# HUSRCF/JaTSR-Just-audio-transformer-super-solution

Measured on AMD Instinct MI355X. Metric: DiT latent-frames/sec (B=28,C=1024,T=512, 50-step CFG), higher is better.
Workload: dtype bf16; 1 GPU; v3mod2 DiT 50-step CFG=3.0 flow-matching sampling, hipGraph, B=28/GPU C=1024 T=512; B_per_gpu=28, global_batch=28, T=512, C=1024, euler_steps=50, weights=recipe (random-init, non-zero adaLN/final), parallelism=replicas x1, no collective in the loop, rccl_ranks=1

## Files before the change

### include/jat_hip.h

```cpp
#ifndef JAT_HIP_H
#define JAT_HIP_H

#include <stddef.h>
#include <stdint.h>

#ifdef __cplusplus
extern "C" {
#endif

#define JAT_OK 0
#define JAT_E_INVALID (-1)
#define JAT_E_HIP (-2)
#define JAT_E_STATE (-3)
#define JAT_E_SEQLEN (-4)

#define JAT_NORM_RMS_W 0
#define JAT_NORM_LN_NOAFFINE 1

typedef struct jat_model jat_model;
typedef struct jat_sampler jat_sampler;

typedef struct jat_config {
  int32_t input_channels;
  int32_t cond_channels;
  int32_t patch_len;
  int32_t hidden_size;
  int32_t depth;
  int32_t num_q_heads;
  int32_t num_kv_heads;
  int32_t bottleneck_dim;
  int32_t mlp_hidden;
  int32_t norm_mode;
} jat_config;

typedef struct jat_tensor_ref {
  const char* name;
  const float* data;
  int64_t numel;
} jat_tensor_ref;

const char* jat_last_error(void);
int jat_version(void);
int jat_operand_dtype(void);

int jat_model_create(const jat_config* cfg, jat_model** out);
void jat_model_destroy(jat_model* m);
int jat_model_load_weights(jat_model* m, const jat_tensor_ref* named, int32_t n, void* stream);
int jat_model_workspace_bytes(const jat_model* m, int32_t B, int32_t T, size_t* out);
int jat_model_set_switch(jat_model* m, const char* name, int32_t value);

int jat_forward(jat_model* m, const float* x_t, const float* t, const float* x_cond, float* x_pred,
                int32_t B, int32_t T, void* workspace, size_t workspace_bytes, void* stream);

int jat_block_forward(jat_model* m, int32_t layer, const float* x, const float* t_emb, float* y,
                      int32_t B, int32_t N, void* workspace, size_t workspace_bytes, void* stream);
int jat_attn_forward(jat_model* m, int32_t layer, const float* x, float* y, int32_t B, int32_t N,
                     void* workspace, size_t workspace_bytes, void* stream);
int jat_time_embed(jat_model* m, const float* t, float* t_emb, int32_t B, void* workspace,
                   size_t workspace_bytes, void* stream);

int jat_sampler_create(jat_model* m, int32_t B, int32_t T, int32_t steps, float cfg_scale,
                       jat_sampler** out);
void jat_sampler_destroy(jat_sampler* s);
int jat_sampler_info(const jat_sampler* sampler, int32_t* folded, int32_t* fused_attn, int64_t* fold_bytes);
int jat_sampler_set_lengths(jat_sampler* sampler, const int32_t* frames, int32_t n, void* stream);

int jat_sampler_run(jat_sampler* s, const float* lr_latent, const float* z0_noise, float* z_out,
                    int32_t use_graph, void* stream);
int jat_cfg_euler_step(const float* x_pred_2B, float* z, float cfg_scale, float t, float dt, int32_t B,
                       int32_t C, int32_t T, void* stream);

int jat_channel_affine(const float* in, const float* mean, const float* std, float* out, int32_t B,
                       int32_t C, int32_t T, int32_t inverse, void* stream);
int jat_crossfade_pair(const float* prev, int32_t Tp, const float* cur, int32_t Tc, int32_t overlap,
                       float* out, int32_t rows, void* stream);

typedef struct jat_trainer jat_trainer;
int jat_trainer_create(jat_model* m, const jat_tensor_ref* params, int32_t n_params, float* params_flat,
                       float* grads_flat, float* exp_avg, float* exp_avg_sq, int64_t total, int32_t B, int32_t T,
                       void* stream, jat_trainer** out);
void jat_trainer_destroy(jat_trainer* tr);
int jat_trainer_set_grad_hook(jat_trainer* tr, void (*hook)(int64_t off, int64_t n, void* user), void* user);
int jat_trainer_set_regularisers(jat_trainer* tr, const float* dropout, const float* drop_path);
int jat_trainer_set_latent_loss(jat_trainer* tr, double latent_weight, double freq_weight, double ms_weight,
                                double consistency_weight, double low_freq_phase_ratio, double strict_cutoff,
                                double soft_cutoff);
int jat_trainer_set_charbonnier(jat_trainer* tr, double eps);
int jat_trainer_loss_terms(jat_trainer* tr, float* out6, void* stream);
int jat_trainer_workspace_bytes(const jat_trainer* tr, size_t* out);
int jat_trainer_repack(jat_trainer* tr, void* stream);
int jat_trainer_prepare(jat_trainer* tr, const float* hr_norm, float* cond, const float* noise,
                        const float* cond_noise, float cond_noise_ratio, int32_t adaptive, const float* keep,
                        const float* t, float* z_t, void* stream);
int jat_trainer_fwd_bwd(jat_trainer* tr, const float* z_t, const float* t, const float* x_cond, const float* target,
                        const float* cond_clean, float loss_scale, uint64_t rng_seed, float* loss_out, float* x_pred_out,
                        void* stream);
int jat_trainer_optim(jat_trainer* tr, float lr, float beta1, float beta2, float eps, float weight_decay,
                      float max_grad_norm, float loss_scale, int32_t step, float* grad_norm_out, void* stream);

int jat_k_norm_modulate(const float* x, const float* w, const float* shift, const float* scale,
                        int64_t mod_bstride, uint16_t* y_bf16, int32_t M, int32_t D, int32_t rows_per_batch,
                        int32_t norm_mode, void* stream);
int jat_k_gemm(const uint16_t* A, const uint16_t* W, const float* bias, void* C, int32_t M, int32_t N,
               int32_t K, int32_t epilogue, const float* gate, int64_t gate_bstride, int32_t rows_per_batch,
               int32_t variant, void* stream);
int jat_k_gemm_fold(const uint16_t* A, const uint16_t* W, const float* bias, void* C, int32_t M, int32_t N, int32_t K,
                    int32_t epilogue, const float* gate, int64_t gate_bstride, int32_t rows_per_batch, uint16_t* hi,
                    uint16_t* lo, float* part_out, const float* part_in, int32_t part_in_np, int32_t variant, void* stream);
int jat_k_gemm_splitk(const uint16_t* A, const uint16_t* W, float* parts, int32_t M, int32_t N, int32_t K, int32_t ksplit,
                      int32_t variant, void* stream);
int jat_k_qkv_attn(const uint16_t* A, const uint16_t* Wg, const float* bias, uint16_t* out, int32_t M, int32_t Hkv, int32_t K,
                   const float* rope_inv_freq, const float* part_in, int32_t part_in_np, void* stream);
int jat_k_gemm_wave_n(int32_t variant);
int jat_k_gemm_plan(const jat_model* m, int32_t site, int32_t M, int32_t N, int32_t K, int32_t folding, int32_t* variant,
                    int32_t* ksplit);
int jat_k_weight_grad(const uint16_t* dY, const uint16_t* X, float* dW, float* db, int32_t tokens, int32_t out, int32_t in,
                      int32_t ksplit, void* work, size_t work_bytes, void* stream);
int jat_k_attention(const uint16_t* q, const uint16_t* k, const uint16_t* vt, uint16_t* o, int32_t B,
                    int32_t N, int32_t Hq, int32_t Hkv, int32_t Npad, void* stream);
int jat_k_latent_loss(const float* pred, const float* target, const float* lr, float* dpred, float* out6,
                      int32_t rows, int32_t T, double latent_weight, double freq_weight, double ms_weight,
                      double consistency_weight, double low_freq_phase_ratio, double strict_cutoff, double soft_cutoff,
                      float loss_scale, void* work, size_t work_bytes, void* stream);
int jat_k_recon_loss(const float* pred, const float* target, float* dpred, float* loss_out, int64_t n, double eps,
                     float loss_scale, void* work, size_t work_bytes, void* stream);
int jat_k_cast_bf16(const float* in, uint16_t* out, int64_t n, void* stream);

int jat_k_attention_train(const uint16_t* q, const uint16_t* k, const uint16_t* vt, uint16_t* o, float* lse, int32_t B,
                          int32_t N, int32_t Hq, int32_t Hkv, int32_t Npad, uint64_t seed, int32_t site, float p, void* stream);
int jat_k_attention_bwd(const uint16_t* q, const uint16_t* k, const uint16_t* vt, const uint16_t* o, const uint16_t* dout,
                        const float* lse, uint16_t* dqkv, const float* rope_cos, const float* rope_sin, int32_t B, int32_t N,
                        int32_t Hq, int32_t Hkv, int32_t Npad, uint64_t seed, int32_t site, float p, int32_t split_heads,
                        void* work, size_t work_bytes, void* stream);
int jat_k_norm_bwd(const float* x, const uint16_t* dy, const float* w, const float* scale, int64_t mod_bstride, float* dx,
                   int32_t accumulate, float* dshift, float* dscale, int64_t dmod_bstride, float* dw, int32_t B, int32_t D,
                   int32_t ntok, int32_t mode, void* work, size_t work_bytes, void* stream);
int jat_k_gate_bwd(const float* dx, const uint16_t* y, const float* gate, int64_t gate_bstride, uint16_t* dy, float* dgate,
                   int64_t dgate_bstride, int32_t B, int32_t D, int32_t ntok, uint64_t seed, int32_t path_site, float path_p,
                   int32_t elem_site, float elem_p, void* work, size_t work_bytes, void* stream);
int jat_k_resid_gate(const float* x_in, const uint16_t* y, const float* gate, int64_t gate_bstride, float* x_out, int32_t M,
                     int32_t D, int32_t ntok, uint64_t seed, int32_t path_site, float path_p, int32_t elem_site, float elem_p,
                     void* stream);
int jat_k_gelu(const uint16_t* in, uint16_t* out, int64_t n, uint64_t seed, int32_t site, float p, void* stream);
int jat_k_gelu_bwd(const uint16_t* pre, uint16_t* d, int64_t n, uint64_t seed, int32_t site, float p, void* stream);
int jat_k_adamw(float* p, const float* g, float* m, float* v, int64_t n, float lr, float beta1, float beta2, float eps,
                float weight_decay, float max_grad_norm, float loss_scale, int32_t step, float* grad_norm_out, void* work,
                size_t work_bytes, void* stream);
int jat_k_small_dw(const float* dy, int64_t ldy, const float* x, int64_t ldx, float* dW, float* db, int32_t B, int32_t N,
                   int32_t K, int32_t silu_x, void* stream);
int jat_k_small_dx(const float* dy, int64_t ldy, const void* W, int32_t w_is_bf16, float* dx, int32_t B, int32_t N, int32_t K,
                   int32_t accumulate, const float* silu_pre, void* work, size_t work_bytes, void* stream);

int jat_prof_gemm_site(jat_model* m, int32_t site, int32_t max_launches);
int jat_prof_collect(jat_model* m, double* total_ms, int32_t* launches, double* flops, int32_t* variant);

typedef struct jat_dac_decoder jat_dac_decoder;
#define JAT_DAC_BF16X3 0
#define JAT_DAC_BF16 1
typedef struct jat_dac_config {
  int32_t latent_channels;
  int32_t channels;
  int32_t n_blocks;
  int32_t strides[4];
} jat_dac_config;
int jat_dac_decoder_create(const jat_dac_config* cfg, const jat_tensor_ref* named, int32_t n, int32_t max_B,
                           int32_t max_T, void* stream, jat_dac_decoder** out);
void jat_dac_decoder_destroy(jat_dac_decoder* d);
int jat_dac_workspace_bytes(const jat_dac_decoder* d, size_t* bytes);
int jat_dac_decode(jat_dac_decoder* d, const float* z, float* audio, int32_t B, int32_t T, int32_t precision, void* stream);
int jat_dac_pack_weight(int32_t kind, const float* w, int32_t cin, int32_t cout, int32_t k_or_stride, float* out);
int jat_k_dac_split(const float* x, uint16_t* hi, uint16_t* lo, int64_t n, void* stream);
int jat_k_dac_conv(const uint16_t* a_hi, const uint16_t* a_lo, const uint16_t* w_hi, const uint16_t* w_lo,
                   const float* bias, const float* res, float* out32, const float* alpha, uint16_t* o_hi, uint16_t* o_lo,
                   int32_t B, int32_t T, int32_t cin, int32_t N, int32_t cch, int32_t taps, int32_t dil,
                   int32_t precision, void* stream);
int jat_k_dac_tail(const float* x, const float* alpha, const float* w, const float* bias, float* out, int32_t B, int32_t T,
                   int32_t C, void* stream);

typedef struct jat_dac_encoder jat_dac_encoder;
#define JAT_DAC_MAX_CODEBOOKS 9
typedef struct jat_dac_encoder_config {
  int32_t channels;
  int32_t hidden_size;
  int32_t n_blocks;
  int32_t strides[4];
  int32_t n_codebooks;
  int32_t codebook_size;
  int32_t codebook_dim;
} jat_dac_encoder_config;
int jat_dac_encoder_create(const jat_dac_encoder_config* cfg, const jat_tensor_ref* named, int32_t n, int32_t max_B,
                           int32_t max_T, void* stream, jat_dac_encoder** out);
// ... 46 lines not shown
```

### jatsr-just-audio-transformer-super-solution_amd/_lib.py

```python
from __future__ import annotations

import ctypes as C
import os

_HERE = os.path.dirname(os.path.abspath(__file__))
OPERAND_DTYPE = os.environ.get("JAT_OPERAND_DTYPE", "bf16").lower()
if OPERAND_DTYPE not in ("bf16", "fp16", "float16", "bfloat16"):
    raise ValueError(f"JAT_OPERAND_DTYPE must be bf16 or fp16, got {OPERAND_DTYPE!r}")
OPERAND_DTYPE = "fp16" if OPERAND_DTYPE in ("fp16", "float16") else "bf16"
LIB_PATH = os.environ.get("JAT_LIB_PATH") or os.path.join(
    _HERE, "csrc", "libjat_hip_fp16.so" if OPERAND_DTYPE == "fp16" else "libjat_hip.so")

JAT_OK, JAT_E_INVALID, JAT_E_HIP, JAT_E_STATE, JAT_E_SEQLEN = 0, -1, -2, -3, -4
NORM_RMS_W, NORM_LN_NOAFFINE = 0, 1


class JatConfig(C.Structure):
    _fields_ = [(n, C.c_int32) for n in (
        "input_channels", "cond_channels", "patch_len", "hidden_size", "depth", "num_q_heads",
        "num_kv_heads", "bottleneck_dim", "mlp_hidden", "norm_mode")]


class JatDacConfig(C.Structure):
    _fields_ = [("latent_channels", C.c_int32), ("channels", C.c_int32), ("n_blocks", C.c_int32),
                ("strides", C.c_int32 * 4)]


class JatDacEncoderConfig(C.Structure):
    _fields_ = [("channels", C.c_int32), ("hidden_size", C.c_int32), ("n_blocks", C.c_int32), ("strides", C.c_int32 * 4),
                ("n_codebooks", C.c_int32), ("codebook_size", C.c_int32), ("codebook_dim", C.c_int32)]


class JatTensorRef(C.Structure):
    _fields_ = [("name", C.c_char_p), ("data", C.c_void_p), ("numel", C.c_int64)]


_VP, _I32, _I64, _F32, _SZ = C.c_void_p, C.c_int32, C.c_int64, C.c_float, C.c_size_t
SIGNATURES = {
    "jat_last_error": (C.c_char_p, []),
    "jat_version": (C.c_int, []),
    "jat_operand_dtype": (C.c_int, []),
    "jat_model_create": (C.c_int, [C.POINTER(JatConfig), C.POINTER(_VP)]),
    "jat_model_destroy": (None, [_VP]),
    "jat_model_load_weights": (C.c_int, [_VP, C.POINTER(JatTensorRef), _I32, _VP]),
    "jat_model_set_switch": (C.c_int, [_VP, C.c_char_p, _I32]),
    "jat_model_workspace_bytes": (C.c_int, [_VP, _I32, _I32, C.POINTER(_SZ)]),
    "jat_forward": (C.c_int, [_VP, _VP, _VP, _VP, _VP, _I32, _I32, _VP, _SZ, _VP]),
    "jat_block_forward": (C.c_int, [_VP, _I32, _VP, _VP, _VP, _I32, _I32, _VP, _SZ, _VP]),
    "jat_attn_forward": (C.c_int, [_VP, _I32, _VP, _VP, _I32, _I32, _VP, _SZ, _VP]),
    "jat_time_embed": (C.c_int, [_VP, _VP, _VP, _I32, _VP, _SZ, _VP]),
    "jat_sampler_create": (C.c_int, [_VP, _I32, _I32, _I32, _F32, C.POINTER(_VP)]),
    "jat_sampler_destroy": (None, [_VP]),
    "jat_sampler_run": (C.c_int, [_VP, _VP, _VP, _VP, _I32, _VP]),
    "jat_sampler_info": (C.c_int, [_VP, _VP, _VP, _VP]),
    "jat_sampler_set_lengths": (C.c_int, [_VP, C.POINTER(_I32), _I32, _VP]),
    "jat_cfg_euler_step": (C.c_int, [_VP, _VP, _F32, _F32, _F32, _I32, _I32, _I32, _VP]),
    "jat_channel_affine": (C.c_int, [_VP, _VP, _VP, _VP, _I32, _I32, _I32, _I32, _VP]),
    "jat_crossfade_pair": (C.c_int, [_VP, _I32, _VP, _I32, _I32, _VP, _I32, _VP]),
    "jat_k_norm_modulate": (C.c_int, [_VP, _VP, _VP, _VP, _I64, _VP, _I32, _I32, _I32, _I32, _VP]),
    "jat_k_gemm": (C.c_int, [_VP, _VP, _VP, _VP, _I32, _I32, _I32, _I32, _VP, _I64, _I32, _I32, _VP]),
    "jat_k_gemm_fold": (C.c_int, [_VP, _VP, _VP, _VP, _I32, _I32, _I32, _I32, _VP, _I64, _I32, _VP, _VP, _VP, _VP, _I32, _I32, _VP]),
    "jat_k_gemm_splitk": (C.c_int, [_VP, _VP, _VP, _I32, _I32, _I32, _I32, _I32, _VP]),
    "jat_k_gemm_wave_n": (C.c_int, [_I32]),
    "jat_k_gemm_plan": (C.c_int, [_VP, _I32, _I32, _I32, _I32, _I32, _VP, _VP]),
    "jat_k_qkv_attn": (C.c_int, [_VP, _VP, _VP, _VP, _I32, _I32, _I32, _VP, _VP, _I32, _VP]),
    "jat_k_weight_grad": (C.c_int, [_VP, _VP, _VP, _VP, _I32, _I32, _I32, _I32, _VP, _SZ, _VP]),
    "jat_k_attention": (C.c_int, [_VP, _VP, _VP, _VP, _I32, _I32, _I32, _I32, _I32, _VP]),
    "jat_k_recon_loss": (C.c_int, [_VP, _VP, _VP, _VP, _I64, C.c_double, _F32, _VP, _SZ, _VP]),
    "jat_k_cast_bf16": (C.c_int, [_VP, _VP, _I64, _VP]),
    "jat_k_attention_train": (C.c_int, [_VP] * 5 + [_I32] * 5 + [C.c_uint64, _I32, _F32, _VP]),
    "jat_k_attention_bwd": (C.c_int, [_VP] * 9 + [_I32] * 5 + [C.c_uint64, _I32, _F32, _I32, _VP, _SZ, _VP]),
    "jat_k_norm_bwd": (C.c_int, [_VP, _VP, _VP, _VP, _I64, _VP, _I32, _VP, _VP, _I64, _VP] + [_I32] * 4 + [_VP, _SZ, _VP]),
    "jat_k_gate_bwd": (C.c_int, [_VP, _VP, _VP, _I64, _VP, _VP, _I64] + [_I32] * 3 + [C.c_uint64, _I32, _F32, _I32, _F32] +
                       [_VP, _SZ, _VP]),
    "jat_k_resid_gate": (C.c_int, [_VP, _VP, _VP, _I64, _VP] + [_I32] * 3 + [C.c_uint64, _I32, _F32, _I32, _F32, _VP]),
    "jat_k_gelu": (C.c_int, [_VP, _VP, _I64, C.c_uint64, _I32, _F32, _VP]),
    "jat_k_gelu_bwd": (C.c_int, [_VP, _VP, _I64, C.c_uint64, _I32, _F32, _VP]),
    "jat_k_adamw": (C.c_int, [_VP, _VP, _VP, _VP, _I64] + [_F32] * 7 + [_I32, _VP, _VP, _SZ, _VP]),
    "jat_k_small_dw": (C.c_int, [_VP, _I64, _VP, _I64, _VP, _VP] + [_I32] * 4 + [_VP]),
    "jat_k_small_dx": (C.c_int, [_VP, _I64, _VP, _I32, _VP] + [_I32] * 4 + [_VP, _VP, _SZ, _VP]),
    "jat_k_latent_loss": (C.c_int, [_VP, _VP, _VP, _VP, _VP, _I32, _I32] + [C.c_double] * 7 + [_F32, _VP, _SZ, _VP]),
    "jat_trainer_create": (C.c_int, [_VP, C.POINTER(JatTensorRef), _I32, _VP, _VP, _VP, _VP, _I64, _I32, _I32, _VP,
                                     C.POINTER(_VP)]),
    "jat_trainer_destroy": (None, [_VP]),
    "jat_trainer_workspace_bytes": (C.c_int, [_VP, C.POINTER(_SZ)]),
    "jat_trainer_repack": (C.c_int, [_VP, _VP]),
    "jat_trainer_prepare": (C.c_int, [_VP, _VP, _VP, _VP, _VP, _F32, _I32, _VP, _VP, _VP, _VP]),
    "jat_trainer_set_grad_hook": (C.c_int, [_VP, _VP, _VP]),
    "jat_trainer_set_regularisers": (C.c_int, [_VP, C.POINTER(_F32), C.POINTER(_F32)]),
    "jat_trainer_set_latent_loss": (C.c_int, [_VP] + [C.c_double] * 7),
    "jat_trainer_set_charbonnier": (C.c_int, [_VP, C.c_double]),
    "jat_trainer_loss_terms": (C.c_int, [_VP, _VP, _VP]),
    "jat_trainer_fwd_bwd": (C.c_int, [_VP, _VP, _VP, _VP, _VP, _VP, _F32, C.c_uint64, _VP, _VP, _VP]),
    "jat_trainer_optim": (C.c_int, [_VP, _F32, _F32, _F32, _F32, _F32, _F32, _F32, _I32, _VP, _VP]),
    "jat_prof_gemm_site": (C.c_int, [_VP, _I32, _I32]),
    "jat_prof_collect": (C.c_int, [_VP, C.POINTER(C.c_double), C.POINTER(_I32), C.POINTER(C.c_double), C.POINTER(_I32)]),
    "jat_dac_decoder_create": (C.c_int, [C.c_void_p, C.POINTER(JatTensorRef), _I32, _I32, _I32, _VP, C.POINTER(_VP)]),
    "jat_dac_decoder_destroy": (None, [_VP]),
    "jat_dac_workspace_bytes": (C.c_int, [_VP, C.POINTER(_SZ)]),
    "jat_dac_decode": (C.c_int, [_VP, _VP, _VP, _I32, _I32, _I32, _VP]),
    "jat_dac_pack_weight": (C.c_int, [_I32, _VP, _I32, _I32, _I32, _VP]),
    "jat_k_dac_split": (C.c_int, [_VP, _VP, _VP, _I64, _VP]),
    "jat_k_dac_conv": (C.c_int, [_VP] * 10 + [_I32] * 8 + [_VP]),
    "jat_k_dac_tail": (C.c_int, [_VP] * 5 + [_I32] * 3 + [_VP]),
    "jat_dac_encoder_create": (C.c_int, [C.c_void_p, C.POINTER(JatTensorRef), _I32, _I32, _I32, _VP, C.POINTER(_VP)]),
    "jat_dac_encoder_destroy": (None, [_VP]),
    "jat_dac_encoder_workspace_bytes": (C.c_int, [_VP, C.POINTER(_SZ)]),
    "jat_dac_encode": (C.c_int, [_VP] * 6 + [_I32] * 4 + [_VP]),
    "jat_k_dac_head": (C.c_int, [_VP] * 7 + [_I32] * 3 + [_VP]),
    "jat_k_dac_rvq": (C.c_int, [_VP] * 10 + [_I32] * 4 + [_VP]),
    "jat_resample_table": (C.c_int, [_I32, _I32, _I32, C.c_double, _VP] + [C.POINTER(_I32)] * 4),
    "jat_resampler_create": (C.c_int, [_I32, _I32, _I32, C.c_double, _VP, C.POINTER(_VP)]),
    "jat_resampler_destroy": (None, [_VP]),
    "jat_resample_out_length": (C.c_int, [_VP, _I64, C.POINTER(_I64)]),
    "jat_resample": (C.c_int, [_VP, _VP, _VP, _I32, _I64, _VP]),
    "jat_channel_stats": (C.c_int, [_VP, _I32, _I32, _I32, _VP, _VP, _VP, _SZ, _VP]),
    "jat_mel_filterbank": (C.c_int, [_I32, _I32, _I32, _VP]),
    "jat_stft_frames": (C.c_int, [_I64, _I32, C.POINTER(_I64)]),
    "jat_audio_metrics_create": (C.c_int, [_I32, _I32, _I32, _I32, _VP, C.POINTER(_VP)]),
    "jat_audio_metrics_destroy": (None, [_VP]),
    "jat_audio_metrics_workspace_bytes": (C.c_int, [_VP, _I32, _I64, C.POINTER(_SZ)]),
    "jat_audio_metrics_run": (C.c_int, [_VP, _VP, _VP, _I32, _I64, _I32, _VP, _VP, _VP, _VP, _VP, _SZ, _VP]),
    "jat_stft": (C.c_int, [_VP, _VP, _VP, _I32, _I64, _VP, _VP, _VP]),
    "jat_latent_gather": (C.c_int, [_VP] * 10 + [_I32] * 3 + [_VP]),
    "jat_train_monitor": (C.c_int, [_VP, _VP, _VP, _I64, _VP, _VP, _SZ, _VP]),
}
MONITOR_WORK_BYTES = 49152

GRAD_HOOK = C.CFUNCTYPE(None, C.c_int64, C.c_int64, C.c_void_p)

_lib = None


class JatError(RuntimeError):
    pass


def lib():
    global _lib
    if _lib is None:
        if not os.path.exists(LIB_PATH):
            raise JatError(f"{LIB_PATH} not found: build it first (`python -c 'import __graft_entry__ as g; "
                           f"g.build()'` or `make -C {os.path.dirname(LIB_PATH)}`); there is no CPU fallback")
        h = C.CDLL(LIB_PATH)
# ... 40 lines not shown
```

### jatsr-just-audio-transformer-super-solution_amd/csrc/elementwise.hip

```cpp
#include "jat_kernels.h"
#include "jat_gelu.h"
#include "jat_dtype.h"
#include <cstdlib>

__device__ __forceinline__ unsigned short f2bf_e(float f) { return jat_f2op(f); }
__device__ __forceinline__ uint2 pack4_e(float a, float b, float c, float d) {
  uint2 r;
  r.x = jat_pack2(a, b);
  r.y = jat_pack2(c, d);
  return r;
}
__device__ __forceinline__ float wave_sum(float v) {
#pragma unroll
  for (int o = 32; o > 0; o >>= 1) v += __shfl_xor(v, o);
  return v;
}
__device__ __forceinline__ float silu_f(float x) { return x / (1.0f + __expf(-x)); }

__global__ void __launch_bounds__(256) norm_modulate_kernel(const float* __restrict__ x, const float* __restrict__ w,
                                                            const float* __restrict__ shift,
                                                            const float* __restrict__ scale, int64_t mod_bstride,
                                                            bf16_t* __restrict__ y, int M, int D, int ntok, int mode) {
  const int lane = threadIdx.x & 63;
  const int row = blockIdx.x * 4 + (threadIdx.x >> 6);
  if (row >= M) return;
  const int nch = D >> 8;
  const float* xr = x + (int64_t)row * D + lane * 4;
  float4 v[8];
  float s1 = 0.f, s2 = 0.f;
#pragma unroll
  for (int c = 0; c < 8; ++c) {
    if (c < nch) {
      v[c] = *(const float4*)(xr + c * 256);
      s1 += v[c].x + v[c].y + v[c].z + v[c].w;
      s2 += v[c].x * v[c].x + v[c].y * v[c].y + v[c].z * v[c].z + v[c].w * v[c].w;
    }
  }
  float mu = 0.f, rstd = 1.f;
  if (mode == 0) {
    s2 = wave_sum(s2);
    rstd = rsqrtf(s2 / (float)D + 1e-6f);
  } else if (mode == 1) {
    s1 = wave_sum(s1);
    mu = s1 / (float)D;
    float var = 0.f;
#pragma unroll
    for (int c = 0; c < 8; ++c)
      if (c < nch) {
        const float a = v[c].x - mu, b2 = v[c].y - mu, c2 = v[c].z - mu, d2 = v[c].w - mu;
        var += a * a + b2 * b2 + c2 * c2 + d2 * d2;
      }
    var = wave_sum(var);
    rstd = rsqrtf(var / (float)D + 1e-6f);
  }
  const int b = row / ntok;
  const float* sh = shift ? shift + (int64_t)b * mod_bstride + lane * 4 : nullptr;
  const float* sc = scale ? scale + (int64_t)b * mod_bstride + lane * 4 : nullptr;
  bf16_t* yr = y + (int64_t)row * D + lane * 4;
#pragma unroll
  for (int c = 0; c < 8; ++c) {
    if (c < nch) {
      float4 t = v[c];
      t.x = (t.x - mu) * rstd; t.y = (t.y - mu) * rstd; t.z = (t.z - mu) * rstd; t.w = (t.w - mu) * rstd;
      if (mode == 0 && w) {
        const float4 ww = *(const float4*)(w + c * 256 + lane * 4);
        t.x *= ww.x; t.y *= ww.y; t.z *= ww.z; t.w *= ww.w;
      }
      if (sc) {
        const float4 a = *(const float4*)(sc + c * 256);
        const float4 s = *(const float4*)(sh + c * 256);
        t.x = t.x * (1.f + a.x) + s.x; t.y = t.y * (1.f + a.y) + s.y;
        t.z = t.z * (1.f + a.z) + s.z; t.w = t.w * (1.f + a.w) + s.w;
      }
      *(uint2*)(yr + c * 256) = pack4_e(t.x, t.y, t.z, t.w);
    }
  }
}

typedef __attribute__((ext_vector_type(4))) float f32x4_e;
template <int NCH>
__global__ void __launch_bounds__(256) norm_modulate_rows_kernel(const float* __restrict__ x, const float* __restrict__ w,
                                                                 const float* __restrict__ shift,
                                                                 const float* __restrict__ scale, int64_t mod_bstride,
                                                                 bf16_t* __restrict__ y, int M, int ntok, int mode) {
  constexpr int D = NCH * 256;
// ... 223 lines not shown
  if (n <= 0) return hipSuccess;
  hipLaunchKernelGGL(cast_bf16_kernel, dim3((unsigned)((n + 1023) / 1024)), dim3(256), 0, s, in, out, n, 1);
  return hipGetLastError();
}

__global__ void cast_bf16_rope_rows_kernel(const float* __restrict__ in, bf16_t* __restrict__ out, int rows, int cols) {
  const int64_t i = ((int64_t)blockIdx.x * blockDim.x + threadIdx.x) * 4;
  if (i >= (int64_t)rows * cols) return;
  const int r = (int)(i / cols), c = (int)(i - (int64_t)r * cols);
  const int h = r >> 6, q = r & 63;
  const int src = (h << 6) + (q >> 1) + ((q & 1) << 5);
  const float4 v = *(const float4*)(in + (int64_t)src * cols + c);
  *(uint2*)(out + i) = pack4_e(v.x, v.y, v.z, v.w);
}
hipError_t launch_cast_bf16_rope_rows(const float* in, bf16_t* out, int rows, int cols, hipStream_t s) {
  if (rows % 64 != 0 || cols % 4 != 0) return hipErrorInvalidValue;
  const int64_t n = (int64_t)rows * cols;
  hipLaunchKernelGGL(cast_bf16_rope_rows_kernel, dim3((unsigned)((n / 4 + 255) / 256)), dim3(256), 0, s, in, out, rows,
                     cols);
  return hipGetLastError();
}

__global__ void fold_weight_kernel(const float* __restrict__ in, const float* __restrict__ w, const float* __restrict__ scale,
                                   bf16_t* __restrict__ out, int rows, int cols, int rope) {
  const int64_t i = ((int64_t)blockIdx.x * blockDim.x + threadIdx.x) * 4;
  if (i >= (int64_t)rows * cols) return;
  const int r = (int)(i / cols), c = (int)(i - (int64_t)r * cols);
  int src = r;
  if (rope) {
    const int h = r >> 6, q = r & 63;
    src = (h << 6) + (q >> 1) + ((q & 1) << 5);
  }
  const float4 v = *(const float4*)(in + (int64_t)src * cols + c);
  float4 g = *(const float4*)(w + c);
  if (scale) {
    const float4 sc = *(const float4*)(scale + c);
    g.x *= 1.0f + sc.x; g.y *= 1.0f + sc.y; g.z *= 1.0f + sc.z; g.w *= 1.0f + sc.w;
  }
  *(uint2*)(out + i) = pack4_e(v.x * g.x, v.y * g.y, v.z * g.z, v.w * g.w);
}
hipError_t launch_fold_weight(const float* in, const float* w, const float* scale, bf16_t* out, int rows, int cols, int rope,
                              hipStream_t s) {
  if ((rope && rows % 64 != 0) || cols % 4 != 0) return hipErrorInvalidValue;
  const int64_t n = (int64_t)rows * cols;
  hipLaunchKernelGGL(fold_weight_kernel, dim3((unsigned)((n / 4 + 255) / 256)), dim3(256), 0, s, in, w, scale, out, rows, cols, rope);
  return hipGetLastError();
}

__global__ void fold_scale_kernel(const float* __restrict__ w, const float* __restrict__ scale, int64_t in_stride,
                                  float* __restrict__ out, int64_t out_stride, int rows, int cols) {
  const int i = blockIdx.x * blockDim.x + threadIdx.x;
  if (i >= rows * cols) return;
  const int r = i / cols, k = i - r * cols;
  out[(int64_t)r * out_stride + k] = w[k] * (1.0f + scale[(int64_t)r * in_stride + k]);
}
hipError_t launch_fold_scale(const float* w, const float* scale, int64_t in_stride, float* out, int64_t out_stride,
                             int rows, int cols, hipStream_t s) {
  const int n = rows * cols;
  hipLaunchKernelGGL(fold_scale_kernel, dim3((n + 255) / 256), dim3(256), 0, s, w, scale, in_stride, out, out_stride, rows, cols);
  return hipGetLastError();
}
__global__ void gather_cast_rows_kernel(const float* __restrict__ in, int64_t in_stride, bf16_t* __restrict__ out, int rows,
                                        int cols) {
  const int i = blockIdx.x * blockDim.x + threadIdx.x;
  if (i >= rows * cols) return;
  const int r = i / cols, k = i - r * cols;
  out[(int64_t)r * cols + k] = f2bf_e(in[(int64_t)r * in_stride + k]);
}
hipError_t launch_gather_cast_rows(const float* in, int64_t in_stride, bf16_t* out, int rows, int cols, hipStream_t s) {
  const int n = rows * cols;
  hipLaunchKernelGGL(gather_cast_rows_kernel, dim3((n + 255) / 256), dim3(256), 0, s, in, in_stride, out, rows, cols);
  return hipGetLastError();
}

__global__ void __launch_bounds__(256) cfg_euler_kernel(const float* __restrict__ xp, float* __restrict__ z,
                                                        float cfg_scale, float denom, float dt, int use_cfg,
                                                        int direct, int64_t n) {
  const int64_t stride = (int64_t)gridDim.x * blockDim.x * 4;
  for (int64_t i = ((int64_t)blockIdx.x * blockDim.x + threadIdx.x) * 4; i < n; i += stride) {
    if (i + 3 < n) {
      float4 c = *(const float4*)(xp + i);
      if (use_cfg) {
        const float4 u = *(const float4*)(xp + n + i);
        c.x = u.x + cfg_scale * (c.x - u.x); c.y = u.y + cfg_scale * (c.y - u.y);
        c.z = u.z + cfg_scale * (c.z - u.z); c.w = u.w + cfg_scale * (c.w - u.w);
      }
      if (!direct) {
        const float4 zz = *(const float4*)(z + i);
        c.x = zz.x + __fdiv_rn(c.x - zz.x, denom) * dt; c.y = zz.y + __fdiv_rn(c.y - zz.y, denom) * dt;
        c.z = zz.z + __fdiv_rn(c.z - zz.z, denom) * dt; c.w = zz.w + __fdiv_rn(c.w - zz.w, denom) * dt;
      }
      *(float4*)(z + i) = c;
    } else {
      for (int64_t j = i; j < n; ++j) {
        float c = xp[j];
        if (use_cfg) { const float u = xp[n + j]; c = u + cfg_scale * (c - u); }
        if (!direct) c = z[j] + __fdiv_rn(c - z[j], denom) * dt;
        z[j] = c;
      }
    }
  }
}
hipError_t launch_cfg_euler(const float* xp, float* z, float cfg_scale, float t, float dt, int use_cfg,
                            int64_t n_per_half, hipStream_t s) {
  const int direct = !(t < 0.999f);
  const float denom = 1.0f - t + 1e-5f;
  int64_t blocks = (n_per_half / 4 + 255) / 256;
  if (blocks > 2048) blocks = 2048;
  if (blocks < 1) blocks = 1;
  hipLaunchKernelGGL(cfg_euler_kernel, dim3((unsigned)blocks), dim3(256), 0, s, xp, z, cfg_scale, denom, dt, use_cfg,
                     direct, n_per_half);
  return hipGetLastError();
}

__global__ void channel_affine_kernel(const float* __restrict__ in, const float* __restrict__ mean,
                                      const float* __restrict__ sd, float* __restrict__ out, int C, int T,
                                      int inverse, int64_t n) {
  const int64_t i = (int64_t)blockIdx.x * blockDim.x + threadIdx.x;
  if (i >= n) return;
  const int c = (int)((i / T) % C);
  out[i] = inverse ? in[i] * sd[c] + mean[c] : (in[i] - mean[c]) / sd[c];
}
hipError_t launch_channel_affine(const float* in, const float* mean, const float* std, float* out, int B, int C, int T,
                                 int inverse, hipStream_t s) {
  const int64_t n = (int64_t)B * C * T;
  if (n <= 0) return hipSuccess;
  hipLaunchKernelGGL(channel_affine_kernel, dim3((unsigned)((n + 255) / 256)), dim3(256), 0, s, in, mean, std, out, C,
                     T, inverse, n);
  return hipGetLastError();
}

__device__ __forceinline__ float linspace_at(float a, float b, int n, int i) {
  if (n == 1) return a;
  const float step = (b - a) / (float)(n - 1);
  return i < n / 2 ? fmaf(step, (float)i, a) : fmaf(-step, (float)(n - 1 - i), b);
}
__global__ void crossfade_pair_kernel(const float* __restrict__ prev, int Tp, const float* __restrict__ cur, int Tc,
                                      int ov, float* __restrict__ out, int rows) {
  const int To = Tp + Tc - ov;
  const int64_t i = (int64_t)blockIdx.x * blockDim.x + threadIdx.x;
  if (i >= (int64_t)rows * To) return;
  const int r = (int)(i / To), t = (int)(i - (int64_t)r * To);
  float v;
  if (t < Tp - ov) {
    v = prev[(int64_t)r * Tp + t];
  } else if (t < Tp) {
    const int k = t - (Tp - ov);
    v = prev[(int64_t)r * Tp + t] * linspace_at(1.f, 0.f, ov, k) + cur[(int64_t)r * Tc + k] * linspace_at(0.f, 1.f, ov, k);
  } else {
    v = cur[(int64_t)r * Tc + (t - Tp + ov)];
  }
  out[i] = v;
}
hipError_t launch_crossfade_pair(const float* prev, int Tp, const float* cur, int Tc, int overlap, float* out, int rows,
                                 hipStream_t s) {
  if (overlap < 0 || overlap > Tp || overlap > Tc) return hipErrorInvalidValue;
  const int64_t n = (int64_t)rows * (Tp + Tc - overlap);
  if (n <= 0) return hipSuccess;
  hipLaunchKernelGGL(crossfade_pair_kernel, dim3((unsigned)((n + 255) / 256)), dim3(256), 0, s, prev, Tp, cur, Tc,
                     overlap, out, rows);
  return hipGetLastError();
}

__global__ void __launch_bounds__(256) splitk_resid_finish_kernel(const float* __restrict__ part, int nsplit, int64_t stride,
                                                                  const float* __restrict__ bias, const float* __restrict__ gate,
                                                                  int64_t gate_bstride, int ntok, float* __restrict__ x, int M,
                                                                  int N) {
  const int64_t i = (int64_t)blockIdx.x * 256 + threadIdx.x;
  const int per_row = N / 4;
  if (i >= (int64_t)M * per_row) return;
  const int row = (int)(i / per_row), c = (int)(i % per_row) * 4;
  f32x4_e acc = *(const f32x4_e*)(part + (int64_t)row * N + c);
  for (int z = 1; z < nsplit; ++z) {
    const f32x4_e v = *(const f32x4_e*)(part + (int64_t)z * stride + (int64_t)row * N + c);
    acc[0] += v[0]; acc[1] += v[1]; acc[2] += v[2]; acc[3] += v[3];
  }
  const f32x4_e b = bias ? *(const f32x4_e*)(bias + c) : f32x4_e{0.f, 0.f, 0.f, 0.f};
  const f32x4_e g = *(const f32x4_e*)(gate + (int64_t)(row / ntok) * gate_bstride + c);
  f32x4_e xv = *(const f32x4_e*)(x + (int64_t)row * N + c);
#pragma unroll
  for (int j = 0; j < 4; ++j) xv[j] += g[j] * (acc[j] + b[j]);
  *(f32x4_e*)(x + (int64_t)row * N + c) = xv;
}
__global__ void __launch_bounds__(256) splitk_gelu_finish_kernel(const float* __restrict__ part, int nsplit, int64_t stride,
                                                                 const float* __restrict__ bias, const float* __restrict__ dual_add,
                                                                 int dual_rows, bf16_t* __restrict__ out, int64_t ldo, int M, int N) {
  const int64_t i = (int64_t)blockIdx.x * 256 + threadIdx.x;
  const int per_row = N / 4;
  if (i >= (int64_t)M * per_row) return;
  const int row = (int)(i / per_row), c = (int)(i % per_row) * 4;
  f32x4_e acc = *(const f32x4_e*)(part + (int64_t)row * N + c);
  for (int z = 1; z < nsplit; ++z) {
    const f32x4_e v = *(const f32x4_e*)(part + (int64_t)z * stride + (int64_t)row * N + c);
    acc[0] += v[0]; acc[1] += v[1]; acc[2] += v[2]; acc[3] += v[3];
  }
// ... 127 lines not shown
```

### jatsr-just-audio-transformer-super-solution_amd/csrc/gemm.hip

```cpp
#include "jat_kernels.h"
#include "jat_dtype.h"
#include "gemm_variants.h"

#include <type_traits>
#include <utility>

typedef jat_opx8 bf16x8;
typedef __attribute__((ext_vector_type(4))) float f32x4;
typedef __attribute__((ext_vector_type(4))) unsigned u32x4;
typedef __attribute__((address_space(3))) void* lds_ptr_t;

template <int I, int N, class F>
__device__ __forceinline__ void static_for(F&& f) {
  if constexpr (I < N) {
    f(std::integral_constant<int, I>{});
    static_for<I + 1, N>(f);
  }
}

__device__ __forceinline__ unsigned short f2bf(float f) { return jat_f2op(f); }
__device__ __forceinline__ uint2 pack4(float a, float b, float c, float d) {
  uint2 r;
  r.x = jat_pack2(a, b);
  r.y = jat_pack2(c, d);
  return r;
}
#include "jat_gelu.h"
__device__ __forceinline__ uint2 gelu_pack4(float a, float b, float c, float d) {
  f32x2 g[2] = {f32x2{a, b}, f32x2{c, d}};
  gelu_erf_n<2>(g);
  return pack4(g[0][0], g[0][1], g[1][0], g[1][1]);
}

__device__ __forceinline__ float2 rope_rot(float a, float b, float c, float s) {
  return float2{__builtin_fmaf(a, c, -(b * s)), __builtin_fmaf(b, c, a * s)};
}

template <int TM>
__device__ __forceinline__ void rows_rstd_issue(const GemmArgs& p, int row0, int lane, f32x4 (&rsv)[TM]) {
  const int lg = p.rs_np >> 3;
  const int rpi = 64 >> lg;
#pragma unroll
  for (int t = 0; t < TM; ++t) {
    const int row = min(row0 + t * rpi + (lane >> lg), p.M - 1);
    const float* ptr = p.rs_part + (int64_t)row * p.rs_np + (lane & ((1 << lg) - 1)) * 4;
    asm volatile("global_load_dwordx4 %0, %1, off" : "=v"(rsv[t]) : "v"(ptr) : "memory");
  }
}
template <int TM, int YOUNGER>
__device__ __forceinline__ void rows_rstd_reduce(const GemmArgs& p, f32x4 (&rsv)[TM], float (&sums)[TM]) {
  asm volatile("s_waitcnt vmcnt(%0)" ::"n"(YOUNGER) : "memory");
#pragma unroll
  for (int t = 0; t < TM; ++t) asm volatile("" : "+v"(rsv[t]));
  const int lpr = p.rs_np >> 2;
#pragma unroll
  for (int t = 0; t < TM; ++t) {
    float sq = (rsv[t][0] + rsv[t][1]) + (rsv[t][2] + rsv[t][3]);
    if (lpr >= 2) sq += __shfl_xor(sq, 1);
    if (lpr >= 4) sq += __shfl_xor(sq, 2);
    sums[t] = sq;
  }
}
template <int TM>
__device__ __forceinline__ void rows_rstd_finish(const GemmArgs& p, int lane, const float (&sums)[TM], float (&rstd)[TM]) {
  const int lg = p.rs_np >> 3, rlog = 6 - lg, frow = lane & 15;
  const float invk = 1.0f / (float)p.K;
  float sq[TM];
#pragma unroll
  for (int i = 0; i < TM; ++i) {
    const int ti = (i * 16) >> rlog;
    float sel = sums[0];
#pragma unroll
    for (int t = 1; t < TM; ++t) sel = (t == ti) ? sums[t] : sel;
    sq[i] = __shfl(sel, ((i * 16 + frow) & ((1 << rlog) - 1)) << lg);
  }
#pragma unroll
  for (int i = 0; i < TM; ++i) rstd[i] = rsqrtf(sq[i] * invk + 1e-6f);
}
template <int WM, int WN, int TM, int TN, int PIPE, int CE, int EPI>
__global__ void __launch_bounds__((WM * WN + (PIPE == 6 ? 4 : 0)) * 64, (WM * WN == 4 && TM * TN <= 20) ? 2 : 1)
    gemm_bf16_kernel(const GemmArgs p_in) {
  GemmArgs p = p_in;
#ifdef JAT_TIMELINE
  unsigned long long tl_[7] = {0, 0, 0, 0, 0, 0, 0}, tlx_[8] = {0, 0, 0, 0, 0, 0, 0, 0};
#define JAT_TL(i)                                                                          \
  if (p.dbg_out) {                                                                         \
    __builtin_amdgcn_sched_barrier(0);                                                     \
    asm volatile("s_memtime %0\n\ts_waitcnt lgkmcnt(0)" : "=s"(tl_[i])::"memory");       \
    __builtin_amdgcn_sched_barrier(0);                                                     \
  }
#define JAT_TLX(i)                                                                         \
  if (p.dbg_out) {                                                                         \
    __builtin_amdgcn_sched_barrier(0);                                                     \
    asm volatile("s_memtime %0\n\ts_waitcnt lgkmcnt(0)" : "=s"(tlx_[i])::"memory");      \
    __builtin_amdgcn_sched_barrier(0);                                                     \
  }
#define JAT_TLR(i)                                                                         \
  if (p.dbg_out) {                                                                         \
    __builtin_amdgcn_sched_barrier(0);                                                     \
    asm volatile("s_memrealtime %0\n\ts_waitcnt lgkmcnt(0)" : "=s"(tl_[i])::"memory");   \
    __builtin_amdgcn_sched_barrier(0);                                                     \
  }
#define JAT_TL_FLUSH()                                                                     \
  {                                                                                        \
    JAT_TL(4) JAT_TLR(6)                                                                   \
    if (p.dbg_out && (threadIdx.x & 63) == 0) {                                            \
      unsigned long long* o_ = p.dbg_out + ((size_t)blockIdx.x * (blockDim.x >> 6) + (threadIdx.x >> 6)) * 16; \
      for (int i_ = 0; i_ < 7; ++i_) o_[i_] = tl_[i_];                                     \
      o_[7] = blockIdx.x;                                                                  \
      for (int i_ = 0; i_ < 8; ++i_) o_[8 + i_] = tlx_[i_];                                \
    }                                                                                      \
  }
  JAT_TL(0) JAT_TLR(5)
#else
#define JAT_TL(i)
#define JAT_TLX(i)
#define JAT_TLR(i)
#define JAT_TL_FLUSH()
#endif
  if (p.ksplit > 1) {
    const int z = blockIdx.y;
    p.A += (int64_t)z * p.K;
    p.W += (int64_t)z * p.K;
    p.out = (float*)p.out + (int64_t)z * p.split_stride;
  }
  constexpr int BM = WM * TM * 16, BN = WN * TN * 16, BK = 64;
  constexpr int NW = WM * WN;
  constexpr int A_BYTES = BM * 128, B_BYTES = BN * 128, STAGE = A_BYTES + B_BYTES;
  constexpr int PA = BM / 8, PB = BN / 8;
  constexpr int AI = (PA + NW - 1) / NW, BI = (PB + NW - 1) / NW;
  static_assert(BM % 8 == 0 && BN % 8 == 0, "tile rows must be a multiple of 8");
  extern __shared__ __attribute__((aligned(16))) char smem[];

  const int tid = threadIdx.x, lane = tid & 63;
  const int wave = __builtin_amdgcn_readfirstlane(tid >> 6);
  const int wm = wave / WN, wn = wave % WN;

  const int tiles_m = (p.M + BM - 1) / BM, tiles_n = p.N / BN;
  int id;
  {
    const int nwg = gridDim.x, bid = blockIdx.x;
    const int q = nwg >> 3, r = nwg & 7, xcd = bid & 7;
    id = (xcd < r ? xcd * (q + 1) : r * (q + 1) + (xcd - r) * q) + (bid >> 3);
  }
  constexpr int GROUP = 8;
  const int per_group = GROUP * tiles_n;
  const int first_m = (id / per_group) * GROUP;
  const int gsz = min(tiles_m - first_m, GROUP);
  const int in_g = id % per_group;
  const int m0 = (first_m + in_g % gsz) * BM;
  const int n0 = (in_g / gsz) * BN;

  const int srow = lane >> 3;
  const int schunk = (lane & 7) ^ srow;
  const bf16_t* a_src[AI];
  const bf16_t* b_src[BI];
#pragma unroll
  for (int j = 0; j < AI; ++j) {
    const int r = min(wave + j * NW, PA - 1) * 8 + srow;
    const int gm = min(m0 + r, p.M - 1);
    a_src[j] = p.A + (int64_t)gm * p.lda + schunk * 8;
  }
#pragma unroll
  for (int j = 0; j < BI; ++j) {
    const int r = min(wave + j * NW, PB - 1) * 8 + srow;
    b_src[j] = p.W + (int64_t)(n0 + r) * p.ldw + schunk * 8;
  }
  auto stage = [&](int st, int kt) {
    char* sA = smem + st * STAGE;
    char* sB = sA + A_BYTES;
    const int koff = kt * BK;
#pragma unroll
    for (int j = 0; j < AI; ++j)
      if (PA % NW == 0 || wave + j * NW < PA)
        __builtin_amdgcn_global_load_lds((const void*)(a_src[j] + koff),
                                         (lds_ptr_t)(sA + min(wave + j * NW, PA - 1) * 1024), 16, 0, 0);
#pragma unroll
    for (int j = 0; j < BI; ++j)
      if (PB % NW == 0 || wave + j * NW < PB)
        __builtin_amdgcn_global_load_lds((const void*)(b_src[j] + koff),
                                         (lds_ptr_t)(sB + min(wave + j * NW, PB - 1) * 1024), 16, 0, 0);
  };

  f32x4 acc[TM][TN];
#pragma unroll
  for (int i = 0; i < TM; ++i)
#pragma unroll
    for (int j = 0; j < TN; ++j) acc[i][j] = f32x4{0.f, 0.f, 0.f, 0.f};

  const int frow = lane & 15, fg = lane >> 4;
  const int a_row_off = (wm * TM * 16 + frow) * 128;
  const int b_row_off = (wn * TN * 16 + frow) * 128;
  const int coff0 = ((0 + fg) ^ (frow & 7)) * 16, coff1 = ((4 + fg) ^ (frow & 7)) * 16;
  constexpr bool QA = EPI == EPI_QKV_ATTN;
  static_assert(!QA || (TN == 7 && WN == 4), "fused QKV + attention: 5 q + k + v tiles per wave column");
  auto ctile = [](int w, int j) { return QA ? (j < 5 ? w * 5 + j : j == 5 ? 20 + w : 24 + w) : w * TN + j; };
  auto b_frag_off = [&](int j) {
    return QA ? ctile(wn, j) * 2048 + frow * 128 : b_row_off + j * 2048;
  };

  auto read_frags = [&](bf16x8(&af)[TM], bf16x8(&wf)[TN], int st, int coff) {
    const char* sA = smem + st * STAGE;
    const char* sB = sA + A_BYTES;
#pragma unroll
    for (int i = 0; i < TM; ++i) af[i] = *(const bf16x8*)(sA + a_row_off + i * 2048 + coff);
#pragma unroll
    for (int j = 0; j < TN; ++j) wf[j] = *(const bf16x8*)(sB + b_row_off + j * 2048 + coff);
  };
  auto mma = [&](const bf16x8(&af)[TM], const bf16x8(&wf)[TN]) {
#pragma unroll
    for (int i = 0; i < TM; ++i)
#pragma unroll
      for (int j = 0; j < TN; ++j)
        acc[i][j] = JAT_MFMA_16x16x32(wf[j], af[i], acc[i][j], 0, 0, 0);
  };

  float rstd_rows[TM], rstd_sums[TM];
  [[maybe_unused]] f32x4 rstd_raw[TM];
#pragma unroll
  for (int i = 0; i < TM; ++i) rstd_rows[i] = 1.0f;
  if (p.rs_part) {
    rows_rstd_issue<TM>(p, m0 + wm * TM * 16, lane, rstd_raw);
    if constexpr (PIPE != 8) rows_rstd_reduce<TM, 0>(p, rstd_raw, rstd_sums);
  }

  const int nk = p.K / BK;
  if constexpr (PIPE == 6) {
    static_assert(NW == 8 && PA % 4 == 0 && PB % 4 == 0, "PIPE 6: 8 MFMA waves + 4 DMA waves");
    constexpr int NDW = 4, AI6 = PA / NDW, BI6 = PB / NDW;
    if (wave >= NW) {
      const int dw = wave - NW;
      const bf16_t* asrc[AI6];
      const bf16_t* bsrc[BI6];
#pragma unroll
      for (int j = 0; j < AI6; ++j)
        asrc[j] = p.A + (int64_t)min(m0 + (dw + j * NDW) * 8 + srow, p.M - 1) * p.lda + schunk * 8;
#pragma unroll
      for (int j = 0; j < BI6; ++j) bsrc[j] = p.W + (int64_t)(n0 + (dw + j * NDW) * 8 + srow) * p.ldw + schunk * 8;
      auto issue_a = [&](int st, int kt) {
#pragma unroll
        for (int j = 0; j < AI6; ++j)
          __builtin_amdgcn_global_load_lds((const void*)(asrc[j] + kt * BK),
                                           (lds_ptr_t)(smem + st * STAGE + (dw + j * NDW) * 1024), 16, 0, 0);
      };
      auto issue_b = [&](int st, int kt) {
#pragma unroll
        for (int j = 0; j < BI6; ++j)
          __builtin_amdgcn_global_load_lds((const void*)(bsrc[j] + kt * BK),
                                           (lds_ptr_t)(smem + st * STAGE + A_BYTES + (dw + j * NDW) * 1024), 16, 0, 0);
      };
      issue_a(0, 0);
      issue_b(0, 0);
      if (nk > 1) {
        issue_a(1, 1);
        issue_b(1, 1);
        asm volatile("s_waitcnt vmcnt(%0)" ::"n"(AI6 + BI6) : "memory");
      } else {
        asm volatile("s_waitcnt vmcnt(0)" ::: "memory");
      }
      __builtin_amdgcn_s_barrier();
      int st = 2;
      for (int sl = 0; sl <= 2 * nk; ++sl) {
        const int t = (sl >> 1) + 2;
        if (t < nk) {
          if (sl & 1) issue_b(st, t); else issue_a(st, t);
          asm volatile("s_waitcnt vmcnt(%0)" ::"n"(AI6 + BI6) : "memory");
        } else {
          asm volatile("s_waitcnt vmcnt(0)" ::: "memory");
        }
        __builtin_amdgcn_s_barrier();
        if (sl & 1) st = st == 2 ? 0 : st + 1;
      }
      if constexpr (CE && EPI <= EPI_QKV_ROPE) __builtin_amdgcn_s_barrier();
      return;
    }
    const int grp = wave >> 2;
    bf16x8 a0[TM], w0[TN], a1[TM], w1[TN];
    __builtin_amdgcn_s_barrier();
    if (grp == 1) __builtin_amdgcn_s_barrier();
    int cur = 0;
    for (int kt = 0; kt < nk; ++kt) {
      read_frags(a0, w0, cur, coff0);
      read_frags(a1, w1, cur, coff1);
      asm volatile("s_waitcnt lgkmcnt(0)" ::: "memory");
      __builtin_amdgcn_sched_barrier(0);
      __builtin_amdgcn_s_barrier();
      __builtin_amdgcn_s_setprio(1);
      mma(a0, w0);
      mma(a1, w1);
      __builtin_amdgcn_s_setprio(0);
      __builtin_amdgcn_sched_barrier(0);
      __builtin_amdgcn_s_barrier();
      cur = cur == 2 ? 0 : cur + 1;
    }
    if (grp == 0) __builtin_amdgcn_s_barrier();
  } else if constexpr (PIPE == 8) {
    static_assert(NW == 8, "quadrant ping-pong needs two waves per SIMD in one block");
    constexpr bool SPLIT_M = TM * TN > 20;
    constexpr int TMa = SPLIT_M ? (TM + 1) / 2 : TM, TMb = TM - TMa, TNa = (TN + 1) / 2, TNb = TN - TNa;
    constexpr int PA0 = WM * TMa * 2, PA1 = WM * TMb * 2, PB0 = WN * TNa * 2, PB1 = WN * TNb * 2;
    constexpr int CA0 = (PA0 + 7) / 8, CA1 = (PA1 + 7) / 8, CB0 = (PB0 + 7) / 8, CB1 = (PB1 + 7) / 8;
    constexpr int CTILE = CA0 + CA1 + CB0 + CB1;
    const int grp = wave >> 2;
    const char* a_base = (const char*)(p.A + (int64_t)m0 * p.lda);
    const char* b_base = (const char*)(p.W + (int64_t)n0 * p.ldw);
    unsigned oa0[CA0], oa1[CA1 > 0 ? CA1 : 1], ob0[CB0], ob1[CB1];
    int la0[CA0], la1[CA1 > 0 ? CA1 : 1], lb0[CB0], lb1[CB1];
    auto piece_row = [&](int q, int per, int tiles, int first) {
      const int w = q / per, in = q - w * per;
      return w * tiles * 16 + first * 16 + in * 8;
    };
#pragma unroll
    for (int j = 0; j < CA0; ++j) {
      const int r = piece_row(min(wave + 8 * j, PA0 - 1), TMa * 2, TM, 0);
      oa0[j] = (unsigned)((min(m0 + r + srow, p.M - 1) - m0) * (int)p.lda * 2 + schunk * 16);
      la0[j] = r * 128;
    }
#pragma unroll
    for (int j = 0; j < CA1; ++j) {
      const int r = piece_row(min(wave + 8 * j, PA1 - 1), TMb * 2, TM, TMa);
      oa1[j] = (unsigned)((min(m0 + r + srow, p.M - 1) - m0) * (int)p.lda * 2 + schunk * 16);
      la1[j] = r * 128;
    }
    auto piece_row_b = [&](int q, int per, int first) {
      const int w = q / per, in = q - w * per;
      return ctile(w, first + (in >> 1)) * 16 + (in & 1) * 8;
    };
#pragma unroll
    for (int j = 0; j < CB0; ++j) {
      const int r = piece_row_b(min(wave + 8 * j, PB0 - 1), TNa * 2, 0);
      ob0[j] = (unsigned)((r + srow) * (int)p.ldw * 2 + schunk * 16);
      lb0[j] = A_BYTES + r * 128;
    }
#pragma unroll
    for (int j = 0; j < CB1; ++j) {
      const int r = piece_row_b(min(wave + 8 * j, PB1 - 1), TNb * 2, TNa);
      ob1[j] = (unsigned)((r + srow) * (int)p.ldw * 2 + schunk * 16);
      lb1[j] = A_BYTES + r * 128;
    }
    auto dma_a0 = [&](int st, int kt) {
#pragma unroll
      for (int j = 0; j < CA0; ++j)
        __builtin_amdgcn_global_load_lds((const void*)(a_base + kt * 128 + oa0[j]), (lds_ptr_t)(smem + st * STAGE + la0[j]), 16, 0, 0);
    };
    auto dma_a1 = [&](int st, int kt) {
#pragma unroll
      for (int j = 0; j < CA1; ++j)
        __builtin_amdgcn_global_load_lds((const void*)(a_base + kt * 128 + oa1[j]), (lds_ptr_t)(smem + st * STAGE + la1[j]), 16, 0, 0);
    };
    auto dma_b0 = [&](int st, int kt) {
#pragma unroll
      for (int j = 0; j < CB0; ++j)
        __builtin_amdgcn_global_load_lds((const void*)(b_base + kt * 128 + ob0[j]), (lds_ptr_t)(smem + st * STAGE + lb0[j]), 16, 0, 0);
    };
    auto dma_b1 = [&](int st, int kt) {
#pragma unroll
      for (int j = 0; j < CB1; ++j)
        __builtin_amdgcn_global_load_lds((const void*)(b_base + kt * 128 + ob1[j]), (lds_ptr_t)(smem + st * STAGE + lb1[j]), 16, 0, 0);
    };
    bf16x8 fa[2][TMa], fb[2][TNa];
    auto rd_a = [&](int st, int i0, int cnt) {
      const char* sA = smem + st * STAGE + a_row_off + i0 * 2048;
#pragma unroll
      for (int i = 0; i < TMa; ++i)
        if (i < cnt) {
          fa[0][i] = *(const bf16x8*)(sA + i * 2048 + coff0);
          fa[1][i] = *(const bf16x8*)(sA + i * 2048 + coff1);
        }
    };
    auto rd_b = [&](int st, int j0, int cnt) {
      if constexpr (QA) {
        const char* sB = smem + st * STAGE + A_BYTES;
#pragma unroll
        for (int j = 0; j < TNa; ++j)
          if (j < cnt) {
            fb[0][j] = *(const bf16x8*)(sB + b_frag_off(j0 + j) + coff0);
            fb[1][j] = *(const bf16x8*)(sB + b_frag_off(j0 + j) + coff1);
          }
      } else {
        const char* sB = smem + st * STAGE + A_BYTES + b_row_off + j0 * 2048;
#pragma unroll
        for (int j = 0; j < TNa; ++j)
          if (j < cnt) {
            fb[0][j] = *(const bf16x8*)(sB + j * 2048 + coff0);
            fb[1][j] = *(const bf16x8*)(sB + j * 2048 + coff1);
          }
      }
    };
#define JAT_Q(I0, IC, J0, JC)                                                                                   \
  _Pragma("unroll") for (int ks = 0; ks < 2; ++ks)                                                              \
  _Pragma("unroll") for (int i = 0; i < (IC); ++i)                                                              \
  _Pragma("unroll") for (int j = 0; j < (JC); ++j)                                                              \
    acc[(I0) + i][(J0) + j] = (QA && (J0) + j == TN - 1)                                                        \
        ? JAT_MFMA_16x16x32(fa[ks][i], fb[ks][j], acc[(I0) + i][(J0) + j], 0, 0, 0)                             \
        : JAT_MFMA_16x16x32(fb[ks][j], fa[ks][i], acc[(I0) + i][(J0) + j], 0, 0, 0);
#define JAT_LOAD_END()                              \
  asm volatile("s_waitcnt lgkmcnt(0)" ::: "memory"); \
  __builtin_amdgcn_sched_barrier(0);                \
  __builtin_amdgcn_s_barrier();                     \
  __builtin_amdgcn_s_setprio(1);
#define JAT_MMA_END()                 \
  __builtin_amdgcn_s_setprio(0);      \
  __builtin_amdgcn_sched_barrier(0);  \
  __builtin_amdgcn_s_barrier();
// ... 493 lines not shown
    const int q = wave * 16 + frow;
    constexpr int G = 5;
    const int hbase = (n0 / 448) * G;
    bf16x8 qf[G][2];
#pragma unroll
    for (int h = 0; h < G; ++h) {
      qf[h][0] = *(const bf16x8*)(smem + SQ + h * 16384 + q * 128 + (((0 + fg) ^ (q & 7)) << 4));
      qf[h][1] = *(const bf16x8*)(smem + SQ + h * 16384 + q * 128 + (((4 + fg) ^ (q & 7)) << 4));
    }
    f32x4 st[G][8];
#pragma unroll
    for (int h = 0; h < G; ++h)
#pragma unroll
      for (int kt = 0; kt < 8; ++kt) st[h][kt] = f32x4{0.f, 0.f, 0.f, 0.f};
#pragma unroll
    for (int kt = 0; kt < 8; ++kt) {
      const int r = 32 * (kt >> 1) + 8 * (frow >> 2) + (frow & 3) + 4 * (kt & 1);
      const int ks = (r & 3) | (((r >> 3) & 1) << 2);
      const bf16x8 kf0 = *(const bf16x8*)(smem + SK + r * 128 + (((0 + fg) ^ ks) << 4));
      const bf16x8 kf1 = *(const bf16x8*)(smem + SK + r * 128 + (((4 + fg) ^ ks) << 4));
#pragma unroll
      for (int h = 0; h < G; ++h) {
        st[h][kt] = JAT_MFMA_16x16x32(kf0, qf[h][0], st[h][kt], 0, 0, 0);
        st[h][kt] = JAT_MFMA_16x16x32(kf1, qf[h][1], st[h][kt], 0, 0, 0);
      }
    }
    JAT_TLX(2)
    float inv[G];
    bf16x8 pf[G][4];
#pragma unroll
    for (int h = 0; h < G; ++h) {
      float mx = -1e30f;
#pragma unroll
      for (int kt = 0; kt < 8; ++kt) mx = fmaxf(mx, fmaxf(fmaxf(st[h][kt][0], st[h][kt][1]), fmaxf(st[h][kt][2], st[h][kt][3])));
      mx = fmaxf(mx, __shfl_xor(mx, 16));
      mx = fmaxf(mx, __shfl_xor(mx, 32));
      const float nb = -mx * p.attn_scale_log2e;
      float sum = 0.f;
#pragma unroll
      for (int kt = 0; kt < 8; ++kt)
#pragma unroll
        for (int e = 0; e < 4; ++e) {
          const float pv = __builtin_amdgcn_exp2f(fmaf(st[h][kt][e], p.attn_scale_log2e, nb));
          st[h][kt][e] = pv;
          sum += pv;
        }
      sum += __shfl_xor(sum, 16);
      sum += __shfl_xor(sum, 32);
      inv[h] = 1.0f / sum;
#pragma unroll
      for (int kk = 0; kk < 4; ++kk) {
        pf[h][kk] = jat_pack8(st[h][2 * kk], st[h][2 * kk + 1]);
      }
    }
    JAT_TLX(3)
    f32x4 o[G][4];
#pragma unroll
    for (int h = 0; h < G; ++h)
#pragma unroll
      for (int dt = 0; dt < 4; ++dt) o[h][dt] = f32x4{0.f, 0.f, 0.f, 0.f};
#pragma unroll
    for (int kk = 0; kk < 4; ++kk)
#pragma unroll
      for (int dt = 0; dt < 4; ++dt) {
        const int d = dt * 16 + frow, ch = kk * 4 + fg;
        const bf16x8 vf = *(const bf16x8*)(smem + SV + d * 256 + (ch >> 3) * 128 + (((ch & 7) ^ (d & 7)) << 4));
#pragma unroll
        for (int h = 0; h < G; ++h) o[h][dt] = JAT_MFMA_16x16x32(vf, pf[h][kk], o[h][dt], 0, 0, 0);
      }
    JAT_TLX(4)
    if (m0 + q < p.M) {
#pragma unroll
      for (int h = 0; h < G; ++h) {
        bf16_t* op = (bf16_t*)p.out + (int64_t)(m0 + q) * p.ldo + (hbase + h) * 64 + fg * 4;
#pragma unroll
        for (int dt = 0; dt < 4; ++dt)
          *(uint2*)(op + dt * 16) = pack4(o[h][dt][0] * inv[h], o[h][dt][1] * inv[h], o[h][dt][2] * inv[h], o[h][dt][3] * inv[h]);
      }
    }
    JAT_TL_FLUSH()
    return;
  }

#pragma unroll
  for (int i = 0; i < TM; ++i) {
    const int m = m0 + wm * TM * 16 + i * 16 + frow;
    if (m >= p.M) continue;
    int b = 0, pos = m;
    if constexpr (EPI == EPI_RESID || EPI == EPI_QKV_ROPE || EPI == EPI_UNPATCH) {
      b = m / p.ntok;
      pos = m - b * p.ntok;
    }
    const float rstd_d = rstd_rows[i];
#pragma unroll
    for (int j = 0; j < TN; ++j) {
      const int nt = nw0 + j * 16;
      const int n = nt + fg * 4;
      f32x4 v = acc[i][j] * rstd_d;
      if constexpr (EPI == EPI_QKV_ROPE) {
        if (nt < p.D + p.kvD) {
          const int d0 = ((nt & 63) >> 1) + fg * 2;
          const float2 c = *(const float2*)(p.rope_cos + (int64_t)pos * 32 + d0);
          const float2 s = *(const float2*)(p.rope_sin + (int64_t)pos * 32 + d0);
          const float o0 = v[0] * c.x - v[1] * s.x, o1 = v[1] * c.x + v[0] * s.x;
          const float o2 = v[2] * c.y - v[3] * s.y, o3 = v[3] * c.y + v[2] * s.y;
          bf16_t* dst = (nt < p.D) ? ((bf16_t*)p.out + (int64_t)m * p.D + n)
                                   : (p.k_out + (int64_t)m * p.kvD + (n - p.D));
          *(uint2*)dst = pack4(o0, o1, o2, o3);
        } else {
          const int nv = n - p.D - p.kvD;
          bf16_t* dst = p.vt_out + ((int64_t)(b * (p.kvD >> 6) + (nv >> 6)) * 64 + (nv & 63)) * p.npad + pos;
#pragma unroll
          for (int r = 0; r < 4; ++r) dst[(int64_t)r * p.npad] = f2bf(v[r]);
        }
      } else {
        if (p.bias) {
          const float4 bb = *(const float4*)(p.bias + n);
          v[0] += bb.x; v[1] += bb.y; v[2] += bb.z; v[3] += bb.w;
        }
        if constexpr (EPI == EPI_F32) {
          *(float4*)((float*)p.out + (int64_t)m * p.ldo + n) = float4{v[0], v[1], v[2], v[3]};
        } else if constexpr (EPI == EPI_BF16) {
          *(uint2*)((bf16_t*)p.out + (int64_t)m * p.ldo + n) = pack4(v[0], v[1], v[2], v[3]);
        } else if constexpr (EPI == EPI_BF16_GELU) {
          *(uint2*)((bf16_t*)p.out + (int64_t)m * p.ldo + n) = gelu_pack4(v[0], v[1], v[2], v[3]);
        } else if constexpr (EPI == EPI_RESID) {
          const float4 g = *(const float4*)(p.gate + (int64_t)b * p.gate_bstride + n);
          float4* xp = (float4*)((float*)p.out + (int64_t)m * p.ldo + n);
          float4 x = *xp;
          x.x += g.x * v[0]; x.y += g.y * v[1]; x.z += g.z * v[2]; x.w += g.w * v[3];
          *xp = x;
        } else if constexpr (EPI == EPI_UNPATCH) {
          const int c = n >> 2, t0 = pos * 4;
          float* dst = (float*)p.out + ((int64_t)b * p.C_out + c) * p.T_orig + t0;
          if ((p.T_orig & 3) == 0) {
            *(float4*)dst = float4{v[0], v[1], v[2], v[3]};
          } else {
#pragma unroll
            for (int r = 0; r < 4; ++r)
              if (t0 + r < p.T_orig) dst[r] = v[r];
          }
        }
      }
    }
  }
}

template <int WM, int WN, int TM, int TN, int EPI>
__global__ void __launch_bounds__(WM * WN * 64, 1) gemm_persist_kernel(const GemmArgs p) {
  constexpr int BM = WM * TM * 16, BN = WN * TN * 16;
  constexpr int NW = WM * WN;
  constexpr int A_BYTES = BM * 128, B_BYTES = BN * 128, STAGE = A_BYTES + B_BYTES;
  static_assert(NW == 8 && TM * TN > 20, "the row-split quadrant ping-pong of the large wave tiles");
  static_assert(EPI == EPI_BF16 || EPI == EPI_BF16_GELU, "consumer epilogues only");
  constexpr int TMa = (TM + 1) / 2, TMb = TM - TMa, TNa = (TN + 1) / 2, TNb = TN - TNa;
  constexpr int PA0 = WM * TMa * 2, PA1 = WM * TMb * 2, PB0 = WN * TNa * 2, PB1 = WN * TNb * 2;
  constexpr int CA0 = (PA0 + 7) / 8, CA1 = (PA1 + 7) / 8, CB0 = (PB0 + 7) / 8, CB1 = (PB1 + 7) / 8;
  constexpr int CTILE = CA0 + CA1 + CB0 + CB1;
  constexpr int XB_PIECES = (BN * 4 + 1023) / 1024, XP_PIECES = BM * 64 / 1024;
  constexpr int XB_OFF = 2 * STAGE, XP_OFF = XB_OFF + XB_PIECES * 1024;
  constexpr int CXP = (XP_PIECES + 7) / 8, CX = 1 + CXP;
  static_assert(BM * 64 % 1024 == 0, "whole pieces of row partials");
  constexpr int RS = TN * 32 + 16, SLAB = 16 * RS, CPR = TN * 2, NCH = (16 * CPR + 63) / 64;
  constexpr int NST = TM * NCH;
  static_assert(NW * 2 * SLAB <= STAGE, "slabs live in stage 1");
  static_assert(NST + CTILE <= 63 && 2 * CTILE + CX <= 63, "vmcnt immediates");
  extern __shared__ __attribute__((aligned(16))) char smem[];

  const int tid = threadIdx.x, lane = tid & 63;
  const int wave = __builtin_amdgcn_readfirstlane(tid >> 6);
  const int wm = wave / WN, wn = wave % WN, grp = wave >> 2;
  const int tiles_m = p.M / BM, tiles_n = p.N / BN, ntiles = tiles_m * tiles_n;
  const int nk = p.K / 64;
  auto coords = [&](int v, int& m0, int& n0) {
    const int q = ntiles >> 3, r = ntiles & 7, xcd = v & 7;
    const int id = (xcd < r ? xcd * (q + 1) : r * (q + 1) + (xcd - r) * q) + (v >> 3);
    constexpr int GROUP = 8;
    const int per_group = GROUP * tiles_n;
    const int first_m = (id / per_group) * GROUP;
    const int gsz = min(tiles_m - first_m, GROUP);
    const int in_g = id % per_group;
    m0 = (first_m + in_g % gsz) * BM;
    n0 = (in_g / gsz) * BN;
  };
  const int srow = lane >> 3, schunk = (lane & 7) ^ srow;
  const int frow = lane & 15, fg = lane >> 4;
  const int a_row_off = (wm * TM * 16 + frow) * 128;
  const int b_row_off = (wn * TN * 16 + frow) * 128;
  const int coff0 = ((0 + fg) ^ (frow & 7)) * 16, coff1 = ((4 + fg) ^ (frow & 7)) * 16;
  unsigned oa0[CA0], oa1[CA1], ob0[CB0], ob1[CB1];
  int la0[CA0], la1[CA1], lb0[CB0], lb1[CB1];
  auto piece_row = [&](int q, int per, int tiles, int first) {
    const int w = q / per, in = q - w * per;
    return w * tiles * 16 + first * 16 + in * 8;
  };
#pragma unroll
  for (int j = 0; j < CA0; ++j) {
    const int r = piece_row(min(wave + 8 * j, PA0 - 1), TMa * 2, TM, 0);
    oa0[j] = (unsigned)((r + srow) * (int)p.lda * 2 + schunk * 16);
// ... 487 lines not shown
        if (row < 32) *(float*)slot = live ? sq : 0.f;
      }
      asm volatile("s_waitcnt lgkmcnt(0)" ::: "memory");
      if constexpr (!PART) {
        constexpr int HALF = CPR8 / 2;
        const int r = lane >> 1, h = lane & 1;
        float sq = 0.f;
#pragma unroll
        for (int cc = 0; cc < HALF; ++cc) sq += *(const float*)(wbuf + r * RS + (h * HALF + cc) * 32);
        sq += __shfl_xor(sq, 1);
        const int m = mw0 + ig * 32 + r;
        if (h == 0 && r < grows) p.fold_part[(int64_t)m * p.fold_np + nw0 / (TN * 16)] = sq;
      }
      asm volatile("s_waitcnt lgkmcnt(0)" ::: "memory");
    }
  };
  if (grp == 0) half_epilogue(std::integral_constant<int, 0>{}, std::integral_constant<int, 4>{});
  else half_epilogue(std::integral_constant<int, 4>{}, std::integral_constant<int, 3>{});
  JAT_TL_FLUSH()
}

static bool gemm_kpair_eligible(const GemmArgs& a, int epi) {
  return (epi == EPI_RESID || epi == EPI_F32) && a.fold_out && a.fold_lo && a.fold_part && a.M > 0 && a.M % 224 == 0 &&
         a.N % 160 == 0 && a.K % 64 == 0 && a.ksplit <= 1 && !a.rs_part &&
         (int64_t)a.M * a.ldo * 2 < (1ll << 32);
}
static bool gemm_kpair_part_eligible(const GemmArgs& a, int epi) {
  return epi == EPI_F32 && a.ksplit > 1 && !a.fold_out && !a.rs_part && !a.dual_rows && a.out && a.M > 0 && a.M % 224 == 0 &&
         a.N % 160 == 0 && a.K % 64 == 0 && a.K >= 192;
}
template <int EPI, int LONGK, bool PART = false>
static hipError_t launch_kpair(const GemmArgs& a, hipStream_t s) {
  constexpr int LDS = 3 * (224 + 160) * 128;
  static_assert(LDS <= 160 * 1024, "three stages must fit the 160 KiB LDS");
  static bool attr_set = false;
  auto kern = gemm_kpair_kernel<EPI, LONGK, PART>;
  if (!attr_set) {
    hipError_t e = hipFuncSetAttribute((const void*)kern, hipFuncAttributeMaxDynamicSharedMemorySize, LDS);
    if (e != hipSuccess) return e;
    attr_set = true;
  }
  hipLaunchKernelGGL(kern, dim3((a.M / 224) * (a.N / 160), PART ? a.ksplit : 1), dim3(512), LDS, s, a);
  return hipGetLastError();
}

static bool gemm_persist_eligible(const GemmArgs& a, int epi) {
  return (epi == EPI_BF16 || epi == EPI_BF16_GELU) && a.M > 0 && a.M % 224 == 0 && a.N % 320 == 0 && a.K % 64 == 0 && a.ksplit <= 1 &&
         a.dual_rows == 0 && !a.fold_out && (!a.rs_part || a.rs_np == 16) && a.ldo * 2 * 16 < (1ll << 31);
}
template <int EPI>
static hipError_t launch_persist(const GemmArgs& a, hipStream_t s) {
  constexpr int BM = 224, BN = 320, STAGE = (BM + BN) * 128;
  constexpr int LDS = 2 * STAGE + 2048 + BM * 64;
  static_assert(LDS <= 160 * 1024, "stages + bias slice + row partials must fit the 160 KiB LDS");
  static bool attr_set = false;
  auto kern = gemm_persist_kernel<2, 4, 7, 5, EPI>;
  if (!attr_set) {
    hipError_t e = hipFuncSetAttribute((const void*)kern, hipFuncAttributeMaxDynamicSharedMemorySize, LDS);
    if (e != hipSuccess) return e;
    attr_set = true;
  }
  const int tiles = (a.M / BM) * (a.N / BN);
  int grid = tiles <= 256 ? tiles : (tiles + 1) / 2;
  if (grid < 256 && tiles > 256) grid = 256;
  static const int half_env = getenv("JAT_PERSIST_HALF") ? atoi(getenv("JAT_PERSIST_HALF")) : 0;
  if (half_env > 0 && tiles > half_env && tiles <= 2 * half_env) grid = (tiles + 1) / 2;
  hipLaunchKernelGGL(kern, dim3(grid), dim3(512), LDS, s, a);
  return hipGetLastError();
}

template <int WM, int WN, int TM, int TN, int PIPE, int CE, int EPI>
static hipError_t launch_one(const GemmArgs& a, hipStream_t s) {
  constexpr int BM = WM * TM * 16, BN = WN * TN * 16;
  constexpr int LDS = (PIPE == 6 ? 3 : 2) * (BM + BN) * 128;
  static_assert(LDS <= 160 * 1024, "tile does not fit the 160 KiB LDS");
  static bool attr_set = false;
  auto kern = gemm_bf16_kernel<WM, WN, TM, TN, PIPE, CE, EPI>;
  if (!attr_set) {
    hipError_t e = hipFuncSetAttribute((const void*)kern, hipFuncAttributeMaxDynamicSharedMemorySize, LDS);
    if (e != hipSuccess) return e;
    attr_set = true;
  }
  if (a.N % BN != 0 || a.K % 64 != 0 || a.M <= 0) return hipErrorInvalidValue;
  const int tiles = ((a.M + BM - 1) / BM) * (a.N / BN);
  if (a.ksplit > 1 && EPI != EPI_F32) return hipErrorInvalidValue;
  hipLaunchKernelGGL(kern, dim3(tiles, a.ksplit > 1 ? a.ksplit : 1), dim3((WM * WN + (PIPE == 6 ? 4 : 0)) * 64), LDS, s, a);
  return hipGetLastError();
}

template <int WM, int WN, int TM, int TN, int PIPE, int CE = 0>
static hipError_t launch_epi(const GemmArgs& a, int epi, hipStream_t s) {
  switch (epi) {
    case EPI_F32: return launch_one<WM, WN, TM, TN, PIPE, CE, EPI_F32>(a, s);
    case EPI_BF16: return launch_one<WM, WN, TM, TN, PIPE, CE, EPI_BF16>(a, s);
    case EPI_BF16_GELU: return launch_one<WM, WN, TM, TN, PIPE, CE, EPI_BF16_GELU>(a, s);
    case EPI_RESID: return launch_one<WM, WN, TM, TN, PIPE, CE, EPI_RESID>(a, s);
    case EPI_QKV_ROPE: return launch_one<WM, WN, TM, TN, PIPE, CE, EPI_QKV_ROPE>(a, s);
    case EPI_UNPATCH: return launch_one<WM, WN, TM, TN, PIPE, CE, EPI_UNPATCH>(a, s);
  }
  return hipErrorInvalidValue;
}

hipError_t launch_qkv_attn(const GemmArgs& a, hipStream_t s) {
  if (a.ntok != 128 || a.N % 448 != 0 || a.M % 128 != 0) return hipErrorInvalidValue;
  return launch_one<2, 4, 4, 7, 8, 0, EPI_QKV_ATTN>(a, s);
}

template <int I>
static hipError_t launch_row(const GemmArgs& a, int epi, hipStream_t s) {
  constexpr GemmVariant v = kGemmVariants[I];
  static_assert(v.fallback >= 0 || v.blocks_per_cu == ((v.WM * v.WN == 4 && v.TM * v.TN <= 20) ? 2 : 1),
                "blocks_per_cu must be what the launch bounds of gemm_bf16_kernel allow");
  if constexpr (v.fallback >= 0) {
    constexpr const GemmVariant* f = gemm_variant(v.fallback);
    static_assert(f && f->fallback < 0 && f->WM == v.WM && f->WN == v.WN && f->TM == v.TM && f->TN == v.TN && f->PIPE == v.PIPE && f->CE == v.CE,
                  "a variant with a kernel of its own carries the row of its (live, final) fallback");
  }
  return launch_epi<v.WM, v.WN, v.TM, v.TN, v.PIPE, v.CE>(a, epi, s);
}
template <int... I>
static hipError_t launch_rows(int id, const GemmArgs& a, int epi, hipStream_t s, std::integer_sequence<int, I...>) {
  hipError_t e = hipErrorInvalidValue;
  (void)((kGemmVariants[I].id == id && ((e = launch_row<I>(a, epi, s)), true)) || ...);
  return e;
}

hipError_t launch_gemm(const GemmArgs& a, int epi, int variant, hipStream_t s) {
  const GemmVariant* v = gemm_variant(variant);
  if (!v) return hipErrorInvalidValue;
  if (a.N % v->bn() != 0) v = gemm_variant(a.N % 128 == 0 ? V_128x128 : V_LAST_RESORT);
  if (v->id == V_KPAIR) {
    if (gemm_kpair_part_eligible(a, epi)) return launch_kpair<EPI_F32, 0, true>(a, s);
    if (gemm_kpair_eligible(a, epi))
      return epi != EPI_RESID ? launch_kpair<EPI_F32, 0>(a, s) : a.K >= 4096 ? launch_kpair<EPI_RESID, 1>(a, s) : launch_kpair<EPI_RESID, 0>(a, s);
  }
  if (v->id == V_PERSIST && gemm_persist_eligible(a, epi))
    return epi == EPI_BF16 ? launch_persist<EPI_BF16>(a, s) : launch_persist<EPI_BF16_GELU>(a, s);
  return launch_rows(v->fallback >= 0 ? v->fallback : v->id, a, epi, s, std::make_integer_sequence<int, kNumGemmVariants>{});
}
```

### jatsr-just-audio-transformer-super-solution_amd/csrc/jat_api.cpp

```cpp
#include "../../include/jat_hip.h"

#include <hip/hip_runtime.h>

#include <cmath>
#include <cstdarg>
#include <cstdio>
#include <cstdlib>
#include <cstring>
#include <string>
#include <unordered_map>
#include <vector>

#include "jat_internal.h"
#include "jat_dtype.h"
#include "gemm_plan.h"
#include "gemm_variants.h"

static thread_local char g_err[512] = "";
int jat_fail(int code, const char* fmt, ...) {
  va_list ap;
  va_start(ap, fmt);
  vsnprintf(g_err, sizeof(g_err), fmt, ap);
  va_end(ap);
  return code;
}

struct Workspace {
  bf16_t *a_patch, *h_patch, *xn, *xlo, *q, *k, *vt, *ao, *hm, *t_silu;
  float *x, *mod, *e_sin, *t_h, *t_emb, *part;
  float* kpart;
  const int* lens = nullptr;
  const int* tvalid = nullptr;
  int npad;
  size_t vt_bytes, total;
};

static Workspace carve(const jat_model* m, int B, int ntok, char* base) {
  Workspace w;
  size_t off = 0;
  const size_t M = (size_t)B * ntok;
  auto take = [&](size_t bytes) {
    char* p = base ? base + off : nullptr;
    off += align_up(bytes, 256);
    return p;
  };
  w.npad = (int)align_up((size_t)ntok, 64);
  w.a_patch = (bf16_t*)take(M * m->Kp * 2);
  w.h_patch = (bf16_t*)take(M * m->bott * 2);
  w.x = (float*)take(M * m->D * 4);
  w.xn = (bf16_t*)take(M * m->D * 2);
  w.xlo = (bf16_t*)take(M * m->D * 2);
  w.q = (bf16_t*)take(M * m->D * 2);
  w.k = (bf16_t*)take(M * m->kvD * 2);
  w.vt_bytes = (size_t)B * m->Hkv * HEAD_DIM * w.npad * 2;
  w.vt = (bf16_t*)take(w.vt_bytes);
  w.ao = (bf16_t*)take(M * m->D * 2);
  w.hm = (bf16_t*)take(M * m->mlp * 2);
  w.mod = (float*)take((size_t)B * m->depth * 6 * m->D * 4);
  w.e_sin = (float*)take((size_t)B * m->D * 4);
  w.t_h = (float*)take((size_t)B * m->D * 4);
  w.t_emb = (float*)take((size_t)B * m->D * 4);
  w.t_silu = (bf16_t*)take((size_t)B * m->D * 2);
  w.part = (float*)take(M * 32 * 4);
  w.kpart = split_ws_slices(M) ? (float*)take((size_t)split_ws_slices(M) * M * (m->D + 2 * m->kvD) * 4) : nullptr;
  w.total = off;
  return w;
}

extern "C" const char* jat_last_error(void) { return g_err; }
extern "C" int jat_version(void) { return 2; }
extern "C" int jat_operand_dtype(void) { return JAT_OPERAND_DTYPE; }

extern "C" int jat_model_create(const jat_config* c, jat_model** out) {
  if (!c || !out) return fail(JAT_E_INVALID, "null argument");
  if (c->num_q_heads <= 0 || c->hidden_size % c->num_q_heads != 0)
    return fail(JAT_E_INVALID, "hidden_size must be divisible by num_q_heads");
  if (c->num_kv_heads <= 0 || c->num_q_heads % c->num_kv_heads != 0)
    return fail(JAT_E_INVALID, "num_q_heads must be divisible by num_kv_heads");
  if (c->hidden_size / c->num_q_heads != HEAD_DIM) return fail(JAT_E_INVALID, "head_dim must be 64");
  if (c->patch_len != 4) return fail(JAT_E_INVALID, "patch_len must be 4");
  if (c->hidden_size % 256 != 0 || c->hidden_size > 2048)
    return fail(JAT_E_INVALID, "hidden_size must be a multiple of 256, <= 2048");
  if (c->bottleneck_dim % 128 != 0 || c->mlp_hidden % 128 != 0)
    return fail(JAT_E_INVALID, "bottleneck_dim and mlp_hidden must be multiples of 128");
  if (c->input_channels % 32 != 0 || c->cond_channels % 32 != 0 || c->input_channels <= 0 || c->cond_channels <= 0)
    return fail(JAT_E_INVALID, "channel counts must be positive multiples of 32");
  if (c->depth <= 0) return fail(JAT_E_INVALID, "depth must be positive");
  if (c->norm_mode != JAT_NORM_RMS_W && c->norm_mode != JAT_NORM_LN_NOAFFINE)
    return fail(JAT_E_INVALID, "unknown norm_mode");
  jat_model* m = new jat_model();
  m->cfg = *c;
  m->D = c->hidden_size; m->depth = c->depth; m->Hq = c->num_q_heads; m->Hkv = c->num_kv_heads;
  m->kvD = m->Hkv * HEAD_DIM; m->mlp = c->mlp_hidden; m->bott = c->bottleneck_dim;
  m->Cin = c->input_channels; m->Cc = c->cond_channels; m->P = 4;
  m->Kp = m->P * (m->Cin + m->Cc); m->Fout = m->P * m->Cin;
  auto env_int = [](const char* name, int dflt) { const char* v = getenv(name); return v ? atoi(v) : dflt; };
  m->sw.fuse_qkv_attn = env_int("JAT_FUSE_QKV_ATTN", 1); m->sw.qkv_split = env_int("JAT_QKV_SPLIT", 1);
  m->sw.fuse_finish = env_int("JAT_FUSE_FINISH", 1); m->sw.fold_norm = env_int("JAT_FOLD_NORM", 1);
  m->sw.split_patch = env_int("JAT_SPLIT_PATCH", 1);
  m->sw.fold_cap_mb = env_int("JAT_FOLD_CAP_MB", 0); m->sw.patch_split = env_int("JAT_PATCH_SPLIT", 1);
  if (const char* v = getenv("JAT_GEMM_VARIANT"))
    for (int i = 0; i < 5; ++i) m->variants[i] = atoi(v);
  if (const char* v = getenv("JAT_GEMM_VARIANTS")) {
    int x[5];
    if (sscanf(v, "%d,%d,%d,%d,%d", &x[0], &x[1], &x[2], &x[3], &x[4]) == 5)
      for (int i = 0; i < 5; ++i) m->variants[i] = x[i];
  }
  *out = m;
  return JAT_OK;
}

extern "C" int jat_model_set_switch(jat_model* m, const char* name, int32_t value) {
  if (!m || !name) return fail(JAT_E_INVALID, "null argument");
  const std::string n(name);
  int* slot = n == "fuse_qkv_attn" ? &m->sw.fuse_qkv_attn : n == "qkv_split" ? &m->sw.qkv_split : n == "fuse_finish" ? &m->sw.fuse_finish
            : n == "fold_norm" ? &m->sw.fold_norm : n == "split_patch" ? &m->sw.split_patch
            : n == "fold_cap_mb" ? &m->sw.fold_cap_mb : n == "patch_split" ? &m->sw.patch_split : nullptr;
  if (!slot) return fail(JAT_E_INVALID, "unknown switch '%s'", name);
  *slot = value;
  return JAT_OK;
}

extern "C" void jat_model_destroy(jat_model* m) {
  if (!m) return;
  for (hipEvent_t e : m->prof.ev) (void)hipEventDestroy(e);
  if (m->blob) (void)hipFree(m->blob);
  delete m;
}

extern "C" int jat_model_load_weights(jat_model* m, const jat_tensor_ref* named, int32_t n, void* stream_) {
  if (!m || !named) return fail(JAT_E_INVALID, "null argument");
  return jat_pack_weights(m, named, n, (hipStream_t)stream_, true);
}

int jat_pack_weights(jat_model* m, const jat_tensor_ref* named, int32_t n, hipStream_t s, bool build_tables) {
  std::unordered_map<std::string, const jat_tensor_ref*> by_name;
  for (int i = 0; i < n; ++i) by_name[named[i].name] = &named[i];
  const int D = m->D, kvD = m->kvD, mlp = m->mlp, bott = m->bott, depth = m->depth;
  const bool rms = m->cfg.norm_mode == JAT_NORM_RMS_W;

  size_t off = 0;
  auto take = [&](size_t bytes) { size_t o = off; off += align_up(bytes, 256); return o; };
  const size_t o_pe_w1 = take((size_t)bott * m->Kp * 2), o_pe_w2 = take((size_t)D * bott * 2);
  const size_t o_wada = take((size_t)depth * 6 * D * D * 2), o_wfinal = take((size_t)m->Fout * D * 2);
  std::vector<size_t> o_qkv(depth), o_wo(depth), o_w1(depth), o_w2(depth), o_n1(depth), o_n2(depth), o_b1(depth),
      o_b2(depth), o_qkvg(depth), o_q32(depth), o_k32(depth), o_v32(depth), o_w132(depth);
  const bool keep32 = rms;
  const bool group5 = m->Hq / m->Hkv == 5;
  for (int l = 0; l < depth; ++l) {
    o_qkv[l] = take((size_t)(D + 2 * kvD) * D * 2); o_wo[l] = take((size_t)D * D * 2);
    o_qkvg[l] = group5 ? take((size_t)(D + 2 * kvD) * D * 2) : 0;
    o_w1[l] = take((size_t)mlp * D * 2); o_w2[l] = take((size_t)D * mlp * 2);
    o_n1[l] = take((size_t)D * 4); o_n2[l] = take((size_t)D * 4);
    o_b1[l] = take((size_t)mlp * 4); o_b2[l] = take((size_t)D * 4);
    if (keep32) {
      o_q32[l] = take((size_t)D * D * 4); o_k32[l] = take((size_t)kvD * D * 4); o_v32[l] = take((size_t)kvD * D * 4);
      o_w132[l] = take((size_t)mlp * D * 4);
    }
  }
  const size_t o_wfinal32 = keep32 ? take((size_t)m->Fout * D * 4) : 0;
  const size_t o_pe_b1 = take((size_t)bott * 4), o_pe_b2 = take((size_t)D * 4);
  const size_t o_te_w1 = take((size_t)D * D * 4), o_te_b1 = take((size_t)D * 4);
  const size_t o_te_w2 = take((size_t)D * D * 4), o_te_b2 = take((size_t)D * 4);
  const size_t o_bada = take((size_t)depth * 6 * D * 4), o_fn = take((size_t)D * 4), o_bfinal = take((size_t)m->Fout * 4);
  const size_t o_cos = take((size_t)MAX_LEN * 32 * 4), o_sin = take((size_t)MAX_LEN * 32 * 4), o_invf = take(32 * 4);
  if (!m->blob) {
    HIPCHK(hipMalloc((void**)&m->blob, off));
    m->blob_bytes = off;
  }
  char* base = m->blob;
  m->pe_w1 = (bf16_t*)(base + o_pe_w1); m->pe_w2 = (bf16_t*)(base + o_pe_w2);
  m->wada = (bf16_t*)(base + o_wada); m->wfinal = (bf16_t*)(base + o_wfinal);
  m->pe_b1 = (float*)(base + o_pe_b1); m->pe_b2 = (float*)(base + o_pe_b2);
  m->te_w1 = (float*)(base + o_te_w1); m->te_b1 = (float*)(base + o_te_b1);
  m->te_w2 = (float*)(base + o_te_w2); m->te_b2 = (float*)(base + o_te_b2);
  m->bada = (float*)(base + o_bada); m->final_norm = (float*)(base + o_fn); m->bfinal = (float*)(base + o_bfinal);
  m->rope_cos = (float*)(base + o_cos); m->rope_sin = (float*)(base + o_sin); m->rope_invf = (float*)(base + o_invf);
  m->layers.resize(depth);
  for (int l = 0; l < depth; ++l) {
    LayerW& L = m->layers[l];
    L.wqkv = (bf16_t*)(base + o_qkv[l]); L.wo = (bf16_t*)(base + o_wo[l]);
    L.wqkv_g = group5 ? (bf16_t*)(base + o_qkvg[l]) : nullptr;
    L.w1 = (bf16_t*)(base + o_w1[l]); L.w2 = (bf16_t*)(base + o_w2[l]);
    L.norm1 = (float*)(base + o_n1[l]); L.norm2 = (float*)(base + o_n2[l]);
    L.b1 = (float*)(base + o_b1[l]); L.b2 = (float*)(base + o_b2[l]);
    if (keep32) {
      L.q32 = (float*)(base + o_q32[l]); L.k32 = (float*)(base + o_k32[l]); L.v32 = (float*)(base + o_v32[l]);
      L.w132 = (float*)(base + o_w132[l]);
    }
  }
  m->wfinal32 = keep32 ? (float*)(base + o_wfinal32) : nullptr;
  m->fold_cache.clear();
  m->fold_src_ok = false;

  int rc = JAT_OK;
  auto find = [&](const std::string& name, int64_t numel) -> const float* {
    auto it = by_name.find(name);
    if (it == by_name.end()) { rc = fail(JAT_E_STATE, "missing parameter '%s'", name.c_str()); return nullptr; }
    if (it->second->numel != numel) {
      rc = fail(JAT_E_INVALID, "parameter '%s' has %lld elements, expected %lld", name.c_str(),
// ... 166 lines not shown
  *norm_done = false;
  const GemmPlan plan = plan_resid(m, site, M, K, folding, w.kpart != nullptr);
  if (plan.ksplit == 1) {
    GemmArgs e{};
    e.out = w.x; e.ldo = D; e.bias = bias; e.gate = gate; e.gate_bstride = bstride; e.ntok = ntok;
    if (folding) { e.fold_out = w.xn; e.fold_lo = w.xlo; e.fold_part = w.part; }
    return jat_gemm(m, site, A, K, W, K, M, D, K, EPI_RESID, e, s, &plan);
  }
  GemmArgs p{};
  p.out = w.kpart; p.ldo = D; p.ntok = ntok; p.split_stride = (int64_t)M * D;
  JCHK(jat_gemm(m, site, A, K, W, K, M, D, K, EPI_F32, p, s, &plan));
  if (next && !folding && m->sw.fuse_finish && splitk_resid_norm_supported(D)) {
    KCHK(launch_splitk_resid_norm(w.kpart, plan.ksplit, (int64_t)M * D, bias, gate, bstride, w.x, next->w, next->shift, next->scale,
                                  bstride, w.xn, M, D, ntok, m->cfg.norm_mode, s));
    *norm_done = true;
  } else {
    KCHK(launch_splitk_resid_finish(w.kpart, plan.ksplit, (int64_t)M * D, bias, gate, bstride, ntok, w.x, M, D, s));
  }
  return JAT_OK;
}

static int run_block(const jat_model* m, const Workspace& w, int l, int B, int ntok, const float* mod_l,
                     int64_t bstride, hipStream_t s, const Fold* f = nullptr, bool xn_ready = false,
                     const NextNorm* next = nullptr, bool* next_done = nullptr) {
  const int D = m->D, M = B * ntok, Nqkv = D + 2 * m->kvD;
  const LayerW& L = m->layers[l];
  if (!f && !xn_ready) KCHK(launch_norm_modulate(w.x, L.norm1, mod_l + 0 * D, mod_l + 1 * D, bstride, w.xn, M, D, ntok, m->cfg.norm_mode, s));
  const int fuse_env = m->sw.fuse_qkv_attn;
  const bool fused_attn = f ? f->wqkv_g != nullptr
                            : (fuse_env && L.wqkv_g && !m->group_copy_stale && ntok == 128 && (B * m->Hkv >= 192 || fuse_env == 2));
  if (fused_attn) {
    GemmArgs a{};
    a.A = w.xn; a.lda = D; a.W = f ? f->wqkv_g + (int64_t)l * Nqkv * D : L.wqkv_g; a.ldw = D; a.M = M; a.N = m->Hkv * 448; a.K = D;
    a.out = w.ao; a.ldo = D; a.ntok = ntok; a.rope_inv_freq = m->rope_invf;
    a.attn_scale_log2e = kAttnScaleLog2e;
    if (f) { a.rs_part = w.part; a.rs_np = m->last_fold_np; a.bias = f->bq_g + (int64_t)l * Nqkv; }
    KCHK(launch_qkv_attn(a, s));
  } else {
    const GemmPlan plan = plan_qkv(m, M, D, f != nullptr, w.kpart != nullptr);
    if (plan.ksplit > 1) {
      GemmArgs p{};
      p.out = w.kpart; p.ldo = Nqkv; p.ntok = ntok; p.split_stride = (int64_t)M * Nqkv;
      JCHK(jat_gemm(m, G_QKV, w.xn, D, L.wqkv, D, M, Nqkv, D, EPI_F32, p, s, &plan));
      KCHK(launch_splitk_qkv_finish(w.kpart, plan.ksplit, (int64_t)M * Nqkv, m->rope_cos, m->rope_sin, w.q, w.k, w.vt, M, D, m->kvD,
                                    ntok, w.npad, s));
    } else {
      GemmArgs e = qkv_rope_args(m, w, ntok);
      if (f) { e.rs_part = w.part; e.bias = f->bq_i + (int64_t)l * Nqkv; }
      JCHK(jat_gemm(m, G_QKV, w.xn, D, f ? f->wqkv_i + (int64_t)l * Nqkv * D : L.wqkv, D, M, Nqkv, D, EPI_QKV_ROPE, e, s, &plan));
    }
    KCHK(launch_attention(attn_args(m, w, B, ntok), s));
  }
  const NextNorm norm2{L.norm2, mod_l + 3 * D, mod_l + 4 * D};
  bool norm2_done = false, done = false;
  JCHK(resid_gemm(m, w, G_OUT, w.ao, L.wo, D, nullptr, mod_l + 2 * D, bstride, M, ntok, f != nullptr, &norm2, &norm2_done, s));
  if (!f && !norm2_done) KCHK(launch_norm_modulate(w.x, L.norm2, mod_l + 3 * D, mod_l + 4 * D, bstride, w.xn, M, D, ntok, m->cfg.norm_mode, s));
  {
    GemmArgs e{};
    e.out = w.hm; e.ldo = m->mlp; e.bias = L.b1; e.ntok = ntok;
    if (f) { e.rs_part = w.part; e.bias = f->bf + (int64_t)l * m->mlp; }
    JCHK(jat_gemm(m, G_FC1, w.xn, D, f ? f->w1 + (int64_t)l * m->mlp * D : L.w1, D, M, m->mlp, D, EPI_BF16_GELU, e, s));
  }
  JCHK(resid_gemm(m, w, G_FC2, w.hm, L.w2, m->mlp, L.b2, mod_l + 5 * D, bstride, M, ntok, f != nullptr, next, &done, s));
  if (next_done) *next_done = done;
  return JAT_OK;
}

static int patch_linear1(const jat_model* m, const Workspace& w, int rows, int K, const float* pc, int ntok, hipStream_t s) {
  const GemmPlan plan = plan_patch(m, rows, K);
  GemmArgs e{};
  e.ldo = m->bott; e.ntok = ntok;
  if (plan.ksplit > 1) {
    e.out = w.hm; e.split_stride = (int64_t)rows * m->bott;
    JCHK(jat_gemm(m, G_OTHER, w.a_patch, K, m->pe_w1, m->Kp, rows, m->bott, K, EPI_F32, e, s, &plan));
    KCHK(launch_splitk_gelu_finish((const float*)w.hm, plan.ksplit, (int64_t)rows * m->bott, m->pe_b1, pc, pc ? rows : 0, w.h_patch,
                                   m->bott, rows, m->bott, s));
    return JAT_OK;
  }
  e.out = w.h_patch; e.bias = m->pe_b1;
  if (pc) { e.dual_add = pc; e.dual_rows = rows; }
  return jat_gemm(m, G_OTHER, w.a_patch, K, m->pe_w1, m->Kp, rows, m->bott, K, EPI_BF16_GELU, e, s, &plan);
}

static int forward_impl(const jat_model* m, const Workspace& w, const float* x_t, int B_src, const float* x_cond,
                        int cond_zero_from, const float* t, const float* mod, int64_t mod_bstride, float* x_pred,
                        int B, int T, hipStream_t s, const Fold* f = nullptr, const float* pc = nullptr) {
  const int ntok = (T + 3) / 4, M = B * ntok, D = m->D;
  if (!mod) {
    JCHK(time_path(m, w, t, B, s));
    JCHK(adaln_path(m, w.t_silu, w.mod, B, 0, m->depth, s));
    mod = w.mod;
    mod_bstride = (int64_t)m->depth * 6 * D;
  }
  if (t) HIPCHK(hipMemsetAsync(w.vt, 0, w.vt_bytes, s));
  if (pc) {
    KCHK(launch_patchify(x_t, nullptr, w.a_patch, B_src, B_src, B_src, m->Cin, 0, T, ntok, s, w.tvalid));
    JCHK(patch_linear1(m, w, M / 2, m->P * m->Cin, pc, ntok, s));
  } else {
    KCHK(launch_patchify(x_t, x_cond, w.a_patch, B, B_src, cond_zero_from, m->Cin, m->Cc, T, ntok, s, w.tvalid));
    JCHK(patch_linear1(m, w, M, m->Kp, nullptr, ntok, s));
  }
  {
    GemmArgs e{};
    e.out = w.x; e.ldo = D; e.bias = m->pe_b2; e.ntok = ntok;
    if (f) { e.fold_out = w.xn; e.fold_lo = w.xlo; e.fold_part = w.part; }
    JCHK(jat_gemm(m, G_OTHER, w.h_patch, m->bott, m->pe_w2, m->bott, M, D, m->bott, EPI_F32, e, s));
  }
  bool xn_ready = false;
  for (int l = 0; l < m->depth; ++l) {
    const float* mod_n = mod + (int64_t)(l + 1) * 6 * D;
    const NextNorm nn = l + 1 < m->depth ? NextNorm{m->layers[l + 1].norm1, mod_n + 0 * D, mod_n + 1 * D}
                                         : NextNorm{m->final_norm, nullptr, nullptr};
    bool done = false;
    JCHK(run_block(m, w, l, B, ntok, mod + (int64_t)l * 6 * D, mod_bstride, s, f, xn_ready, &nn, &done));
    xn_ready = done;
  }
  if (!f && !xn_ready) KCHK(launch_norm_modulate(w.x, m->final_norm, nullptr, nullptr, 0, w.xn, M, D, ntok, m->cfg.norm_mode, s));
  {
    GemmArgs e{};
    e.out = x_pred; e.bias = m->bfinal; e.ntok = ntok; e.C_out = m->Cin; e.T_orig = T;
    if (f) e.rs_part = w.part;
    JCHK(jat_gemm(m, G_OTHER, w.xn, D, f ? f->wfinal : m->wfinal, D, M, m->Fout, D, EPI_UNPATCH, e, s));
  }
  return JAT_OK;
}

static int check_ready(const jat_model* m, int B, int ntok, void* ws, size_t ws_bytes, Workspace* w) {
  if (!m) return fail(JAT_E_INVALID, "null model");
  if (!m->loaded) return fail(JAT_E_STATE, "weights not loaded");
  if (B <= 0 || ntok <= 0) return fail(JAT_E_INVALID, "B and T must be positive");
  if (ntok > MAX_LEN) return fail(JAT_E_SEQLEN, "Sequence length %d exceeds max_len %d", ntok, MAX_LEN);
  *w = carve(m, B, ntok, (char*)ws);
  if (!ws || ws_bytes < w->total)
    return fail(JAT_E_STATE, "workspace too small: %zu < %zu bytes", ws_bytes, w->total);
  return JAT_OK;
}

extern "C" int jat_forward(jat_model* m, const float* x_t, const float* t, const float* x_cond, float* x_pred,
                           int32_t B, int32_t T, void* ws, size_t ws_bytes, void* stream) {
  if (T <= 0) return fail(JAT_E_INVALID, "T must be positive");
  Workspace w;
  JCHK(check_ready(m, B, (T + 3) / 4, ws, ws_bytes, &w));
  return forward_impl(m, w, x_t, B, x_cond, B, t, nullptr, 0, x_pred, B, T, (hipStream_t)stream);
}

extern "C" int jat_time_embed(jat_model* m, const float* t, float* t_emb, int32_t B, void* ws, size_t ws_bytes,
                              void* stream) {
  Workspace w;
  JCHK(check_ready(m, B, 1, ws, ws_bytes, &w));
  hipStream_t s = (hipStream_t)stream;
  JCHK(time_path(m, w, t, B, s));
  HIPCHK(hipMemcpyAsync(t_emb, w.t_emb, (size_t)B * m->D * 4, hipMemcpyDeviceToDevice, s));
  return JAT_OK;
}

extern "C" int jat_block_forward(jat_model* m, int32_t layer, const float* x, const float* t_emb, float* y, int32_t B,
                                 int32_t N, void* ws, size_t ws_bytes, void* stream) {
  Workspace w;
  JCHK(check_ready(m, B, N, ws, ws_bytes, &w));
  if (layer < 0 || layer >= m->depth) return fail(JAT_E_INVALID, "layer out of range");
  hipStream_t s = (hipStream_t)stream;
  const size_t xb = (size_t)B * N * m->D * 4;
  KCHK(launch_silu_bf16(t_emb, w.t_silu, (int64_t)B * m->D, s));
  JCHK(adaln_path(m, w.t_silu, w.mod, B, layer, 1, s));
  HIPCHK(hipMemsetAsync(w.vt, 0, w.vt_bytes, s));
  HIPCHK(hipMemcpyAsync(w.x, x, xb, hipMemcpyDeviceToDevice, s));
  JCHK(run_block(m, w, layer, B, N, w.mod, (int64_t)6 * m->D, s));
  HIPCHK(hipMemcpyAsync(y, w.x, xb, hipMemcpyDeviceToDevice, s));
  return JAT_OK;
}

extern "C" int jat_attn_forward(jat_model* m, int32_t layer, const float* x, float* y, int32_t B, int32_t N, void* ws,
                                size_t ws_bytes, void* stream) {
  Workspace w;
  JCHK(check_ready(m, B, N, ws, ws_bytes, &w));
  if (layer < 0 || layer >= m->depth) return fail(JAT_E_INVALID, "layer out of range");
  hipStream_t s = (hipStream_t)stream;
  const int D = m->D, M = B * N;
  const LayerW& L = m->layers[layer];
  HIPCHK(hipMemsetAsync(w.vt, 0, w.vt_bytes, s));
  KCHK(launch_norm_modulate(x, nullptr, nullptr, nullptr, 0, w.xn, M, D, N, 2, s));
  JCHK(jat_gemm(m, G_QKV, w.xn, D, L.wqkv, D, M, D + 2 * m->kvD, D, EPI_QKV_ROPE, qkv_rope_args(m, w, N), s));
  KCHK(launch_attention(attn_args(m, w, B, N), s));
  {
    GemmArgs e{};
    e.out = y; e.ldo = D; e.ntok = N;
    JCHK(jat_gemm(m, G_OUT, w.ao, D, L.wo, D, M, D, D, EPI_F32, e, s));
  }
  return JAT_OK;
}

struct jat_sampler {
  jat_model* m;
  int B, T, steps, Bf;
  float cfg_scale;
  bool use_cfg;
  std::vector<float> ts;
  char* blob = nullptr;
  float *z, *lr, *xpred, *mod_table, *ts_dev;
  std::shared_ptr<FoldTable> fold;
  bool fused_attn = false;
  float* pc = nullptr;
  int* lens_dev = nullptr;
  int* frames_dev = nullptr;
  bool folded = false;
  void* ws;
  size_t ws_bytes;
  Workspace w;
  hipStream_t cap_stream = nullptr;
  hipGraph_t graph = nullptr;
  hipGraphExec_t exec = nullptr;
};

static void linspace01(int n, std::vector<float>& out) {
  out.resize(n);
  const float step = 1.0f / (float)(n - 1);
  for (int i = 0; i < n; ++i)
    out[i] = i < n / 2 ? (float)((double)step * i) : (float)(1.0 - (double)step * (n - 1 - i));
}

static int sampler_cond_part(jat_sampler* sp, hipStream_t s) {
  if (!sp->pc) return JAT_OK;
  jat_model* m = sp->m;
  const int ntok = (sp->T + 3) / 4, Kc = m->P * m->Cc;
  KCHK(launch_patchify(sp->lr, nullptr, sp->w.a_patch, sp->B, sp->B, sp->B, m->Cc, 0, sp->T, ntok, s, sp->w.tvalid));
  GemmArgs e{};
  e.out = sp->pc; e.ldo = m->bott; e.ntok = ntok;
  return jat_gemm(m, G_OTHER, sp->w.a_patch, Kc, m->pe_w1 + (int64_t)m->P * m->Cin, m->Kp, sp->B * ntok, m->bott, Kc, EPI_F32, e, s);
}

static int sampler_steps(jat_sampler* sp, hipStream_t s) {
  jat_model* m = sp->m;
  const int64_t n_half = (int64_t)sp->B * m->Cin * sp->T;
  const int64_t row = (int64_t)m->depth * 6 * m->D;
  for (int i = 0; i < sp->steps; ++i) {
    const float t_curr = sp->ts[i], dt = sp->ts[i + 1] - sp->ts[i];
    Fold f{};
    if (sp->folded) {
      const FoldTable& ft = *sp->fold;
      const int64_t Nqkv = m->D + 2 * m->kvD, dl = m->depth;
      if (sp->fused_attn) { f.wqkv_g = ft.qkv_g + (int64_t)i * dl * Nqkv * m->D; f.bq_g = ft.bq_g + (int64_t)i * dl * Nqkv; }
      else { f.wqkv_i = ft.qkv_i + (int64_t)i * dl * Nqkv * m->D; f.bq_i = ft.bq_i + (int64_t)i * dl * Nqkv; }
      f.w1 = ft.w1 + (int64_t)i * dl * m->mlp * m->D;
      f.bf = ft.bf + (int64_t)i * dl * m->mlp;
      f.wfinal = ft.wfinal;
    }
    JCHK(forward_impl(m, sp->w, sp->z, sp->B, sp->lr, sp->B, nullptr, sp->mod_table + i * row, 0, sp->xpred, sp->Bf,
                      sp->T, s, sp->folded ? &f : nullptr, sp->pc));
    KCHK(launch_cfg_euler(sp->xpred, sp->z, sp->cfg_scale, t_curr, dt, sp->use_cfg ? 1 : 0, n_half, s));
  }
  return JAT_OK;
}

static int fold_alloc(FoldTable& ft, void** p, size_t bytes) {
  if (hipMalloc(p, bytes) != hipSuccess) { (void)hipGetLastError(); return fail(JAT_E_HIP, "hipMalloc(%zu) for the folded weights", bytes); }
  ft.allocs.push_back(*p);
  return JAT_OK;
}
static int build_fold_table_impl(jat_model* m, FoldTable& ft, int steps, const float* mod, bool group_major, bf16_t* sh_bf16,
                                 hipStream_t s, bool need_w1, bool need_qkv);
static int build_fold_table(jat_model* m, FoldTable& ft, int steps, const float* mod, bool group_major, bf16_t* sh_bf16,
                            hipStream_t s) {
  const bool need_w1 = ft.w1 == nullptr;
  const bool need_qkv = group_major ? ft.qkv_g == nullptr : ft.qkv_i == nullptr;
  const size_t keep = ft.allocs.size();
  const int rc = build_fold_table_impl(m, ft, steps, mod, group_major, sh_bf16, s, need_w1, need_qkv);
  if (rc != JAT_OK) {
    (void)hipStreamSynchronize(s);
    while (ft.allocs.size() > keep) { (void)hipFree(ft.allocs.back()); ft.allocs.pop_back(); }
    if (need_w1) { ft.w1 = nullptr; ft.bf = nullptr; ft.wfinal = nullptr; }
    if (need_qkv) { if (group_major) { ft.qkv_g = nullptr; ft.bq_g = nullptr; } else { ft.qkv_i = nullptr; ft.bq_i = nullptr; } }
  }
  return rc;
}
static int build_fold_table_impl(jat_model* m, FoldTable& ft, int steps, const float* mod, bool group_major, bf16_t* sh_bf16,
                                 hipStream_t s, bool need_w1, bool need_qkv) {
  const int D = m->D, kvD = m->kvD, mlp = m->mlp, depth = m->depth, Nqkv = D + 2 * kvD;
  const int64_t mrow = (int64_t)depth * 6 * D;
  if (need_w1) {
    JCHK(fold_alloc(ft, (void**)&ft.w1, (size_t)steps * depth * mlp * D * 2));
    JCHK(fold_alloc(ft, (void**)&ft.bf, (size_t)steps * depth * mlp * 4));
    JCHK(fold_alloc(ft, (void**)&ft.wfinal, (size_t)m->Fout * D * 2));
    KCHK(launch_fold_weight(m->wfinal32, m->final_norm, nullptr, ft.wfinal, m->Fout, D, 0, s));
  }
  bf16_t* qkv = nullptr;
  float* bq = nullptr;
  if (need_qkv) {
    JCHK(fold_alloc(ft, (void**)&qkv, (size_t)steps * depth * Nqkv * D * 2));
    JCHK(fold_alloc(ft, (void**)&bq, (size_t)steps * depth * Nqkv * 4));
    if (group_major) { ft.qkv_g = qkv; ft.bq_g = bq; } else { ft.qkv_i = qkv; ft.bq_i = bq; }
  }
  ft.steps = steps;
  for (int l = 0; l < depth; ++l) {
    const LayerW& L = m->layers[l];
    for (int i = 0; i < steps; ++i) {
      const float* mod_il = mod + i * mrow + (int64_t)l * 6 * D;
      if (need_qkv) {
        bf16_t* dst = qkv + ((int64_t)i * depth + l) * Nqkv * D;
        if (group_major) {
          for (int g = 0; g < m->Hkv; ++g) {
            bf16_t* dg = dst + (int64_t)g * 448 * D;
            KCHK(launch_fold_weight(L.q32 + (int64_t)g * 320 * D, L.norm1, mod_il + D, dg, 320, D, 1, s));
            KCHK(launch_fold_weight(L.k32 + (int64_t)g * 64 * D, L.norm1, mod_il + D, dg + (int64_t)320 * D, 64, D, 1, s));
            KCHK(launch_fold_weight(L.v32 + (int64_t)g * 64 * D, L.norm1, mod_il + D, dg + (int64_t)384 * D, 64, D, 0, s));
          }
        } else {
          KCHK(launch_fold_weight(L.q32, L.norm1, mod_il + D, dst, D, D, 1, s));
          KCHK(launch_fold_weight(L.k32, L.norm1, mod_il + D, dst + (int64_t)D * D, kvD, D, 1, s));
          KCHK(launch_fold_weight(L.v32, L.norm1, mod_il + D, dst + (int64_t)(D + kvD) * D, kvD, D, 0, s));
        }
      }
      if (need_w1) KCHK(launch_fold_weight(L.w132, L.norm2, mod_il + 4 * D, ft.w1 + ((int64_t)i * depth + l) * mlp * D, mlp, D, 0, s));
    }
    if (need_qkv) {
      KCHK(launch_gather_cast_rows(mod + (int64_t)l * 6 * D, mrow, sh_bf16, steps, D, s));
      GemmArgs e{};
      e.out = bq + (int64_t)l * Nqkv; e.ldo = (int64_t)depth * Nqkv; e.ntok = 1;
      JCHK(jat_gemm(m, G_OTHER, sh_bf16, D, group_major ? L.wqkv_g : L.wqkv, D, steps, Nqkv, D, EPI_F32, e, s));
    }
    if (need_w1) {
      KCHK(launch_gather_cast_rows(mod + (int64_t)l * 6 * D + 3 * D, mrow, sh_bf16, steps, D, s));
      GemmArgs e{};
      e.out = ft.bf + (int64_t)l * mlp; e.ldo = (int64_t)depth * mlp; e.bias = L.b1; e.ntok = 1;
      JCHK(jat_gemm(m, G_OTHER, sh_bf16, D, L.w1, D, steps, mlp, D, EPI_F32, e, s));
    }
  }
  return JAT_OK;
}

extern "C" void jat_sampler_destroy(jat_sampler* sp) {
  if (!sp) return;
  if (sp->exec) (void)hipGraphExecDestroy(sp->exec);
  if (sp->graph) (void)hipGraphDestroy(sp->graph);
  if (sp->cap_stream) (void)hipStreamDestroy(sp->cap_stream);
  if (sp->blob) (void)hipFree(sp->blob);
  delete sp;
}

extern "C" int jat_sampler_create(jat_model* m, int32_t B, int32_t T, int32_t steps, float cfg_scale,
                                  jat_sampler** out) {
  if (!m || !out) return fail(JAT_E_INVALID, "null argument");
  if (!m->loaded) return fail(JAT_E_STATE, "weights not loaded");
  if (B <= 0 || T <= 0 || steps <= 0) return fail(JAT_E_INVALID, "B, T, steps must be positive");
  const int ntok = (T + 3) / 4;
  if (ntok > MAX_LEN) return fail(JAT_E_SEQLEN, "Sequence length %d exceeds max_len %d", ntok, MAX_LEN);
  HIPCHK(hipDeviceSynchronize());
  jat_sampler* sp = new jat_sampler();
  sp->m = m; sp->B = B; sp->T = T; sp->steps = steps; sp->cfg_scale = cfg_scale;
  sp->use_cfg = cfg_scale != 1.0f;
  sp->Bf = sp->use_cfg ? 2 * B : B;
  linspace01(steps + 1, sp->ts);

  const size_t lat = (size_t)B * m->Cin * T * 4;
  const size_t row = (size_t)m->depth * 6 * m->D;
  const int Bws = sp->Bf > steps ? sp->Bf : steps;
  const size_t ws_bytes = carve(m, Bws, ntok, nullptr).total;
  size_t off = 0;
  auto take = [&](size_t bytes) { size_t o = off; off += align_up(bytes, 256); return o; };
  const size_t o_z = take(lat), o_lr = take(lat), o_xp = take((size_t)sp->Bf * m->Cin * T * 4);
  const size_t o_tab = take((size_t)steps * row * 4), o_ts = take((size_t)steps * 4), o_ws = take(ws_bytes);
  sp->folded = plan_fold_norms(m, sp->Bf * ntok);
  const int fuse_env = m->sw.fuse_qkv_attn;
  sp->fused_attn = fuse_env && m->Hq / m->Hkv == 5 && !m->group_copy_stale && ntok == 128 && (sp->Bf * m->Hkv >= 192 || fuse_env == 2);
  const size_t o_sh = take((size_t)steps * m->D * 2);
  const size_t o_lens = take((size_t)sp->Bf * 4), o_frames = take((size_t)B * 4);
  const size_t o_pc = take((size_t)B * ntok * m->bott * 4);
  hipError_t e = hipMalloc((void**)&sp->blob, off);
  if (e != hipSuccess) { delete sp; return fail(JAT_E_HIP, "hipMalloc(%zu): %s", off, hipGetErrorString(e)); }
  sp->z = (float*)(sp->blob + o_z); sp->lr = (float*)(sp->blob + o_lr); sp->xpred = (float*)(sp->blob + o_xp);
  sp->mod_table = (float*)(sp->blob + o_tab); sp->ts_dev = (float*)(sp->blob + o_ts);
  sp->ws = sp->blob + o_ws; sp->ws_bytes = ws_bytes;
  bf16_t* sh_bf16 = (bf16_t*)(sp->blob + o_sh);
  sp->lens_dev = (int*)(sp->blob + o_lens);
  sp->frames_dev = (int*)(sp->blob + o_frames);
  if (sp->use_cfg && m->sw.split_patch) sp->pc = (float*)(sp->blob + o_pc);

  int rc = JAT_OK;
  auto bail = [&](int code) { jat_sampler_destroy(sp); return code; };
  if (hipStreamCreateWithFlags(&sp->cap_stream, hipStreamNonBlocking) != hipSuccess)
    return bail(fail(JAT_E_HIP, "hipStreamCreate failed"));
  hipStream_t s = sp->cap_stream;

  {
    Workspace wt = carve(m, steps, ntok, (char*)sp->ws);
    if (hipMemcpyAsync(sp->ts_dev, sp->ts.data(), (size_t)steps * 4, hipMemcpyHostToDevice, s) != hipSuccess)
      return bail(fail(JAT_E_HIP, "memcpy ts"));
    if ((rc = time_path(m, wt, sp->ts_dev, steps, s)) != JAT_OK) return bail(rc);
    if ((rc = adaln_path(m, wt.t_silu, sp->mod_table, steps, 0, m->depth, s)) != JAT_OK) return bail(rc);
    if (sp->folded) {
      for (auto it = m->fold_cache.begin(); it != m->fold_cache.end() && m->fold_cache.size() >= 2;)
        it = (it->first != steps && it->second.use_count() == 1) ? m->fold_cache.erase(it) : std::next(it);
      const size_t Nq = (size_t)m->D + 2 * m->kvD;
      const size_t need = (size_t)steps * m->depth * ((Nq + m->mlp) * m->D * 2 + (Nq + m->mlp) * 4) + (size_t)m->Fout * m->D * 2;
      const bool over_cap = m->sw.fold_cap_mb > 0 && need > (size_t)m->sw.fold_cap_mb * 1048576;
      std::shared_ptr<FoldTable>& slot = m->fold_cache[steps];
      if (!slot) slot = std::make_shared<FoldTable>();
      if (over_cap || build_fold_table(m, *slot, steps, sp->mod_table, sp->fused_attn, sh_bf16, s) != JAT_OK) {
        (void)hipStreamSynchronize(s);
        if (!slot->w1 && !slot->qkv_g && !slot->qkv_i) m->fold_cache.erase(steps);
        sp->folded = false;
      } else {
        sp->fold = slot;
      }
    }
    if (hipStreamSynchronize(s) != hipSuccess) return bail(fail(JAT_E_HIP, "sync after table build"));
  }
  sp->w = carve(m, sp->Bf, ntok, (char*)sp->ws);
  if (hipMemsetAsync(sp->w.vt, 0, sp->w.vt_bytes, s) != hipSuccess) return bail(fail(JAT_E_HIP, "memset vt"));
  {
    std::vector<int> full((size_t)sp->Bf, ntok), fullT((size_t)B, T);
    if (hipMemcpyAsync(sp->lens_dev, full.data(), full.size() * 4, hipMemcpyHostToDevice, s) != hipSuccess ||
        hipMemcpyAsync(sp->frames_dev, fullT.data(), fullT.size() * 4, hipMemcpyHostToDevice, s) != hipSuccess ||
        hipStreamSynchronize(s) != hipSuccess)
      return bail(fail(JAT_E_HIP, "lengths upload"));
    if (!sp->fused_attn) { sp->w.lens = sp->lens_dev; sp->w.tvalid = sp->frames_dev; }
  }

  if (hipMemsetAsync(sp->z, 0, lat, s) != hipSuccess || hipMemsetAsync(sp->lr, 0, lat, s) != hipSuccess)
    return bail(fail(JAT_E_HIP, "memset"));
  {
    const int saved = sp->steps;
    sp->steps = 1;
    if ((rc = sampler_cond_part(sp, s)) != JAT_OK) return bail(rc);
    rc = sampler_steps(sp, s);
    sp->steps = saved;
    if (rc != JAT_OK) return bail(rc);
    if (hipStreamSynchronize(s) != hipSuccess)
      return bail(fail(JAT_E_HIP, "eager warm-up step failed: %s", hipGetErrorString(hipGetLastError())));
  }
  if (hipStreamBeginCapture(s, hipStreamCaptureModeRelaxed) != hipSuccess)
    return bail(fail(JAT_E_HIP, "hipStreamBeginCapture failed"));
  rc = sampler_steps(sp, s);
  e = hipStreamEndCapture(s, &sp->graph);
  if (rc != JAT_OK) return bail(rc);
  if (e != hipSuccess) return bail(fail(JAT_E_HIP, "hipStreamEndCapture: %s", hipGetErrorString(e)));
  e = hipGraphInstantiate(&sp->exec, sp->graph, nullptr, nullptr, 0);
  if (e != hipSuccess) return bail(fail(JAT_E_HIP, "hipGraphInstantiate: %s", hipGetErrorString(e)));
  *out = sp;
  return JAT_OK;
}

extern "C" int jat_sampler_info(const jat_sampler* sp, int32_t* folded, int32_t* fused_attn, int64_t* fold_bytes) {
  if (!sp) return fail(JAT_E_INVALID, "null sampler");
  if (folded) *folded = sp->folded ? 1 : 0;
  if (fused_attn) *fused_attn = sp->fused_attn ? 1 : 0;
  if (fold_bytes) {
    const jat_model* m = sp->m;
    const size_t Nq = (size_t)m->D + 2 * m->kvD;
    *fold_bytes = sp->folded ? (int64_t)((size_t)sp->steps * m->depth * ((Nq + m->mlp) * m->D * 2 + (Nq + m->mlp) * 4) + (size_t)m->Fout * m->D * 2) : 0;
  }
  return JAT_OK;
}

extern "C" int jat_sampler_set_lengths(jat_sampler* sp, const int32_t* frames, int32_t n, void* stream) {
  if (!sp || !frames) return fail(JAT_E_INVALID, "null argument");
  if (n != sp->B) return fail(JAT_E_INVALID, "need one length per batch row (%d), got %d", sp->B, n);
  std::vector<int> tok((size_t)sp->Bf);
  bool all_full = true;
  for (int b = 0; b < sp->B; ++b) {
    if (frames[b] <= 0 || frames[b] > sp->T) return fail(JAT_E_INVALID, "length %d of row %d outside (0, %d]", frames[b], b, sp->T);
    tok[b] = (frames[b] + 3) / 4;
    if (sp->use_cfg) tok[sp->B + b] = tok[b];
    all_full = all_full && frames[b] == sp->T;
  }
  if (sp->fused_attn && !all_full)
    return fail(JAT_E_STATE, "this bucket runs the fused QKV+attention kernel (128 tokens), which has no key mask");
  hipStream_t s = (hipStream_t)stream;
  HIPCHK(hipMemcpyAsync(sp->lens_dev, tok.data(), tok.size() * 4, hipMemcpyHostToDevice, s));
  HIPCHK(hipMemcpyAsync(sp->frames_dev, frames, (size_t)sp->B * 4, hipMemcpyHostToDevice, s));
  HIPCHK(hipStreamSynchronize(s));
  return JAT_OK;
}

extern "C" int jat_sampler_run(jat_sampler* sp, const float* lr_latent, const float* z0, float* z_out,
                               int32_t use_graph, void* stream) {
  if (!sp || !lr_latent || !z0 || !z_out) return fail(JAT_E_INVALID, "null argument");
  hipStream_t s = (hipStream_t)stream;
  const size_t lat = (size_t)sp->B * sp->m->Cin * sp->T * 4;
  HIPCHK(hipMemcpyAsync(sp->lr, lr_latent, lat, hipMemcpyDeviceToDevice, s));
  HIPCHK(hipMemcpyAsync(sp->z, z0, lat, hipMemcpyDeviceToDevice, s));
  JCHK(sampler_cond_part(sp, s));
  if (use_graph) {
    HIPCHK(hipGraphLaunch(sp->exec, s));
  } else {
    JCHK(sampler_steps(sp, s));
  }
  HIPCHK(hipMemcpyAsync(z_out, sp->z, lat, hipMemcpyDeviceToDevice, s));
  return JAT_OK;
}

extern "C" int jat_cfg_euler_step(const float* x_pred_2B, float* z, float cfg_scale, float t, float dt, int32_t B,
                                  int32_t C, int32_t T, void* stream) {
  KCHK(launch_cfg_euler(x_pred_2B, z, cfg_scale, t, dt, cfg_scale != 1.0f ? 1 : 0, (int64_t)B * C * T,
                        (hipStream_t)stream));
  return JAT_OK;
}

extern "C" int jat_channel_affine(const float* in, const float* mean, const float* std, float* out, int32_t B, int32_t C,
                                  int32_t T, int32_t inverse, void* stream) {
  KCHK(launch_channel_affine(in, mean, std, out, B, C, T, inverse, (hipStream_t)stream));
  return JAT_OK;
}
extern "C" int jat_crossfade_pair(const float* prev, int32_t Tp, const float* cur, int32_t Tc, int32_t overlap,
                                  float* out, int32_t rows, void* stream) {
  KCHK(launch_crossfade_pair(prev, Tp, cur, Tc, overlap, out, rows, (hipStream_t)stream));
  return JAT_OK;
}

extern "C" int jat_k_norm_modulate(const float* x, const float* w, const float* shift, const float* scale,
                                   int64_t mod_bstride, uint16_t* y, int32_t M, int32_t D, int32_t rows_per_batch,
                                   int32_t norm_mode, void* stream) {
  KCHK(launch_norm_modulate(x, w, shift, scale, mod_bstride, y, M, D, rows_per_batch, norm_mode, (hipStream_t)stream));
  return JAT_OK;
}
static unsigned long long* timeline_out() {
  const char* d = getenv("JAT_GEMM_TIMELINE");
  return d ? (unsigned long long*)strtoull(d, nullptr, 0) : nullptr;
}
extern "C" int jat_k_gemm(const uint16_t* A, const uint16_t* W, const float* bias, void* C, int32_t M, int32_t N,
                          int32_t K, int32_t epilogue, const float* gate, int64_t gate_bstride, int32_t rows_per_batch,
                          int32_t variant, void* stream) {
  if (epilogue < 0 || epilogue > EPI_RESID) return fail(JAT_E_INVALID, "epilogue must be 0..3");
  GemmArgs a{};
  a.A = A; a.W = W; a.lda = K; a.ldw = K; a.M = M; a.N = N; a.K = K;
  a.out = C; a.ldo = N; a.bias = bias; a.gate = gate; a.gate_bstride = gate_bstride;
  a.ntok = rows_per_batch > 0 ? rows_per_batch : 1;
  a.dbg_out = timeline_out();
  KCHK(launch_gemm(a, epilogue, variant, (hipStream_t)stream));
  return JAT_OK;
}
extern "C" int jat_k_gemm_splitk(const uint16_t* A, const uint16_t* W, float* parts, int32_t M, int32_t N, int32_t K,
                                 int32_t ksplit, int32_t variant, void* stream) {
  if (!A || !W || !parts || M <= 0 || N <= 0 || ksplit < 2 || K % (64 * ksplit) != 0) return fail(JAT_E_INVALID, "bad argument");
  if (!gemm_variant(variant)) return fail(JAT_E_INVALID, "unknown variant");
  GemmArgs a{};
  a.A = A; a.W = W; a.lda = K; a.ldw = K; a.M = M; a.N = N; a.K = K / ksplit;
  a.out = parts; a.ldo = N; a.ntok = 1; a.ksplit = ksplit; a.split_stride = (int64_t)M * N;
  KCHK(launch_gemm(a, EPI_F32, variant, (hipStream_t)stream));
  return JAT_OK;
}
extern "C" int jat_k_gemm_wave_n(int32_t variant) { return gemm_variant(variant) ? gemm_variant(variant)->wave_n() : 0; }
extern "C" int jat_k_gemm_plan(const jat_model* m, int32_t site, int32_t M, int32_t N, int32_t K, int32_t folding, int32_t* variant,
                               int32_t* ksplit) {
  if (!m || !variant || !ksplit || site < 0 || site > G_OTHER || M <= 0 || N <= 0 || K <= 0 || K % 64 != 0) return fail(JAT_E_INVALID, "bad argument");
  const bool f = folding != 0, ws = split_ws_slices(M) > 0;
  const GemmPlan p = site == G_QKV && N == m->D + 2 * m->kvD         ? plan_qkv(m, M, K, f, ws)
                     : (site == G_OUT || site == G_FC2) && N == m->D ? plan_resid(m, site, M, K, f, ws)
                     : site == G_OTHER && N == m->bott               ? plan_patch(m, M, K)
                                                                     : plan_gemm(m, site, M, N, 1, f);
  *variant = p.variant; *ksplit = p.ksplit;
  return JAT_OK;
}
extern "C" int jat_k_gemm_fold(const uint16_t* A, const uint16_t* W, const float* bias, void* C, int32_t M, int32_t N, int32_t K,
                               int32_t epilogue, const float* gate, int64_t gate_bstride, int32_t rows_per_batch, uint16_t* hi,
                               uint16_t* lo, float* part_out, const float* part_in, int32_t part_in_np, int32_t variant,
                               void* stream) {
  if (epilogue < 0 || epilogue > EPI_RESID) return fail(JAT_E_INVALID, "epilogue must be 0..3");
  const GemmVariant* t = gemm_variant(variant);
  if (!t || !t->coalesced()) return fail(JAT_E_INVALID, "needs a coalesced-epilogue variant");
  if (hi && (epilogue != EPI_F32 && epilogue != EPI_RESID)) return fail(JAT_E_INVALID, "producer epilogue must be 0 or 3");
  if (hi && (!lo || !part_out)) return fail(JAT_E_INVALID, "producer needs hi, lo and part_out");
  if (part_in && part_in_np != 4 && part_in_np != 8 && part_in_np != 16) return fail(JAT_E_INVALID, "part_in_np must be 4, 8 or 16");
  GemmArgs a{};
  a.A = A; a.W = W; a.lda = K; a.ldw = K; a.M = M; a.N = N; a.K = K;
  a.out = C; a.ldo = N; a.bias = bias; a.gate = gate; a.gate_bstride = gate_bstride;
  a.ntok = rows_per_batch > 0 ? rows_per_batch : 1;
  a.fold_out = hi; a.fold_lo = lo; a.fold_part = part_out;
  if (hi) a.fold_np = N / t->wave_n();
  a.rs_part = part_in; a.rs_np = part_in_np;
  a.dbg_out = timeline_out();
  KCHK(launch_gemm(a, epilogue, variant, (hipStream_t)stream));
  return JAT_OK;
}
extern "C" int jat_k_qkv_attn(const uint16_t* A, const uint16_t* Wg, const float* bias, uint16_t* out, int32_t M, int32_t Hkv,
                              int32_t K, const float* rope_inv_freq, const float* part_in, int32_t part_in_np, void* stream) {
  if (!A || !Wg || !out || !rope_inv_freq || M <= 0 || M % 128 != 0 || K % 64 != 0) return fail(JAT_E_INVALID, "bad argument");
  GemmArgs a{};
  a.A = A; a.lda = K; a.W = Wg; a.ldw = K; a.M = M; a.N = Hkv * 448; a.K = K;
  a.out = out; a.ldo = (int64_t)Hkv * 320; a.ntok = 128; a.rope_inv_freq = rope_inv_freq; a.bias = bias;
  a.attn_scale_log2e = kAttnScaleLog2e;
  a.rs_part = part_in; a.rs_np = part_in_np;
  a.dbg_out = timeline_out();
  KCHK(launch_qkv_attn(a, (hipStream_t)stream));
  return JAT_OK;
}
extern "C" int jat_k_weight_grad(const uint16_t* dY, const uint16_t* X, float* dW, float* db, int32_t tokens, int32_t out,
                                 int32_t in, int32_t ksplit, void* work, size_t work_bytes, void* stream) {
  if (!gemm_tn_supports(out, in)) return fail(JAT_E_INVALID, "out and in must be multiples of 128");
  if (tokens <= 0) return fail(JAT_E_INVALID, "tokens must be positive");
  if (ksplit == 0) ksplit = gemm_tn_ksplit(out, in, tokens);
  if (ksplit < 1 || ksplit > (tokens + 63) / 64) return fail(JAT_E_INVALID, "bad ksplit");
  const int64_t area = (int64_t)out * in;
  const size_t part_f = ksplit > 1 ? (size_t)ksplit * area : 0, col_f = db ? (size_t)colsum_slices(tokens) * out : 0;
  const size_t need = 256 + (part_f + col_f) * 4;
  if (!work || work_bytes < need) return fail(JAT_E_INVALID, "work needs %zu bytes", need);
  hipStream_t s = (hipStream_t)stream;
  HIPCHK(hipMemsetAsync(work, 0, 256, s));
  float* part = (float*)((char*)work + 256);
  KCHK(launch_gemm_tn(dY, out, X, in, ksplit > 1 ? part : dW, in, out, in, tokens, ksplit, area, work, s));
  if (ksplit > 1) KCHK(launch_sum_partials(part, ksplit, area, dW, area, s));
  if (db) KCHK(launch_colsum_bf16(dY, out, tokens, out, part + part_f, db, s));
  return JAT_OK;
}
extern "C" int jat_k_attention(const uint16_t* q, const uint16_t* k, const uint16_t* vt, uint16_t* o, int32_t B,
                               int32_t N, int32_t Hq, int32_t Hkv, int32_t Npad, void* stream) {
  AttnArgs a{};
  a.q = q; a.k = k; a.vt = vt; a.o = o; a.ldq = (int64_t)Hq * 64; a.ldk = (int64_t)Hkv * 64; a.ldo = (int64_t)Hq * 64;
  a.B = B; a.N = N; a.Hq = Hq; a.Hkv = Hkv; a.npad = Npad;
  a.scale_log2e = kAttnScaleLog2e;
  KCHK(launch_attention(a, (hipStream_t)stream));
  return JAT_OK;
}
extern "C" int jat_prof_gemm_site(jat_model* m, int32_t site, int32_t max_launches) {
  if (!m) return fail(JAT_E_INVALID, "null model");
  if (site < -1 || site > G_OTHER) return fail(JAT_E_INVALID, "site must be -1 (off) or 0..4");
  m->prof.site = site; m->prof.n = 0; m->prof.flops = 0.0; m->prof.variant = -1;
  while ((int)m->prof.ev.size() < 2 * max_launches) {
    hipEvent_t e;
    HIPCHK(hipEventCreate(&e));
    m->prof.ev.push_back(e);
  }
  return JAT_OK;
}
extern "C" int jat_prof_collect(jat_model* m, double* total_ms, int32_t* launches, double* flops, int32_t* variant) {
  if (!m) return fail(JAT_E_INVALID, "null model");
  double tot = 0.0;
  for (int i = 0; i < m->prof.n; ++i) {
    HIPCHK(hipEventSynchronize(m->prof.ev[2 * i + 1]));
    float ms = 0.f;
    HIPCHK(hipEventElapsedTime(&ms, m->prof.ev[2 * i], m->prof.ev[2 * i + 1]));
    tot += ms;
  }
  if (m->prof.n > 0 && m->prof.ev.size() >= 2) {
    double ovh = 0.0;
    const int reps = 32;
    for (int i = 0; i < reps; ++i) {
      HIPCHK(hipEventRecord(m->prof.ev[0], m->prof.stream));
      HIPCHK(hipEventRecord(m->prof.ev[1], m->prof.stream));
      HIPCHK(hipEventSynchronize(m->prof.ev[1]));
      float ms = 0.f;
      HIPCHK(hipEventElapsedTime(&ms, m->prof.ev[0], m->prof.ev[1]));
      ovh += ms;
    }
    tot -= ovh / reps * m->prof.n;
    if (tot < 0.0) tot = 0.0;
  }
  if (total_ms) *total_ms = tot;
  if (launches) *launches = m->prof.n;
  if (flops) *flops = m->prof.flops;
  if (variant) *variant = m->prof.variant;
  m->prof.site = -1;
  return JAT_OK;
}
extern "C" int jat_k_cast_bf16(const float* in, uint16_t* out, int64_t n, void* stream) {
  KCHK(launch_cast_bf16(in, out, n, (hipStream_t)stream));
  return JAT_OK;
// ... 2 lines not shown
```

### jatsr-just-audio-transformer-super-solution_amd/csrc/jat_internal.h

```cpp
#pragma once
#include "../../include/jat_hip.h"

#include <hip/hip_runtime.h>

#include <map>
#include <memory>
#include <string>
#include <vector>

#include "jat_kernels.h"

int jat_fail(int code, const char* fmt, ...);
#define fail jat_fail
#define HIPCHK(expr)                                                                                   \
  do {                                                                                                 \
    hipError_t e__ = (expr);                                                                           \
    if (e__ != hipSuccess) return fail(JAT_E_HIP, "%s failed: %s (%s:%d)", #expr, hipGetErrorString(e__), \
                                       __FILE__, __LINE__);                                            \
  } while (0)
#define JCHK(expr)            \
  do {                        \
    int r__ = (expr);         \
    if (r__ != JAT_OK) return r__; \
  } while (0)
#define KCHK(expr)                                                                            \
  do {                                                                                        \
    hipError_t e__ = (expr);                                                                  \
    if (e__ != hipSuccess) return fail(JAT_E_HIP, "%s: %s", #expr, hipGetErrorString(e__));   \
  } while (0)

static inline size_t align_up(size_t v, size_t a) { return (v + a - 1) / a * a; }
static constexpr int MAX_LEN = 2048;
static constexpr int HEAD_DIM = 64;

struct LayerW {
  bf16_t *wqkv, *wo, *w1, *w2;
  bf16_t* wqkv_g = nullptr;
  float *norm1, *norm2, *b1, *b2;
  float *q32 = nullptr, *k32 = nullptr, *v32 = nullptr, *w132 = nullptr;
};

struct FoldTable {
  int steps = 0;
  bf16_t *qkv_g = nullptr, *qkv_i = nullptr;
  bf16_t *w1 = nullptr, *wfinal = nullptr;
  float *bq_g = nullptr, *bq_i = nullptr, *bf = nullptr;
  std::vector<void*> allocs;
  ~FoldTable() { for (void* p : allocs) (void)hipFree(p); }
};

struct jat_switches {
  int fuse_qkv_attn = 1;
  int qkv_split = 1;
  int fuse_finish = 1;
  int fold_norm = 1;
  int split_patch = 1;
  int fold_cap_mb = 0;
  int patch_split = 1;
};
struct GemmProf {
  int site = -1, n = 0, variant = -1;
  double flops = 0.0;
  hipStream_t stream = nullptr;
  std::vector<hipEvent_t> ev;
};

struct jat_model {
  jat_config cfg;
  jat_switches sw;
  mutable GemmProf prof;
  int D, depth, Hq, Hkv, kvD, mlp, bott, Cin, Cc, P, Kp, Fout;
  bool loaded = false;
  char* blob = nullptr;
  size_t blob_bytes = 0;
  bf16_t *pe_w1, *pe_w2, *wada, *wfinal;
  float *pe_b1, *pe_b2, *te_w1, *te_b1, *te_w2, *te_b2, *bada, *final_norm, *bfinal, *rope_cos, *rope_sin, *rope_invf;
  std::vector<LayerW> layers;
  int variants[5] = {-1, -1, -1, -1, -1};
  mutable int last_fold_np = 0;
  float* wfinal32 = nullptr;
  bool fold_src_ok = false;
  std::map<int, std::shared_ptr<FoldTable>> fold_cache;
  bool group_copy_stale = false;
};
enum { G_QKV = 0, G_OUT = 1, G_FC1 = 2, G_FC2 = 3, G_OTHER = 4 };

struct GemmPlan;
int jat_gemm(const jat_model* m, int site, const bf16_t* A, int64_t lda, const bf16_t* W, int64_t ldw, int M, int N, int K,
             int epi, GemmArgs extra, hipStream_t s, const GemmPlan* plan = nullptr);
int jat_pack_weights(jat_model* m, const jat_tensor_ref* named, int32_t n, hipStream_t s, bool build_tables);
```

### jatsr-just-audio-transformer-super-solution_amd/csrc/jat_kernels.h

```cpp
#pragma once
#include <hip/hip_runtime.h>
#include <stdint.h>

#include "jat_rng.h"

typedef uint16_t bf16_t;

enum GemmEpi : int {
  EPI_F32 = 0,
  EPI_BF16 = 1,
  EPI_BF16_GELU = 2,
  EPI_RESID = 3,
  EPI_QKV_ROPE = 4,
  EPI_QKV_ATTN = 6,
  EPI_UNPATCH = 5,
};

struct GemmArgs {
  const bf16_t* A;
  const bf16_t* W;
  int64_t lda, ldw;
  int M, N, K;
  void* out;
  int64_t ldo;
  const float* bias;
  const float* gate;
  int64_t gate_bstride;
  int ntok;
  bf16_t* k_out;
  bf16_t* vt_out;
  int D, kvD, npad;
  const float* rope_cos;
  const float* rope_sin;
  const float* rope_inv_freq;
  int C_out, T_orig;
  bf16_t* fold_out;
  bf16_t* fold_lo;
  float* fold_part;
  int fold_np;
  const float* rs_part;
  int rs_np;
  float attn_scale_log2e;
  const float* dual_add;
  int dual_rows;
  unsigned long long* dbg_out;
  int ksplit;
  int64_t split_stride;
  int variant_hint;
};

hipError_t launch_gemm(const GemmArgs& a, int epi, int variant, hipStream_t s);
hipError_t launch_qkv_attn(const GemmArgs& a, hipStream_t s);

struct AttnArgs {
  const bf16_t* q;
  const bf16_t* k;
  const bf16_t* vt;
  bf16_t* o;
  int64_t ldq, ldk, ldo;
  int B, N, Hq, Hkv, npad;
  float scale_log2e;
  float* lse;
  DropSpec drop;
  const int* lens;
};
hipError_t launch_attention(const AttnArgs& a, hipStream_t s);

hipError_t launch_norm_modulate(const float* x, const float* w, const float* shift, const float* scale,
                                int64_t mod_bstride, bf16_t* y, int M, int D, int ntok, int mode,
                                hipStream_t s);
hipError_t launch_patchify(const float* x_t, const float* x_cond, bf16_t* A, int B, int B_src,
                           int cond_zero_from, int C_t, int C_c, int T_orig, int ntok, hipStream_t s,
                           const int* tvalid = nullptr);
hipError_t launch_time_sinusoid(const float* t, float* e, int B, int D, hipStream_t s);
hipError_t launch_linear_f32(const float* in, const float* W, const float* bias, float* out,
                             bf16_t* out_silu_bf16, int B, int N, int K, int act_out, hipStream_t s);
hipError_t launch_splitk_gelu_finish(const float* part, int nsplit, int64_t stride, const float* bias, const float* dual_add,
                                     int dual_rows, bf16_t* out, int64_t ldo, int M, int N, hipStream_t s);
hipError_t launch_splitk_qkv_finish(const float* part, int nsplit, int64_t stride, const float* rope_cos, const float* rope_sin,
                                    bf16_t* q, bf16_t* k, bf16_t* vt, int M, int D, int kvD, int ntok, int npad, hipStream_t s);
bool splitk_resid_norm_supported(int D);
hipError_t launch_splitk_resid_norm(const float* part, int nsplit, int64_t stride, const float* bias, const float* gate,
                                    int64_t gate_bstride, float* x, const float* w, const float* shift, const float* scale,
                                    int64_t mod_bstride, bf16_t* y, int M, int D, int ntok, int mode, hipStream_t s);
hipError_t launch_splitk_resid_finish(const float* part, int nsplit, int64_t stride, const float* bias, const float* gate,
                                      int64_t gate_bstride, int ntok, float* x, int M, int N, hipStream_t s);
hipError_t launch_silu_bf16(const float* in, bf16_t* out, int64_t n, hipStream_t s);
hipError_t launch_cast_bf16(const float* in, bf16_t* out, int64_t n, hipStream_t s);
hipError_t launch_cast_bf16_rope_rows(const float* in, bf16_t* out, int rows, int cols, hipStream_t s);
hipError_t launch_fold_weight(const float* in, const float* w, const float* scale, bf16_t* out, int rows, int cols, int rope,
                              hipStream_t s);
hipError_t launch_fold_scale(const float* w, const float* scale, int64_t in_stride, float* out, int64_t out_stride,
                             int rows, int cols, hipStream_t s);
hipError_t launch_gather_cast_rows(const float* in, int64_t in_stride, bf16_t* out, int rows, int cols, hipStream_t s);
hipError_t launch_cfg_euler(const float* xp, float* z, float cfg_scale, float t, float dt, int use_cfg,
                            int64_t n_per_half, hipStream_t s);
hipError_t launch_channel_affine(const float* in, const float* mean, const float* std, float* out, int B,
                                 int C, int T, int inverse, hipStream_t s);
hipError_t launch_crossfade_pair(const float* prev, int Tp, const float* cur, int Tc, int overlap,
                                 float* out, int rows, hipStream_t s);

hipError_t launch_sum_partials(const float* part, int nsplit, int64_t stride, float* out, int64_t n, hipStream_t s);
hipError_t launch_transpose_bf16(const bf16_t* in, int64_t ld_in, int M, int C, bf16_t* out, int Mpad, hipStream_t s);
hipError_t launch_rowsum_bf16(const bf16_t* x, int64_t ld, int R, int n, float* out, hipStream_t s);
bool gemm_tn_supports(int M, int N);
int gemm_tn_ksplit(int M, int N, int K);
hipError_t launch_gemm_tn(const bf16_t* dY, int64_t ldy, const bf16_t* X, int64_t ldx, float* dW, int64_t ldo, int M, int N, int K,
                          int ksplit, int64_t split_stride, const void* zeros, hipStream_t s);
int colsum_slices(int R);
hipError_t launch_colsum_bf16(const bf16_t* x, int64_t ld, int R, int C, float* part, float* out, hipStream_t s);
hipError_t launch_gelu_bf16(const bf16_t* in, bf16_t* out, int64_t n, DropSpec drop, hipStream_t s);
hipError_t launch_gelu_bwd(const bf16_t* pre, bf16_t* d, int64_t n, DropSpec drop, hipStream_t s);
hipError_t launch_resid_gate(const float* x_in, const bf16_t* y, const float* gate, int64_t gate_bstride, float* x_out,
                             int M, int D, int ntok, DropSpec path, DropSpec elem, hipStream_t s);
int train_nchunk(int ntok);
int train_red_blocks();
hipError_t launch_gate_bwd(const float* dx, const bf16_t* y, const float* gate, int64_t gate_bstride, bf16_t* dy,
                           float* part, float* dgate, int64_t dgate_bstride, int B, int D, int ntok, DropSpec path,
                           DropSpec elem, hipStream_t s);
hipError_t launch_norm_bwd(const float* x, const bf16_t* dy, const float* w, const float* scale, int64_t mod_bstride,
                           float* dx, int accumulate, float* part, float* dw_part, float* dshift, float* dscale,
                           int64_t dmod_bstride, float* dw, int B, int D, int ntok, int mode, hipStream_t s);
hipError_t launch_attention_bwd(const bf16_t* q, const bf16_t* k, const bf16_t* vt, const bf16_t* o, const bf16_t* dout,
                                const float* lse, float* delta, bf16_t* dqkv, const float* rope_cos, const float* rope_sin,
                                int B, int N, int Hq, int Hkv, int npad, DropSpec drop, float* dkv_part, hipStream_t s);
hipError_t launch_mse_grad(const float* pred, const float* target, float* dpred, float* part, float* loss2, int64_t n,
                           float loss_scale, hipStream_t s);
hipError_t launch_charbonnier_grad(const float* pred, const float* target, float* dpred, float* part, float* loss2, int64_t n,
                                   float eps, float loss_scale, hipStream_t s);
hipError_t launch_latent_loss(const float* pred, const float* target, const float* lr, const float2* tw, float* dpred,
                              float* part, float* out6, int rows, int T, float lw, float fw, float mw, float cw, int low,
                              int strict, int soft, float loss_scale, hipStream_t s);
hipError_t launch_grad_sqsum(const float* g, int64_t n, float* part, float* norm2, hipStream_t s);
hipError_t launch_adamw(float* p, float* g, float* m, float* v, int64_t n, const float* norm2, float inv_scale,
                        float max_norm, float lr, float beta1, float beta2, float eps, float wd, int step, hipStream_t s);
hipError_t launch_small_dw(const float* dy, int64_t ldy, const float* x, int64_t ldx, float* dW, float* db, int B, int N,
                           int K, int silu_x, hipStream_t s);
int small_dx_slab(int N);
hipError_t launch_small_dx(const float* dy, int64_t ldy, const void* W, int w_is_bf16, float* part, float* dx, int B, int N,
                           int K, int accumulate, const float* silu_pre, hipStream_t s);
struct CopyJob { const float* src; float* dst; int64_t n; };
hipError_t launch_multi_copy(const CopyJob* jobs_dev, int njobs, hipStream_t s);
hipError_t launch_silu_f32(const float* in, float* out, int64_t n, hipStream_t s);
hipError_t launch_unpack_qkv_grad(const float* fused, float* gq, float* gk, float* gv, int D, int kvD, int K, hipStream_t s);
hipError_t launch_flow_mix(const float* x, const float* noise, const float* t, float* z, int B, int64_t per_sample, hipStream_t s);
hipError_t launch_cond_augment(float* cond, const float* noise, const float* std2, float ratio, const float* keep, int B,
                               int64_t per_sample, hipStream_t s);
hipError_t launch_tensor_std(const float* x, int64_t n, float* part, float* mean2, float* out2, hipStream_t s);
```

### jatsr-just-audio-transformer-super-solution_amd/sampler.py

```python
from __future__ import annotations

import ctypes as C

import torch

from . import _lib as L


class Sampler:

    def __init__(self, model, B, T, num_steps=50, cfg_scale=1.0):
        self.model = model
        self.B, self.T, self.steps, self.cfg_scale = int(B), int(T), int(num_steps), float(cfg_scale)
        self.ptr = C.c_void_p()
        self._build()

    def _build(self):
        self._destroy()
        h = self.model._get_handle()
        self._handle = h
        self._version = (h.version, getattr(h, "epoch", 0))
        self._lengths = None
        L.check(L.lib().jat_sampler_create(h.ptr, self.B, self.T, self.steps, self.cfg_scale, C.byref(self.ptr)))

    def _destroy(self):
        if self.ptr:
            L.lib().jat_sampler_destroy(self.ptr)
            self.ptr = C.c_void_p()

    def __del__(self):
        try:
            self._destroy()
        except Exception:
            pass

    def info(self):
        f, a, n = C.c_int32(0), C.c_int32(0), C.c_int64(0)
        L.check(L.lib().jat_sampler_info(self.ptr, C.byref(f), C.byref(a), C.byref(n)))
        return {"folded": bool(f.value), "fused_attn": bool(a.value), "fold_bytes": int(n.value)}

    def run(self, lr_latent, z0, use_graph=True, lengths=None):
        lr_latent = lr_latent.detach().to(torch.float32).contiguous()
        z0 = z0.detach().to(torch.float32).contiguous()
        if tuple(lr_latent.shape) != (self.B, self.model.input_channels, self.T) or z0.shape != lr_latent.shape:
            raise ValueError(f"sampler bucket is [B={self.B}, C={self.model.input_channels}, T={self.T}], got "
                             f"lr {tuple(lr_latent.shape)} z0 {tuple(z0.shape)}")
        h = self.model._get_handle()
        if (h.version, getattr(h, "epoch", 0)) != self._version:
            self._build()
        if lengths is None and self._lengths is not None:
            lengths = [self.T] * self.B
        if lengths is not None:
            lengths = [int(v) for v in lengths]
            if lengths != self._lengths:
                arr = (C.c_int32 * self.B)(*lengths)
                L.check(L.lib().jat_sampler_set_lengths(self.ptr, arr, self.B, L.stream_ptr()))
                self._lengths = lengths if any(v != self.T for v in lengths) else None
        out = torch.empty_like(z0)
        L.check(L.lib().jat_sampler_run(self.ptr, L.ptr(lr_latent), L.ptr(z0), L.ptr(out), 1 if use_graph else 0,
                                        L.stream_ptr()))
        return out


def _cached_sampler(model, B, T, num_steps, cfg_scale):
    cache = model.__dict__.setdefault("_jat_samplers", {})
    key = (B, T, num_steps, float(cfg_scale))
    s = cache.get(key)
    h = model._get_handle()
    if s is None or s._version != (h.version, getattr(h, "epoch", 0)):
        s = Sampler(model, B, T, num_steps, cfg_scale)
        cache[key] = s
    return s


@torch.no_grad()
def flow_matching_sample(model, lr_latent, num_steps=50, cfg_scale=1.0, device="cuda", verbose=True, z0=None,
                         use_graph=True, lengths=None):
    L.require_gpu()
    lr_latent = lr_latent.to(device)
    B, Cc, T = lr_latent.shape
    if z0 is None:
        z0 = torch.randn(B, Cc, T, device=lr_latent.device)
    if verbose:
        print(f"  Flow Matching sampling ({num_steps} steps, CFG scale={cfg_scale}) [hipGraph={bool(use_graph)}]")
    s = _cached_sampler(model, B, T, num_steps, cfg_scale)
    return s.run(lr_latent, z0.to(lr_latent.device), use_graph=use_graph, lengths=lengths)


def crossfade_chunks(chunks, overlap_frames):
    if len(chunks) == 0:
        return None
    if len(chunks) == 1:
        return chunks[0]
    L.require_gpu()
    result = chunks[0].contiguous()
    for cur in chunks[1:]:
        cur = cur.contiguous()
        ov = overlap_frames if (overlap_frames > 0 and result.shape[-1] >= overlap_frames) else 0
        rows = result.shape[0] * result.shape[1]
        Tp, Tc = result.shape[-1], cur.shape[-1]
        out = torch.empty(result.shape[0], result.shape[1], Tp + Tc - ov, dtype=torch.float32, device=result.device)
        L.check(L.lib().jat_crossfade_pair(L.ptr(result), Tp, L.ptr(cur), Tc, ov, L.ptr(out), rows, L.stream_ptr()))
        result = out
    return result


def chunk_plan(total_frames, chunk_frames=1378, overlap_frames=172):
    stride = chunk_frames - overlap_frames
    num = (total_frames - overlap_frames + stride - 1) // stride
    return [(i * stride, min(i * stride + chunk_frames, total_frames)) for i in range(num)]


def channel_affine(x, mean, std, inverse=False):
    L.require_gpu()
    x = x.contiguous()
    B, Cc, T = x.shape
    out = torch.empty_like(x)
    L.check(L.lib().jat_channel_affine(L.ptr(x), L.ptr(mean.contiguous().view(-1)), L.ptr(std.contiguous().view(-1)),
                                       L.ptr(out), B, Cc, T, 1 if inverse else 0, L.stream_ptr()))
    return out


# ... 49 lines not shown
```

Baseline: 39310 latent-frames/s.

## Fuse CFG combine and Euler update into the final unpatch GEMM epilogue

Adds an EPI_CFG_EULER GEMM epilogue that pairs each conditional row with its unconditional row in the same tile, exchanges them through LDS, and applies the CFG combine and Euler step directly. It writes the updated latent in patch-major f32 form plus the bf16 patchified input for the next step. This removes the separate xpred buffer, the standalone cfg_euler kernel and the patchify kernel from each step. The cost is a more complex tile row mapping, which is restricted to a few tile variants, and an extra patch/unpatch conversion at the sampler begin and end.

```diff
diff --git a/include/jat_hip.h b/include/jat_hip.h
--- a/include/jat_hip.h
+++ b/include/jat_hip.h
@@ -63,6 +63,7 @@
                        jat_sampler** out);
 void jat_sampler_destroy(jat_sampler* s);
 int jat_sampler_info(const jat_sampler* sampler, int32_t* folded, int32_t* fused_attn, int64_t* fold_bytes);
+int jat_sampler_tail_fused(const jat_sampler* sampler);
 int jat_sampler_set_lengths(jat_sampler* sampler, const int32_t* frames, int32_t n, void* stream);
 
 int jat_sampler_run(jat_sampler* s, const float* lr_latent, const float* z0_noise, float* z_out,
@@ -107,6 +108,10 @@
 int jat_k_gemm_fold(const uint16_t* A, const uint16_t* W, const float* bias, void* C, int32_t M, int32_t N, int32_t K,
                     int32_t epilogue, const float* gate, int64_t gate_bstride, int32_t rows_per_batch, uint16_t* hi,
                     uint16_t* lo, float* part_out, const float* part_in, int32_t part_in_np, int32_t variant, void* stream);
+int jat_k_gemm_cfg_euler(const uint16_t* A, const uint16_t* W, const float* bias, int32_t M, int32_t N, int32_t K,
+                         int32_t rows_per_batch, const float* part_in, int32_t part_in_np, float* z, uint16_t* a_patch,
+                         float* xpred, const int32_t* frames, float cfg_scale, float t, float dt, int32_t variant, int32_t fused,
+                         void* stream);
 int jat_k_gemm_splitk(const uint16_t* A, const uint16_t* W, float* parts, int32_t M, int32_t N, int32_t K, int32_t ksplit,
                       int32_t variant, void* stream);
 int jat_k_qkv_attn(const uint16_t* A, const uint16_t* Wg, const float* bias, uint16_t* out, int32_t M, int32_t Hkv, int32_t K,
diff --git a/jatsr-just-audio-transformer-super-solution_amd/_lib.py b/jatsr-just-audio-transformer-super-solution_amd/_lib.py
--- a/jatsr-just-audio-transformer-super-solution_amd/_lib.py
+++ b/jatsr-just-audio-transformer-super-solution_amd/_lib.py
@@ -53,6 +53,7 @@
     "jat_sampler_destroy": (None, [_VP]),
     "jat_sampler_run": (C.c_int, [_VP, _VP, _VP, _VP, _I32, _VP]),
     "jat_sampler_info": (C.c_int, [_VP, _VP, _VP, _VP]),
+    "jat_sampler_tail_fused": (C.c_int, [_VP]),
     "jat_sampler_set_lengths": (C.c_int, [_VP, C.POINTER(_I32), _I32, _VP]),
     "jat_cfg_euler_step": (C.c_int, [_VP, _VP, _F32, _F32, _F32, _I32, _I32, _I32, _VP]),
     "jat_channel_affine": (C.c_int, [_VP, _VP, _VP, _VP, _I32, _I32, _I32, _I32, _VP]),
@@ -60,6 +61,7 @@
     "jat_k_norm_modulate": (C.c_int, [_VP, _VP, _VP, _VP, _I64, _VP, _I32, _I32, _I32, _I32, _VP]),
     "jat_k_gemm": (C.c_int, [_VP, _VP, _VP, _VP, _I32, _I32, _I32, _I32, _VP, _I64, _I32, _I32, _VP]),
     "jat_k_gemm_fold": (C.c_int, [_VP, _VP, _VP, _VP, _I32, _I32, _I32, _I32, _VP, _I64, _I32, _VP, _VP, _VP, _VP, _I32, _I32, _VP]),
+    "jat_k_gemm_cfg_euler": (C.c_int, [_VP, _VP, _VP, _I32, _I32, _I32, _I32, _VP, _I32, _VP, _VP, _VP, _VP, _F32, _F32, _F32, _I32, _I32, _VP]),
     "jat_k_gemm_splitk": (C.c_int, [_VP, _VP, _VP, _I32, _I32, _I32, _I32, _I32, _VP]),
     "jat_k_gemm_wave_n": (C.c_int, [_I32]),
     "jat_k_gemm_plan": (C.c_int, [_VP, _I32, _I32, _I32, _I32, _I32, _VP, _VP]),
diff --git a/jatsr-just-audio-transformer-super-solution_amd/csrc/elementwise.hip b/jatsr-just-audio-transformer-super-solution_amd/csrc/elementwise.hip
--- a/jatsr-just-audio-transformer-super-solution_amd/csrc/elementwise.hip
+++ b/jatsr-just-audio-transformer-super-solution_amd/csrc/elementwise.hip
@@ -1,6 +1,7 @@
 #include "jat_kernels.h"
 #include "jat_gelu.h"
 #include "jat_dtype.h"
+#include "jat_cfg_euler.h"
 #include <cstdlib>
 
 __device__ __forceinline__ unsigned short f2bf_e(float f) { return jat_f2op(f); }
@@ -390,20 +391,20 @@
       float4 c = *(const float4*)(xp + i);
       if (use_cfg) {
         const float4 u = *(const float4*)(xp + n + i);
-        c.x = u.x + cfg_scale * (c.x - u.x); c.y = u.y + cfg_scale * (c.y - u.y);
-        c.z = u.z + cfg_scale * (c.z - u.z); c.w = u.w + cfg_scale * (c.w - u.w);
+        c.x = jat_cfg_combine(c.x, u.x, cfg_scale); c.y = jat_cfg_combine(c.y, u.y, cfg_scale);
+        c.z = jat_cfg_combine(c.z, u.z, cfg_scale); c.w = jat_cfg_combine(c.w, u.w, cfg_scale);
       }
       if (!direct) {
         const float4 zz = *(const float4*)(z + i);
-        c.x = zz.x + __fdiv_rn(c.x - zz.x, denom) * dt; c.y = zz.y + __fdiv_rn(c.y - zz.y, denom) * dt;
-        c.z = zz.z + __fdiv_rn(c.z - zz.z, denom) * dt; c.w = zz.w + __fdiv_rn(c.w - zz.w, denom) * dt;
+        c.x = jat_euler_step(c.x, zz.x, denom, dt); c.y = jat_euler_step(c.y, zz.y, denom, dt);
+        c.z = jat_euler_step(c.z, zz.z, denom, dt); c.w = jat_euler_step(c.w, zz.w, denom, dt);
       }
       *(float4*)(z + i) = c;
     } else {
       for (int64_t j = i; j < n; ++j) {
         float c = xp[j];
-        if (use_cfg) { const float u = xp[n + j]; c = u + cfg_scale * (c - u); }
-        if (!direct) c = z[j] + __fdiv_rn(c - z[j], denom) * dt;
+        if (use_cfg) c = jat_cfg_combine(c, xp[n + j], cfg_scale);
+        if (!direct) c = jat_euler_step(c, z[j], denom, dt);
         z[j] = c;
       }
     }
@@ -419,6 +420,30 @@
   hipLaunchKernelGGL(cfg_euler_kernel, dim3((unsigned)blocks), dim3(256), 0, s, xp, z, cfg_scale, denom, dt, use_cfg,
                      direct, n_per_half);
   return hipGetLastError();
+}
+
+template <bool TO_PATCH>
+__global__ void __launch_bounds__(256) patch_f32_kernel(const float* __restrict__ in, float* __restrict__ out, int C, int ntok,
+                                                        int64_t n) {
+  const int64_t i = (int64_t)blockIdx.x * blockDim.x + threadIdx.x;
+  if (i >= n) return;
+  const int c = (int)(i % C);
+  const int64_t row = i / C, b = row / ntok, tok = row - b * ntok;
+  const int64_t zi = ((b * C + c) * ntok + tok) * 4, pi = i * 4;
+  *(float4*)(out + (TO_PATCH ? pi : zi)) = *(const float4*)(in + (TO_PATCH ? zi : pi));
+}
+template <bool TO_PATCH>
+static hipError_t launch_patch_f32_dir(const float* in, float* out, int B, int C, int T, hipStream_t s) {
+  if (B <= 0 || C <= 0 || T <= 0 || (T & 3) != 0) return hipErrorInvalidValue;
+  const int64_t n = (int64_t)B * C * (T / 4);
+  hipLaunchKernelGGL(patch_f32_kernel<TO_PATCH>, dim3((unsigned)((n + 255) / 256)), dim3(256), 0, s, in, out, C, T / 4, n);
+  return hipGetLastError();
+}
+hipError_t launch_patch_f32(const float* z, float* zp, int B, int C, int T, hipStream_t s) {
+  return launch_patch_f32_dir<true>(z, zp, B, C, T, s);
+}
+hipError_t launch_unpatch_f32(const float* zp, float* z, int B, int C, int T, hipStream_t s) {
+  return launch_patch_f32_dir<false>(zp, z, B, C, T, s);
 }
 
 __global__ void channel_affine_kernel(const float* __restrict__ in, const float* __restrict__ mean,
diff --git a/jatsr-just-audio-transformer-super-solution_amd/csrc/gemm.hip b/jatsr-just-audio-transformer-super-solution_amd/csrc/gemm.hip
--- a/jatsr-just-audio-transformer-super-solution_amd/csrc/gemm.hip
+++ b/jatsr-just-audio-transformer-super-solution_amd/csrc/gemm.hip
@@ -1,6 +1,7 @@
 #include "jat_kernels.h"
 #include "jat_dtype.h"
 #include "gemm_variants.h"
+#include "jat_cfg_euler.h"
 
 #include <type_traits>
 #include <utility>
@@ -34,6 +35,22 @@
 
 __device__ __forceinline__ float2 rope_rot(float a, float b, float c, float s) {
   return float2{__builtin_fmaf(a, c, -(b * s)), __builtin_fmaf(b, c, a * s)};
+}
+
+__device__ __forceinline__ f32x4 unpatch_pred(f32x4 acc, float rstd, float4 b, bool has_bias) {
+#pragma clang fp contract(off)
+  f32x4 v = acc * rstd;
+  if (has_bias) { v[0] += b.x; v[1] += b.y; v[2] += b.z; v[3] += b.w; }
+  return v;
+}
+__device__ __forceinline__ f32x4 unpatch_pred(f32x4 acc, float rstd, const float* bias4) {
+#pragma clang fp contract(off)
+  f32x4 v = acc * rstd;
+  if (bias4) {
+    const float4 b = *(const float4*)bias4;
+    v[0] += b.x; v[1] += b.y; v[2] += b.z; v[3] += b.w;
+  }
+  return v;
 }
 
 template <int TM>
@@ -136,7 +153,10 @@
   const int wave = __builtin_amdgcn_readfirstlane(tid >> 6);
   const int wm = wave / WN, wn = wave % WN;
 
-  const int tiles_m = (p.M + BM - 1) / BM, tiles_n = p.N / BN;
+  constexpr bool PR = EPI == EPI_CFG_EULER;
+  static_assert(!PR || (WM % 2 == 0 && PIPE != 6), "paired rows: the wave rows split evenly over the halves; no DMA-wave form");
+  [[maybe_unused]] const int Mh = p.M >> 1;
+  const int tiles_m = PR ? (Mh + BM / 2 - 1) / (BM / 2) : (p.M + BM - 1) / BM, tiles_n = p.N / BN;
   int id;
   {
     const int nwg = gridDim.x, bid = blockIdx.x;
@@ -150,6 +170,11 @@
   const int in_g = id % per_group;
   const int m0 = (first_m + in_g % gsz) * BM;
   const int n0 = (in_g / gsz) * BN;
+  [[maybe_unused]] const int m0h = m0 >> 1;
+  [[maybe_unused]] auto pair_row = [&](int r) {
+    const int h = r >= BM / 2 ? 1 : 0;
+    return h * Mh + min(m0h + r - h * (BM / 2), Mh - 1);
+  };
 
   const int srow = lane >> 3;
   const int schunk = (lane & 7) ^ srow;
@@ -158,7 +183,7 @@
 #pragma unroll
   for (int j = 0; j < AI; ++j) {
     const int r = min(wave + j * NW, PA - 1) * 8 + srow;
-    const int gm = min(m0 + r, p.M - 1);
+    const int gm = PR ? pair_row(r) : min(m0 + r, p.M - 1);
     a_src[j] = p.A + (int64_t)gm * p.lda + schunk * 8;
   }
 #pragma unroll
@@ -220,7 +245,8 @@
 #pragma unroll
   for (int i = 0; i < TM; ++i) rstd_rows[i] = 1.0f;
   if (p.rs_part) {
-    rows_rstd_issue<TM>(p, m0 + wm * TM * 16, lane, rstd_raw);
+    const int rs_row0 = PR ? (wm >= WM / 2 ? Mh : 0) + m0h + (wm % (WM / 2 > 0 ? WM / 2 : 1)) * TM * 16 : m0 + wm * TM * 16;
+    rows_rstd_issue<TM>(p, rs_row0, lane, rstd_raw);
     if constexpr (PIPE != 8) rows_rstd_reduce<TM, 0>(p, rstd_raw, rstd_sums);
   }
 
@@ -302,7 +328,7 @@
     constexpr int CA0 = (PA0 + 7) / 8, CA1 = (PA1 + 7) / 8, CB0 = (PB0 + 7) / 8, CB1 = (PB1 + 7) / 8;
     constexpr int CTILE = CA0 + CA1 + CB0 + CB1;
     const int grp = wave >> 2;
-    const char* a_base = (const char*)(p.A + (int64_t)m0 * p.lda);
+    const char* a_base = (const char*)(p.A + (int64_t)(PR ? m0h : m0) * p.lda);
     const char* b_base = (const char*)(p.W + (int64_t)n0 * p.ldw);
     unsigned oa0[CA0], oa1[CA1 > 0 ? CA1 : 1], ob0[CB0], ob1[CB1];
     int la0[CA0], la1[CA1 > 0 ? CA1 : 1], lb0[CB0], lb1[CB1];
@@ -313,13 +339,15 @@
 #pragma unroll
     for (int j = 0; j < CA0; ++j) {
       const int r = piece_row(min(wave + 8 * j, PA0 - 1), TMa * 2, TM, 0);
-      oa0[j] = (unsigned)((min(m0 + r + srow, p.M - 1) - m0) * (int)p.lda * 2 + schunk * 16);
+      oa0[j] = PR ? (unsigned)((pair_row(r + srow) - m0h) * (int)p.lda * 2 + schunk * 16)
+                  : (unsigned)((min(m0 + r + srow, p.M - 1) - m0) * (int)p.lda * 2 + schunk * 16);
       la0[j] = r * 128;
     }
 #pragma unroll
     for (int j = 0; j < CA1; ++j) {
       const int r = piece_row(min(wave + 8 * j, PA1 - 1), TMb * 2, TM, TMa);
-      oa1[j] = (unsigned)((min(m0 + r + srow, p.M - 1) - m0) * (int)p.lda * 2 + schunk * 16);
+      oa1[j] = PR ? (unsigned)((pair_row(r + srow) - m0h) * (int)p.lda * 2 + schunk * 16)
+                  : (unsigned)((min(m0 + r + srow, p.M - 1) - m0) * (int)p.lda * 2 + schunk * 16);
       la1[j] = r * 128;
     }
     auto piece_row_b = [&](int q, int per, int first) {
@@ -979,6 +1007,70 @@
     return;
   }
 
+  if constexpr (PR) {
+    constexpr int TA = (TM + 1) / 2;
+    constexpr int XPAIR = TM * TN * 1024;
+    static_assert((NW / 2) * XPAIR <= 2 * STAGE, "exchange buffers do not fit the staging buffers");
+    __builtin_amdgcn_s_barrier();
+    if (p.M <= 0) return;
+    const int hc = wm >= WM / 2 ? 1 : 0, wmh = wm - hc * (WM / 2);
+    char* xb = smem + (wmh * WN + wn) * XPAIR + lane * 16;
+    float4 bb[TN];
+#pragma unroll
+    for (int j = 0; j < TN; ++j)
+      bb[j] = p.bias ? *(const float4*)(p.bias + nw0 + j * 16 + fg * 4) : float4{0.f, 0.f, 0.f, 0.f};
+    const bool has_bias = p.bias != nullptr;
+#pragma unroll
+    for (int i = 0; i < TM; ++i)
+#pragma unroll
+      for (int j = 0; j < TN; ++j) acc[i][j] = unpatch_pred(acc[i][j], rstd_rows[i], bb[j], has_bias);
+    static_for<0, TM>([&](auto ic) __attribute__((always_inline)) {
+      constexpr int i = decltype(ic)::value;
+      if ((i >= TA) == (hc == 0)) {
+#pragma unroll
+        for (int j = 0; j < TN; ++j) *(f32x4*)(xb + (i * TN + j) * 1024) = acc[i][j];
+      }
+    });
+    asm volatile("s_waitcnt lgkmcnt(0)" ::: "memory");
+    __builtin_amdgcn_s_barrier();
+    float* const zp = (float*)p.out;
+    const float cs = p.ce_scale, denom = p.ce_denom, dt = p.ce_dt;
+    const bool direct = p.ce_direct != 0;
+    static_for<0, TM>([&](auto ic) __attribute__((always_inline)) {
+      constexpr int i = decltype(ic)::value;
+      if ((i >= TA) == (hc == 1)) {
+        const int mh = m0h + wmh * TM * 16 + i * 16 + frow;
+        if (mh < Mh) {
+          const int b = mh / p.ntok, tok = mh - b * p.ntok;
+          const int left = p.ce_frames ? p.ce_frames[b] - 4 * tok : 4;
+          float* zr = zp + (int64_t)mh * p.ldo + nw0 + fg * 4;
+          bf16_t* ar = p.ce_patch + (int64_t)mh * p.ldo + nw0 + fg * 4;
+          float4 zz[TN];
+          if (!direct) {
+#pragma unroll
+            for (int j = 0; j < TN; ++j) zz[j] = *(const float4*)(zr + j * 16);
+          }
+#pragma unroll
+          for (int j = 0; j < TN; ++j) {
+            const f32x4 o = *(const f32x4*)(xb + (i * TN + j) * 1024);
+            const f32x4 c = hc ? o : acc[i][j], u = hc ? acc[i][j] : o;
+            float x[4];
+#pragma unroll
+            for (int e = 0; e < 4; ++e) x[e] = jat_cfg_combine(c[e], u[e], cs);
+            if (!direct) {
+              x[0] = jat_euler_step(x[0], zz[j].x, denom, dt); x[1] = jat_euler_step(x[1], zz[j].y, denom, dt);
+              x[2] = jat_euler_step(x[2], zz[j].z, denom, dt); x[3] = jat_euler_step(x[3], zz[j].w, denom, dt);
+            }
+            *(float4*)(zr + j * 16) = float4{x[0], x[1], x[2], x[3]};
+            *(uint2*)(ar + j * 16) = pack4(left > 0 ? x[0] : 0.f, left > 1 ? x[1] : 0.f, left > 2 ? x[2] : 0.f, left > 3 ? x[3] : 0.f);
+          }
+        }
+      }
+    });
+    JAT_TL_FLUSH()
+    return;
+  }
+
 #pragma unroll
   for (int i = 0; i < TM; ++i) {
     const int m = m0 + wm * TM * 16 + i * 16 + frow;
@@ -993,7 +1085,12 @@
     for (int j = 0; j < TN; ++j) {
       const int nt = nw0 + j * 16;
       const int n = nt + fg * 4;
-      f32x4 v = acc[i][j] * rstd_d;
+      f32x4 v;
+      if constexpr (EPI == EPI_UNPATCH) {
+        v = unpatch_pred(acc[i][j], rstd_d, p.bias ? p.bias + n : nullptr);
+      } else {
+        v = acc[i][j] * rstd_d;
+      }
       if constexpr (EPI == EPI_QKV_ROPE) {
         if (nt < p.D + p.kvD) {
           const int d0 = ((nt & 63) >> 1) + fg * 2;
@@ -1011,7 +1108,7 @@
           for (int r = 0; r < 4; ++r) dst[(int64_t)r * p.npad] = f2bf(v[r]);
         }
       } else {
-        if (p.bias) {
+        if (EPI != EPI_UNPATCH && p.bias) {
           const float4 bb = *(const float4*)(p.bias + n);
           v[0] += bb.x; v[1] += bb.y; v[2] += bb.z; v[3] += bb.w;
         }
@@ -1665,12 +1762,18 @@
     attr_set = true;
   }
   if (a.N % BN != 0 || a.K % 64 != 0 || a.M <= 0) return hipErrorInvalidValue;
-  const int tiles = ((a.M + BM - 1) / BM) * (a.N / BN);
+  if (EPI == EPI_CFG_EULER && (a.M % 2 != 0 || !a.out || !a.ce_patch || a.ntok <= 0 || a.ldo < a.N || a.ldo % 4 != 0 ||
+                               (int64_t)a.M * a.lda * 2 >= (1ll << 31)))
+    return hipErrorInvalidValue;
+  const int tiles = (EPI == EPI_CFG_EULER ? (a.M / 2 + BM / 2 - 1) / (BM / 2) : (a.M + BM - 1) / BM) * (a.N / BN);
   if (a.ksplit > 1 && EPI != EPI_F32) return hipErrorInvalidValue;
   hipLaunchKernelGGL(kern, dim3(tiles, a.ksplit > 1 ? a.ksplit : 1), dim3((WM * WN + (PIPE == 6 ? 4 : 0)) * 64), LDS, s, a);
   return hipGetLastError();
 }
 
+static constexpr bool cfg_euler_tile(int WM, int WN, int TM, int TN, int PIPE, int CE) {
+  return CE == 1 && WM == 2 && TN == 4 && ((PIPE == 2 && WN == 2 && (TM == 2 || TM == 4)) || (PIPE == 8 && WN == 4 && (TM == 7 || TM == 8)));
+}
 template <int WM, int WN, int TM, int TN, int PIPE, int CE = 0>
 static hipError_t launch_epi(const GemmArgs& a, int epi, hipStream_t s) {
   switch (epi) {
@@ -1680,6 +1783,9 @@
     case EPI_RESID: return launch_one<WM, WN, TM, TN, PIPE, CE, EPI_RESID>(a, s);
     case EPI_QKV_ROPE: return launch_one<WM, WN, TM, TN, PIPE, CE, EPI_QKV_ROPE>(a, s);
     case EPI_UNPATCH: return launch_one<WM, WN, TM, TN, PIPE, CE, EPI_UNPATCH>(a, s);
+    case EPI_CFG_EULER:
+      if constexpr (cfg_euler_tile(WM, WN, TM, TN, PIPE, CE)) return launch_one<WM, WN, TM, TN, PIPE, CE, EPI_CFG_EULER>(a, s);
+      break;
   }
   return hipErrorInvalidValue;
 }
@@ -1708,6 +1814,11 @@
   return e;
 }
 
+bool gemm_cfg_euler_supported(int variant) {
+  const GemmVariant* v = gemm_variant(variant);
+  return v && v->fallback < 0 && cfg_euler_tile(v->WM, v->WN, v->TM, v->TN, v->PIPE, v->CE);
+}
+
 hipError_t launch_gemm(const GemmArgs& a, int epi, int variant, hipStream_t s) {
   const GemmVariant* v = gemm_variant(variant);
   if (!v) return hipErrorInvalidValue;
diff --git a/jatsr-just-audio-transformer-super-solution_amd/csrc/jat_api.cpp b/jatsr-just-audio-transformer-super-solution_amd/csrc/jat_api.cpp
--- a/jatsr-just-audio-transformer-super-solution_amd/csrc/jat_api.cpp
+++ b/jatsr-just-audio-transformer-super-solution_amd/csrc/jat_api.cpp
@@ -97,7 +97,7 @@
   auto env_int = [](const char* name, int dflt) { const char* v = getenv(name); return v ? atoi(v) : dflt; };
   m->sw.fuse_qkv_attn = env_int("JAT_FUSE_QKV_ATTN", 1); m->sw.qkv_split = env_int("JAT_QKV_SPLIT", 1);
   m->sw.fuse_finish = env_int("JAT_FUSE_FINISH", 1); m->sw.fold_norm = env_int("JAT_FOLD_NORM", 1);
-  m->sw.split_patch = env_int("JAT_SPLIT_PATCH", 1);
+  m->sw.split_patch = env_int("JAT_SPLIT_PATCH", 1); m->sw.fuse_euler = env_int("JAT_FUSE_EULER", 1);
   m->sw.fold_cap_mb = env_int("JAT_FOLD_CAP_MB", 0); m->sw.patch_split = env_int("JAT_PATCH_SPLIT", 1);
   if (const char* v = getenv("JAT_GEMM_VARIANT"))
     for (int i = 0; i < 5; ++i) m->variants[i] = atoi(v);
@@ -115,7 +115,8 @@
   const std::string n(name);
   int* slot = n == "fuse_qkv_attn" ? &m->sw.fuse_qkv_attn : n == "qkv_split" ? &m->sw.qkv_split : n == "fuse_finish" ? &m->sw.fuse_finish
             : n == "fold_norm" ? &m->sw.fold_norm : n == "split_patch" ? &m->sw.split_patch
-            : n == "fold_cap_mb" ? &m->sw.fold_cap_mb : n == "patch_split" ? &m->sw.patch_split : nullptr;
+            : n == "fold_cap_mb" ? &m->sw.fold_cap_mb : n == "patch_split" ? &m->sw.patch_split
+            : n == "fuse_euler" ? &m->sw.fuse_euler : nullptr;
   if (!slot) return fail(JAT_E_INVALID, "unknown switch '%s'", name);
   *slot = value;
   return JAT_OK;
@@ -448,9 +449,15 @@
   return jat_gemm(m, G_OTHER, w.a_patch, K, m->pe_w1, m->Kp, rows, m->bott, K, EPI_BF16_GELU, e, s, &plan);
 }
 
+struct FusedTail {
+  float* zp;
+  float cfg_scale, t, dt;
+};
+
 static int forward_impl(const jat_model* m, const Workspace& w, const float* x_t, int B_src, const float* x_cond,
                         int cond_zero_from, const float* t, const float* mod, int64_t mod_bstride, float* x_pred,
-                        int B, int T, hipStream_t s, const Fold* f = nullptr, const float* pc = nullptr) {
+                        int B, int T, hipStream_t s, const Fold* f = nullptr, const float* pc = nullptr,
+                        const FusedTail* tail = nullptr) {
   const int ntok = (T + 3) / 4, M = B * ntok, D = m->D;
   if (!mod) {
     JCHK(time_path(m, w, t, B, s));
@@ -460,7 +467,7 @@
   }
   if (t) HIPCHK(hipMemsetAsync(w.vt, 0, w.vt_bytes, s));
   if (pc) {
-    KCHK(launch_patchify(x_t, nullptr, w.a_patch, B_src, B_src, B_src, m->Cin, 0, T, ntok, s, w.tvalid));
+    if (!tail) KCHK(launch_patchify(x_t, nullptr, w.a_patch, B_src, B_src, B_src, m->Cin, 0, T, ntok, s, w.tvalid));
     JCHK(patch_linear1(m, w, M / 2, m->P * m->Cin, pc, ntok, s));
   } else {
     KCHK(launch_patchify(x_t, x_cond, w.a_patch, B, B_src, cond_zero_from, m->Cin, m->Cc, T, ntok, s, w.tvalid));
@@ -486,7 +493,11 @@
     GemmArgs e{};
     e.out = x_pred; e.bias = m->bfinal; e.ntok = ntok; e.C_out = m->Cin; e.T_orig = T;
     if (f) e.rs_part = w.part;
-    JCHK(jat_gemm(m, G_OTHER, w.xn, D, f ? f->wfinal : m->wfinal, D, M, m->Fout, D, EPI_UNPATCH, e, s));
+    if (tail) {
+      e.out = tail->zp; e.ldo = m->Fout; e.ce_patch = w.a_patch; e.ce_frames = w.tvalid;
+      e.ce_scale = tail->cfg_scale; e.ce_denom = 1.0f - tail->t + 1e-5f; e.ce_dt = tail->dt; e.ce_direct = !(tail->t < 0.999f);
+    }
+    JCHK(jat_gemm(m, G_OTHER, w.xn, D, f ? f->wfinal : m->wfinal, D, M, m->Fout, D, tail ? EPI_CFG_EULER : EPI_UNPATCH, e, s));
   }
   return JAT_OK;
 }
@@ -564,6 +575,8 @@
   std::vector<float> ts;
   char* blob = nullptr;
   float *z, *lr, *xpred, *mod_table, *ts_dev;
+  float* zp = nullptr;
+  bool tail_fused = false;
   std::shared_ptr<FoldTable> fold;
   bool fused_attn = false;
   float* pc = nullptr;
@@ -593,6 +606,19 @@
   GemmArgs e{};
   e.out = sp->pc; e.ldo = m->bott; e.ntok = ntok;
   return jat_gemm(m, G_OTHER, sp->w.a_patch, Kc, m->pe_w1 + (int64_t)m->P * m->Cin, m->Kp, sp->B * ntok, m->bott, Kc, EPI_F32, e, s);
+}
+
+static int sampler_begin(jat_sampler* sp, hipStream_t s) {
+  JCHK(sampler_cond_part(sp, s));
+  if (!sp->tail_fused) return JAT_OK;
+  const jat_model* m = sp->m;
+  KCHK(launch_patch_f32(sp->z, sp->zp, sp->B, m->Cin, sp->T, s));
+  KCHK(launch_patchify(sp->z, nullptr, sp->w.a_patch, sp->B, sp->B, sp->B, m->Cin, 0, sp->T, sp->T / 4, s, sp->w.tvalid));
+  return JAT_OK;
+}
+static int sampler_end(jat_sampler* sp, hipStream_t s) {
+  if (sp->tail_fused) KCHK(launch_unpatch_f32(sp->zp, sp->z, sp->B, sp->m->Cin, sp->T, s));
+  return JAT_OK;
 }
 
 static int sampler_steps(jat_sampler* sp, hipStream_t s) {
@@ -611,9 +637,10 @@
       f.bf = ft.bf + (int64_t)i * dl * m->mlp;
       f.wfinal = ft.wfinal;
     }
+    const FusedTail tail{sp->zp, sp->cfg_scale, t_curr, dt};
     JCHK(forward_impl(m, sp->w, sp->z, sp->B, sp->lr, sp->B, nullptr, sp->mod_table + i * row, 0, sp->xpred, sp->Bf,
-                      sp->T, s, sp->folded ? &f : nullptr, sp->pc));
-    KCHK(launch_cfg_euler(sp->xpred, sp->z, sp->cfg_scale, t_curr, dt, sp->use_cfg ? 1 : 0, n_half, s));
+                      sp->T, s, sp->folded ? &f : nullptr, sp->pc, sp->tail_fused ? &tail : nullptr));
+    if (!sp->tail_fused) KCHK(launch_cfg_euler(sp->xpred, sp->z, sp->cfg_scale, t_curr, dt, sp->use_cfg ? 1 : 0, n_half, s));
   }
   return JAT_OK;
 }
@@ -723,7 +750,11 @@
   const size_t ws_bytes = carve(m, Bws, ntok, nullptr).total;
   size_t off = 0;
   auto take = [&](size_t bytes) { size_t o = off; off += align_up(bytes, 256); return o; };
-  const size_t o_z = take(lat), o_lr = take(lat), o_xp = take((size_t)sp->Bf * m->Cin * T * 4);
+  const int Mf = sp->Bf * ntok;
+  sp->tail_fused = m->sw.fuse_euler && sp->use_cfg && m->sw.split_patch && T % 4 == 0 && (int64_t)Mf * m->D * 2 < (1ll << 31) &&
+                   gemm_cfg_euler_supported(plan_gemm(m, G_OTHER, Mf, m->Fout, 1, true).variant) &&
+                   gemm_cfg_euler_supported(plan_gemm(m, G_OTHER, Mf, m->Fout, 1, false).variant);
+  const size_t o_z = take(lat), o_lr = take(lat), o_xp = take(sp->tail_fused ? 0 : (size_t)sp->Bf * m->Cin * T * 4);
   const size_t o_tab = take((size_t)steps * row * 4), o_ts = take((size_t)steps * 4), o_ws = take(ws_bytes);
   sp->folded = plan_fold_norms(m, sp->Bf * ntok);
   const int fuse_env = m->sw.fuse_qkv_attn;
@@ -731,15 +762,18 @@
   const size_t o_sh = take((size_t)steps * m->D * 2);
   const size_t o_lens = take((size_t)sp->Bf * 4), o_frames = take((size_t)B * 4);
   const size_t o_pc = take((size_t)B * ntok * m->bott * 4);
+  const size_t o_zp = take(sp->tail_fused ? lat : 0);
   hipError_t e = hipMalloc((void**)&sp->blob, off);
   if (e != hipSuccess) { delete sp; return fail(JAT_E_HIP, "hipMalloc(%zu): %s", off, hipGetErrorString(e)); }
-  sp->z = (float*)(sp->blob + o_z); sp->lr = (float*)(sp->blob + o_lr); sp->xpred = (float*)(sp->blob + o_xp);
+  sp->z = (float*)(sp->blob + o_z); sp->lr = (float*)(sp->blob + o_lr);
+  sp->xpred = sp->tail_fused ? nullptr : (float*)(sp->blob + o_xp);
   sp->mod_table = (float*)(sp->blob + o_tab); sp->ts_dev = (float*)(sp->blob + o_ts);
   sp->ws = sp->blob + o_ws; sp->ws_bytes = ws_bytes;
   bf16_t* sh_bf16 = (bf16_t*)(sp->blob + o_sh);
   sp->lens_dev = (int*)(sp->blob + o_lens);
   sp->frames_dev = (int*)(sp->blob + o_frames);
   if (sp->use_cfg && m->sw.split_patch) sp->pc = (float*)(sp->blob + o_pc);
+  if (sp->tail_fused) sp->zp = (float*)(sp->blob + o_zp);
 
   int rc = JAT_OK;
   auto bail = [&](int code) { jat_sampler_destroy(sp); return code; };
@@ -787,8 +821,9 @@
   {
     const int saved = sp->steps;
     sp->steps = 1;
-    if ((rc = sampler_cond_part(sp, s)) != JAT_OK) return bail(rc);
+    if ((rc = sampler_begin(sp, s)) != JAT_OK) return bail(rc);
     rc = sampler_steps(sp, s);
+    if (rc == JAT_OK) rc = sampler_end(sp, s);
     sp->steps = saved;
     if (rc != JAT_OK) return bail(rc);
     if (hipStreamSynchronize(s) != hipSuccess)
@@ -817,6 +852,8 @@
   }
   return JAT_OK;
 }
+
+extern "C" int jat_sampler_tail_fused(const jat_sampler* sp) { return sp && sp->tail_fused ? 1 : 0; }
 
 extern "C" int jat_sampler_set_lengths(jat_sampler* sp, const int32_t* frames, int32_t n, void* stream) {
   if (!sp || !frames) return fail(JAT_E_INVALID, "null argument");
@@ -845,12 +882,13 @@
   const size_t lat = (size_t)sp->B * sp->m->Cin * sp->T * 4;
   HIPCHK(hipMemcpyAsync(sp->lr, lr_latent, lat, hipMemcpyDeviceToDevice, s));
   HIPCHK(hipMemcpyAsync(sp->z, z0, lat, hipMemcpyDeviceToDevice, s));
-  JCHK(sampler_cond_part(sp, s));
+  JCHK(sampler_begin(sp, s));
   if (use_graph) {
     HIPCHK(hipGraphLaunch(sp->exec, s));
   } else {
     JCHK(sampler_steps(sp, s));
   }
+  JCHK(sampler_end(sp, s));
   HIPCHK(hipMemcpyAsync(z_out, sp->z, lat, hipMemcpyDeviceToDevice, s));
   return JAT_OK;
 }
@@ -938,6 +976,33 @@
   KCHK(launch_gemm(a, epilogue, variant, (hipStream_t)stream));
   return JAT_OK;
 }
+extern "C" int jat_k_gemm_cfg_euler(const uint16_t* A, const uint16_t* W, const float* bias, int32_t M, int32_t N, int32_t K,
+                                    int32_t rows_per_batch, const float* part_in, int32_t part_in_np, float* z, uint16_t* a_patch,
+                                    float* xpred, const int32_t* frames, float cfg_scale, float t, float dt, int32_t variant,
+                                    int32_t fused, void* stream) {
+  if (!A || !W || !z || !a_patch || M <= 0 || M % 2 != 0 || N % 128 != 0 || K % 64 != 0 || rows_per_batch <= 0 ||
+      (M / 2) % rows_per_batch != 0)
+    return fail(JAT_E_INVALID, "bad argument");
+  if (part_in && part_in_np != 4 && part_in_np != 8 && part_in_np != 16) return fail(JAT_E_INVALID, "part_in_np must be 4, 8 or 16");
+  if (fused ? !gemm_cfg_euler_supported(variant) : (!gemm_variant(variant) || !xpred))
+    return fail(JAT_E_INVALID, fused ? "variant has no CFG + Euler epilogue" : "unknown variant or no xpred");
+  hipStream_t s = (hipStream_t)stream;
+  const int ntok = rows_per_batch, B = M / 2 / ntok, C = N / 4, T = ntok * 4;
+  GemmArgs a{};
+  a.A = A; a.W = W; a.lda = K; a.ldw = K; a.M = M; a.N = N; a.K = K; a.bias = bias; a.ntok = ntok;
+  a.rs_part = part_in; a.rs_np = part_in_np;
+  if (fused) {
+    a.out = z; a.ldo = N; a.ce_patch = a_patch; a.ce_frames = frames;
+    a.ce_scale = cfg_scale; a.ce_denom = 1.0f - t + 1e-5f; a.ce_dt = dt; a.ce_direct = !(t < 0.999f);
+    KCHK(launch_gemm(a, EPI_CFG_EULER, variant, s));
+    return JAT_OK;
+  }
+  a.out = xpred; a.C_out = C; a.T_orig = T;
+  KCHK(launch_gemm(a, EPI_UNPATCH, variant, s));
+  KCHK(launch_cfg_euler(xpred, z, cfg_scale, t, dt, 1, (int64_t)B * C * T, s));
+  KCHK(launch_patchify(z, nullptr, a_patch, B, B, B, C, 0, T, ntok, s, frames));
+  return JAT_OK;
+}
 extern "C" int jat_k_qkv_attn(const uint16_t* A, const uint16_t* Wg, const float* bias, uint16_t* out, int32_t M, int32_t Hkv,
                               int32_t K, const float* rope_inv_freq, const float* part_in, int32_t part_in_np, void* stream) {
   if (!A || !Wg || !out || !rope_inv_freq || M <= 0 || M % 128 != 0 || K % 64 != 0) return fail(JAT_E_INVALID, "bad argument");
diff --git a/jatsr-just-audio-transformer-super-solution_amd/csrc/jat_cfg_euler.h b/jatsr-just-audio-transformer-super-solution_amd/csrc/jat_cfg_euler.h
--- /dev/null
+++ b/jatsr-just-audio-transformer-super-solution_amd/csrc/jat_cfg_euler.h
@@ -0,0 +1,7 @@
+#pragma once
+#include <hip/hip_runtime.h>
+
+__device__ __forceinline__ float jat_cfg_combine(float c, float u, float s) { return __builtin_fmaf(s, c - u, u); }
+__device__ __forceinline__ float jat_euler_step(float x, float z, float denom, float dt) {
+  return __builtin_fmaf(__fdiv_rn(x - z, denom), dt, z);
+}
diff --git a/jatsr-just-audio-transformer-super-solution_amd/csrc/jat_internal.h b/jatsr-just-audio-transformer-super-solution_amd/csrc/jat_internal.h
--- a/jatsr-just-audio-transformer-super-solution_amd/csrc/jat_internal.h
+++ b/jatsr-just-audio-transformer-super-solution_amd/csrc/jat_internal.h
@@ -57,6 +57,7 @@
   int split_patch = 1;
   int fold_cap_mb = 0;
   int patch_split = 1;
+  int fuse_euler = 1;
 };
 struct GemmProf {
   int site = -1, n = 0, variant = -1;
diff --git a/jatsr-just-audio-transformer-super-solution_amd/csrc/jat_kernels.h b/jatsr-just-audio-transformer-super-solution_amd/csrc/jat_kernels.h
--- a/jatsr-just-audio-transformer-super-solution_amd/csrc/jat_kernels.h
+++ b/jatsr-just-audio-transformer-super-solution_amd/csrc/jat_kernels.h
@@ -14,6 +14,7 @@
   EPI_QKV_ROPE = 4,
   EPI_QKV_ATTN = 6,
   EPI_UNPATCH = 5,
+  EPI_CFG_EULER = 7,
 };
 
 struct GemmArgs {
@@ -27,10 +28,12 @@
   const float* gate;
   int64_t gate_bstride;
   int ntok;
-  bf16_t* k_out;
+  union { bf16_t* k_out; bf16_t* ce_patch; };
   bf16_t* vt_out;
-  int D, kvD, npad;
-  const float* rope_cos;
+  union { int D; float ce_scale; };
+  union { int kvD; float ce_denom; };
+  union { int npad; float ce_dt; };
+  union { const float* rope_cos; const int* ce_frames; };
   const float* rope_sin;
   const float* rope_inv_freq;
   int C_out, T_orig;
@@ -46,10 +49,11 @@
   unsigned long long* dbg_out;
   int ksplit;
   int64_t split_stride;
-  int variant_hint;
+  union { int variant_hint; int ce_direct; };
 };
 
 hipError_t launch_gemm(const GemmArgs& a, int epi, int variant, hipStream_t s);
+bool gemm_cfg_euler_supported(int variant);
 hipError_t launch_qkv_attn(const GemmArgs& a, hipStream_t s);
 
 struct AttnArgs {
@@ -95,6 +99,8 @@
 hipError_t launch_gather_cast_rows(const float* in, int64_t in_stride, bf16_t* out, int rows, int cols, hipStream_t s);
 hipError_t launch_cfg_euler(const float* xp, float* z, float cfg_scale, float t, float dt, int use_cfg,
                             int64_t n_per_half, hipStream_t s);
+hipError_t launch_patch_f32(const float* z, float* zp, int B, int C, int T, hipStream_t s);
+hipError_t launch_unpatch_f32(const float* zp, float* z, int B, int C, int T, hipStream_t s);
 hipError_t launch_channel_affine(const float* in, const float* mean, const float* std, float* out, int B,
                                  int C, int T, int inverse, hipStream_t s);
 hipError_t launch_crossfade_pair(const float* prev, int Tp, const float* cur, int Tc, int overlap,
diff --git a/jatsr-just-audio-transformer-super-solution_amd/sampler.py b/jatsr-just-audio-transformer-super-solution_amd/sampler.py
--- a/jatsr-just-audio-transformer-super-solution_amd/sampler.py
+++ b/jatsr-just-audio-transformer-super-solution_amd/sampler.py
@@ -38,6 +38,9 @@
         f, a, n = C.c_int32(0), C.c_int32(0), C.c_int64(0)
         L.check(L.lib().jat_sampler_info(self.ptr, C.byref(f), C.byref(a), C.byref(n)))
         return {"folded": bool(f.value), "fused_attn": bool(a.value), "fold_bytes": int(n.value)}
+
+    def tail_fused(self):
+        return bool(L.lib().jat_sampler_tail_fused(self.ptr))
 
     def run(self, lr_latent, z0, use_graph=True, lengths=None):
         lr_latent = lr_latent.detach().to(torch.float32).contiguous()
```

New measurement: 39800 latent-frames/s (median of 6 runs). +1.3%, better.
